# adobe-research/DiffusionHandles

Hardware: AMD Instinct MI355X
Metric: guided-denoise steps/sec at 512x512 (SD2-depth) (higher is better)
Workload: dtype f16; 1 GPU; single 512x512 edit per GPU, SD2-depth (865.9M params, seeded random weights), guided phase: 3 x (fwd + energy + bwd-to-latent) + CFG fwd (B=2) + DDIM step; resolution=512, edits_per_gpu=1, correspondences=24906, parallelism=independent edits, one process per GPU, no collectives

## Files before the change

diffusionhandles_amd/_lib.py:

```python
import ctypes
import os

import torch

_HERE = os.path.dirname(os.path.abspath(__file__))
LIB_PATH = os.environ.get("DIFFHANDLES_LIB") or os.path.join(_HERE, "libdiffhandles_hip.so")
_LIB = None

c_p = ctypes.c_void_p
c_i = ctypes.c_int
c_f = ctypes.c_float
c_d = ctypes.c_double
c_sz = ctypes.c_size_t


class UNetConfig(ctypes.Structure):
    _fields_ = [("in_channels", c_i), ("out_channels", c_i), ("n_levels", c_i),
                ("block_out_channels", c_i * 4), ("layers_per_block", c_i), ("heads", c_i * 4),
                ("cross_attention_dim", c_i), ("norm_groups", c_i), ("sample_size", c_i),
                ("text_len", c_i), ("max_batch", c_i), ("dtype", c_i), ("max_diff_batch", c_i)]


class VAEConfig(ctypes.Structure):
    _fields_ = [("latent_channels", c_i), ("out_channels", c_i), ("block_out_channels", c_i * 4),
# ... 74 lines not shown
    "dh_vae_encoder_create": (c_i, [c_p, ctypes.POINTER(c_p)]),
    "dh_vae_encoder_encode": (c_i, [c_p, c_p, c_i, c_p, c_p]),
    "dh_text_encoder_create": (c_i, [c_p, ctypes.POINTER(c_p)]),
    "dh_text_encoder_destroy": (None, [c_p]),
    "dh_text_encoder_num_params": (c_i, [c_p]),
    "dh_text_encoder_param_info": (c_i, [c_p, c_i, ctypes.POINTER(ctypes.c_char_p), ctypes.POINTER(c_i),
                                         ctypes.POINTER(ctypes.c_int64)]),
    "dh_text_encoder_load_param": (c_i, [c_p, c_i, c_p, c_p]),
    "dh_text_encoder_bytes": (c_sz, [c_p]),
    "dh_text_encoder_encode": (c_i, [c_p, c_p, c_i, c_i, c_p, c_p]),
    "dh_gemm_profile_begin": (c_i, []),
    "dh_gemm_profile_end": (c_i, [ctypes.POINTER(c_d), ctypes.POINTER(ctypes.c_int64), ctypes.POINTER(c_d)]),
    "dh_gemm_profile_bytes": (c_i, [ctypes.POINTER(c_d)]),
    "dh_ddim_cfg_step": (c_i, [c_p, c_p, c_p, c_p, c_f, c_f, c_f, c_i, c_p]),
    "dh_latent_update": (c_i, [c_p, c_p, c_p, c_f, c_f, c_i, c_p]),
    "dh_adam_step": (c_i, [c_p, c_p, c_p, c_p, c_f, c_f, c_f, c_f, c_i, c_i, c_p]),
    "dh_mse_fwd_bwd": (c_i, [c_p, c_p, c_i, c_p, c_p, c_p]),
    "dh_latent_update_strided": (c_i, [c_p, c_p, c_p, c_i, c_i, c_f, c_f, c_i, c_p]),
    "dh_pack_sample": (c_i, [c_p, c_p, c_i, c_i, c_p, c_i, c_i, c_i, c_i, c_p]),
    "dh_unet_io_ptr": (c_i, [c_p, c_i, c_i, ctypes.POINTER(c_p), ctypes.POINTER(c_sz)]),
    "dh_mse_cotangent": (c_i, [c_p, c_p, c_i, c_f, c_f, c_p, c_p, c_p, c_p]),
    "dh_adam_step_scaled": (c_i, [c_p, c_p, c_p, c_p, c_p, c_f, c_f, c_f, c_f, c_i, c_i, c_p]),
    "dh_mse_cotangent_batch": (c_i, [c_p, c_p, c_i, c_i, c_f, c_f, c_d, c_p, c_p, c_p, c_p, c_p, c_p]),
    "dh_adam_step_scaled_batch": (c_i, [c_p, c_p, c_p, c_p, c_p, c_p, c_f, c_f, c_f, c_f, c_i, c_i, c_i, c_p]),
    "dh_latent_update_guarded": (c_i, [c_p, c_p, c_p, c_i, c_i, c_f, c_i, c_i, c_p, c_i, c_i, c_p, c_p, c_i, c_i, c_p]),
    "dh_ddim_cfg_step_flagged": (c_i, [c_p, c_p, c_p, c_p, c_f, c_f, c_f, c_i, c_i, c_p, c_i, c_i, c_p]),
}

c_l = ctypes.c_long
DEBUG_SIGNATURES = {
    "dh_dbg_gemm": (c_i, [c_i, c_p, c_l, c_p, c_i, c_i, c_i, c_i, c_i, c_i, c_i, c_i, c_i, c_i, c_i, c_p, c_p, c_i, c_i,
                          c_p, c_l, c_p, c_l, c_i, c_p, c_sz, c_p]),
    "dh_dbg_gemm_groupnorm": (c_i, [c_i, c_p, c_l, c_p, c_i, c_i, c_i, c_i, c_i, c_i, c_i, c_p, c_p, c_p, c_sz, c_i, c_i, c_p, c_p, c_f, c_i,
                                    c_p, c_p, c_p, ctypes.POINTER(c_i), c_p]),
    "dh_dbg_gemm_groupnorm_bwd": (c_i, [c_i, c_p, c_l, c_p, c_i, c_i, c_i, c_i, c_i, c_i, c_i, c_p, c_p, c_sz, c_i, c_i, c_p, c_p, c_p, c_p, c_i,
                                        c_p, c_p, ctypes.POINTER(c_i), c_p]),
    "dh_dbg_gemm_groupnorm_res": (c_i, [c_i, c_p, c_l, c_p, c_i, c_i, c_i, c_i, c_i, c_i, c_i, c_p, c_p, c_l, c_p, c_p, c_sz, c_i, c_i, c_p, c_p,
                                    c_f, c_i, c_p, c_p, c_p, ctypes.POINTER(c_i), c_p]),
    "dh_dbg_gemm_groupnorm_bwd_res": (c_i, [c_i, c_p, c_l, c_p, c_i, c_i, c_i, c_i, c_i, c_i, c_i, c_p, c_l, c_p, c_p, c_sz, c_i, c_i, c_p, c_p, c_p,
                                        c_p, c_i, c_p, c_p, ctypes.POINTER(c_i), c_p]),
    "dh_dbg_concat_groupnorm": (c_i, [c_i, c_p, c_i, c_p, c_i, c_p, c_i, c_i, c_i, c_p, c_p, c_f, c_i, c_p, c_p, c_p, c_p]),
    "dh_dbg_gemm_last_tile": (c_i, [ctypes.POINTER(c_i)]),
    "dh_dbg_unet_concat_ops": (c_i, [ctypes.POINTER(UNetConfig), ctypes.POINTER(c_i), c_i, ctypes.POINTER(c_i)]),
    "dh_dbg_gemm_lnfold": (c_i, [c_i, c_p, c_l, c_p, c_i, c_i, c_i, c_p, c_p, c_p, c_f, c_p, c_l, c_p]),
    "dh_dbg_gemm_glu": (c_i, [c_i, c_i, c_p, c_l, c_p, c_i, c_i, c_i, c_p, c_p, c_p, c_p, c_p, c_p]),
    "dh_dbg_gemm_glub_split": (c_i, [c_i, c_p, c_l, c_p, c_i, c_i, c_i, c_i, c_p, c_l, c_i, c_p, c_p, ctypes.POINTER(c_i), c_p]),
    "dh_dbg_unet_ff_fold": (c_i, [c_p, c_i, ctypes.POINTER(c_i), ctypes.POINTER(c_i), c_p, c_p, c_p]),
    "dh_dbg_gemm_family": (c_i, [c_i]),
    "dh_dbg_gemm_stage": (c_i, [c_i]),
    "dh_dbg_gemm_xattn": (c_i, [c_i, c_p, c_l, c_p, c_i, c_i, c_i, c_p, c_p, c_p, c_p, c_f, c_p, c_p, c_p, c_l, c_p, c_p, c_i, c_i, c_i,
                                ctypes.POINTER(c_i), c_p]),
    "dh_dbg_gemm_xattn_dq": (c_i, [c_i, c_p, c_l, c_p, c_i, c_i, c_i, c_p, c_p, c_p, c_p, c_l, c_p, c_p, c_p, c_i, c_i, ctypes.POINTER(c_i), c_p]),
    "dh_dbg_gemm_xattn_carried": (c_i, [ctypes.POINTER(c_i), ctypes.POINTER(ctypes.c_longlong)]),
    "dh_dbg_gemm_pp_variant": (c_i, [c_i, c_p]),
    "dh_dbg_gemm_pp_ablate": (c_i, [c_i]),
    "dh_dbg_gemm_pp_persist": (c_i, [c_i]),
    "dh_dbg_gemm_pp_glu": (c_i, [c_i]),
    "dh_dbg_gemm_pp_plan": (c_i, [c_i, c_i, c_i, c_i, c_i, c_i, c_sz, ctypes.POINTER(c_i), ctypes.POINTER(c_i), ctypes.POINTER(c_i)]),
    "dh_dbg_touch_tiled": (c_i, [c_sz, c_p]),
    "dh_dbg_groupnorm": (c_i, [c_i, c_p, c_p, c_p, c_p, c_p, c_p, c_p, c_p, c_i, c_i, c_i, c_i, c_f, c_i, c_i, c_p]),
    "dh_dbg_layernorm": (c_i, [c_i, c_p, c_p, c_p, c_p, c_p, c_p, c_p, c_p, c_i, c_i, c_f, c_p]),
    "dh_dbg_geglu": (c_i, [c_i, c_p, c_p, c_p, c_p, c_i, c_i, c_p]),
    "dh_dbg_attention": (c_i, [c_i, c_p, c_l, c_p, c_p, c_l, c_p, c_l, c_p, c_p, c_p, c_p, c_p, c_p, c_i, c_i, c_i, c_i, c_p]),
    "dh_dbg_attention_bwd_pair": (c_i, [c_i, c_p, c_l, c_p, c_p, c_l, c_p, c_l, c_p, c_p, c_p, c_p, c_p, c_p, c_i, c_i, c_i, c_i, c_p, c_p]),
    "dh_dbg_pool2x2": (c_i, [c_i, c_p, c_p, c_i, c_i, c_i, c_i, c_i, c_p]),
    "dh_dbg_ellipse_offsets": (c_i, [c_i, ctypes.POINTER(ctypes.c_int32), c_i, ctypes.POINTER(c_i)]),
    "dh_dbg_lane_ops": (c_i, [c_p, c_p, c_p, c_p]),
    "dh_dbg_cg_limits": (c_i, [ctypes.POINTER(c_i)]),
    "dh_dbg_cg_max_iter": (c_i, [c_i]),
}


def lib():
    global _LIB
    if _LIB is None:
        if not os.path.exists(LIB_PATH):
            raise RuntimeError(
                f"native HIP library not found at {LIB_PATH}; build it with "
                "`python -c 'import __graft_entry__ as g; g.build()'` (there is no CPU fallback)")
        handle = ctypes.CDLL(LIB_PATH)
        missing = []
        for name, (res, args) in list(SIGNATURES.items()) + list(DEBUG_SIGNATURES.items()):
            try:
                fn = getattr(handle, name)
            except AttributeError:
                missing.append(name)
                continue
            fn.restype = res
            fn.argtypes = args
        handle.dh_missing_symbols = missing
        for env, fn in (("DH_GEMM_FAMILY", "dh_dbg_gemm_family"), ("DH_PP_GLU", "dh_dbg_gemm_pp_glu"),
                        ("DH_PP_PERSIST", "dh_dbg_gemm_pp_persist"), ("DH_GEMM_STAGE", "dh_dbg_gemm_stage")):
            if os.environ.get(env) and fn not in missing:
                getattr(handle, fn)(int(os.environ[env]))
        _LIB = handle
    return _LIB


def check(rc, what=""):
    if rc != 0:
        raise RuntimeError(f"{what} failed ({rc}): {lib().dh_last_error().decode()}")


def require_gpu(t=None):
    if not torch.cuda.is_available():
        raise RuntimeError("diffusionhandles_amd needs a HIP device (MI355X); there is no CPU fallback")
# ... 15 lines not shown
```

diffusionhandles_amd/csrc/debug_api.cpp:

```cpp
#include <stdlib.h>

#include "unet_kernels.h"
using namespace dh;

static void* g_dbg_tiled = nullptr;

__global__ void k_dbg_touch(const uint4* p, size_t n16, unsigned* sink) {
  unsigned acc = 0;
  for (size_t i = (size_t)blockIdx.x * blockDim.x + threadIdx.x; i < n16; i += (size_t)gridDim.x * blockDim.x) { const uint4 v = p[i]; acc ^= v.x ^ v.y ^ v.z ^ v.w; }
  if (acc == 0x9e3779b9u && sink) sink[0] = acc;
}
extern "C" int dh_dbg_touch_tiled(size_t bytes, void* stream) {
  DH_REQUIRE(g_dbg_tiled != nullptr, "no tiled weights yet (call dh_dbg_gemm first)");
  hipLaunchKernelGGL(k_dbg_touch, dim3(512), dim3(256), 0, (hipStream_t)stream, (const uint4*)g_dbg_tiled, bytes / 16, (unsigned*)nullptr);
  DH_LAUNCH_CHECK();
  return DH_OK;
}

extern "C" int dh_dbg_gemm(int dtype, const void* A, long lda, const void* W, int M, int N, int K, int mode, int Hin,
                           int Win, int Cin, int Hout, int Wout, int stride, int up, const float* bias,
                           const float* rowvec, int rowvec_ld, int rows_per_batch, const void* R, long ldr, void* C,
                           long ldc, int act_silu, float* partial, size_t partial_elems, void* stream) {
  DH_REQUIRE(A && W && C && K % 64 == 0 && N % 64 == 0, "bad arguments (N, K must be multiples of 64)");
  void*& tiled = g_dbg_tiled;
// ... 233 lines not shown
  DH_LAUNCH_CHECK();
  return DH_OK;
}
extern "C" int dh_dbg_attention(int dtype, const void* q, long ldq, const void* k, const void* v, long ldk, void* o,
                                long ldo, float* lse, const void* d_o, float* delta, void* dq, void* dk, void* dv,
                                int B, int H, int Nq, int Nk, void* stream) {
  hipStream_t st = (hipStream_t)stream;
  launch_attention_fwd(dtype, q, ldq, k, v, ldk, o, ldo, lse, B, H, Nq, Nk, st);
  if (d_o) {
    if (dq) launch_attention_bwd_dq(dtype, q, ldq, k, v, ldk, o, ldo, d_o, ldo, lse, delta, dq, ldq, B, H, Nq, Nk, st);
    else launch_attention_delta(dtype, o, ldo, d_o, ldo, delta, B, H, Nq, st);
    if (dk && dv) {
      static float* scratch = nullptr;
      constexpr size_t kScratch = (size_t)16 << 20;
      if (!scratch && hipMalloc((void**)&scratch, kScratch * sizeof(float)) != hipSuccess) scratch = nullptr;
      launch_attention_bwd_dkv(dtype, q, ldq, k, v, ldk, d_o, ldo, lse, delta, dk, dv, ldk, B, H, Nq, Nk, st, scratch,
                               scratch ? kScratch : 0);
    }
  }
  DH_LAUNCH_CHECK();
  return DH_OK;
}
extern "C" int dh_dbg_attention_bwd_pair(int dtype, const void* q, long ldq, const void* k, const void* v, long ldk, const void* o,
                                         long ldo, const float* lse, const void* d_o, float* delta, void* dq, void* dk, void* dv,
                                         int B, int H, int Nq, int Nk, void* stream, void* stream2) {
  hipStream_t st = (hipStream_t)stream, s2 = (hipStream_t)stream2;
  if (!s2) {
    launch_attention_bwd_dq(dtype, q, ldq, k, v, ldk, o, ldo, d_o, ldo, lse, delta, dq, ldq, B, H, Nq, Nk, st);
    launch_attention_bwd_dkv(dtype, q, ldq, k, v, ldk, d_o, ldo, lse, delta, dk, dv, ldk, B, H, Nq, Nk, st, nullptr, 0);
  } else {
    static hipEvent_t fork = nullptr, join = nullptr;
    if (!fork) { DH_CHECK_HIP(hipEventCreateWithFlags(&fork, hipEventDisableTiming)); DH_CHECK_HIP(hipEventCreateWithFlags(&join, hipEventDisableTiming)); }
    launch_attention_delta(dtype, o, ldo, d_o, ldo, delta, B, H, Nq, st);
    DH_CHECK_HIP(hipEventRecord(fork, st));
    DH_CHECK_HIP(hipStreamWaitEvent(s2, fork, 0));
    launch_attention_bwd_dkv(dtype, q, ldq, k, v, ldk, d_o, ldo, lse, delta, dk, dv, ldk, B, H, Nq, Nk, s2, nullptr, 0);
    launch_attention_bwd_dq(dtype, q, ldq, k, v, ldk, o, ldo, d_o, ldo, lse, nullptr, dq, ldq, B, H, Nq, Nk, st);
    DH_CHECK_HIP(hipEventRecord(join, s2));
    DH_CHECK_HIP(hipStreamWaitEvent(st, join, 0));
  }
  DH_LAUNCH_CHECK();
  return DH_OK;
}
extern "C" int dh_dbg_pool2x2(int dtype, const void* src, void* dst, int B, int h, int w, int C, int accumulate, void* stream) {
  launch_pool2x2_sum(dtype, src, dst, B, h, w, C, accumulate, (hipStream_t)stream);
  DH_LAUNCH_CHECK();
  return DH_OK;
}
extern "C" int dh_dbg_lane_ops(const float* in, float* out, unsigned* ex, void* stream) {
  launch_lane_ops_probe(in, out, ex, (hipStream_t)stream);
  DH_LAUNCH_CHECK();
  return DH_OK;
}
```

diffusionhandles_amd/csrc/gemm.hip:

```cpp
#include <stdlib.h>

#include <vector>

#include <hip/hip_ext.h>

#include "attn_tile.h"
#include "gemm_k.h"

namespace dh {

struct GemmProf {
  bool on = false;
  std::vector<hipEvent_t> ev;
  size_t used = 0;
  double flops = 0;
  double bytes = 0;
  hipEvent_t e0 = nullptr, e1 = nullptr;
};
static GemmProf g_prof;
static int g_buf_stage = 1;
static int g_pp_force = 0;
struct GemmTileReport {
  int bm, bn, kg, stages, mw, splits, pp, gn_epi, reduce_gn;
};
static thread_local GemmTileReport g_last_tile;
static thread_local int g_last_xattn = 0;
static thread_local long long g_xattn_total = 0;
#ifdef DH_TUNING
static unsigned long long* g_gemm_ts = nullptr;
#endif
bool gemm_profiling_on() { return g_prof.on; }

constexpr int BK = 64;
#ifdef DH_EXP_SETPRIO
#define DH_PRIO(x) __builtin_amdgcn_s_setprio(x)
#else
#define DH_PRIO(x) do { } while (0)
#endif


template <class T>
__device__ __forceinline__ uint2 epilogue_pack(const GemmK& p, int m, int n, float v0, float v1, float v2, float v3,
                                               bool have_r, uint2 rpre, bool have_b, float4 bpre) {
  float v[4] = {v0, v1, v2, v3};
  if (p.bias) {
    float4 b = bpre;
    if (!have_b) b = *reinterpret_cast<const float4*>(p.bias + n);
    v[0] += b.x; v[1] += b.y; v[2] += b.z; v[3] += b.w;
  }
  if (p.rowvec) {
    const float4 b = *reinterpret_cast<const float4*>(p.rowvec + (size_t)div_small(m, p.inv_rows_per_batch) * p.rowvec_ld + n);
    v[0] += b.x; v[1] += b.y; v[2] += b.z; v[3] += b.w;
  }
  if (p.act_silu) {
#pragma unroll
    for (int i = 0; i < 4; ++i) v[i] = v[i] / (1.f + __expf(-v[i]));
  }
  typedef T T4 __attribute__((ext_vector_type(4)));
  if (p.R) {
    const T* r = reinterpret_cast<const T*>(p.R) + (size_t)m * p.ldr + n;
    uint2 raw = rpre;
    if (!have_r) raw = *reinterpret_cast<const uint2*>(r);
    const T4 rv = __builtin_bit_cast(T4, raw);
#pragma unroll
    for (int i = 0; i < 4; ++i) v[i] += to_f32<T>(rv[i]);
  }
  T4 o;
#pragma unroll
  for (int i = 0; i < 4; ++i) o[i] = from_f32<T>(v[i]);
  return __builtin_bit_cast(uint2, o);
}
template <class T>
__device__ __forceinline__ void epilogue_store(const GemmK& p, int m, int n, float v0, float v1, float v2, float v3,
                                               bool have_r = false, uint2 rpre = make_uint2(0, 0), bool have_b = false,
                                               float4 bpre = make_float4(0.f, 0.f, 0.f, 0.f)) {
  *reinterpret_cast<uint2*>(reinterpret_cast<T*>(p.C) + (size_t)m * p.ldc + n) =
      epilogue_pack<T>(p, m, n, v0, v1, v2, v3, have_r, rpre, have_b, bpre);
}

template <class T>
__device__ __forceinline__ float epilogue_scalar(const GemmK& p, int m, int n, float v) {
  if (p.bias) v += p.bias[n];
  if (p.rowvec) v += p.rowvec[(size_t)div_small(m, p.inv_rows_per_batch) * p.rowvec_ld + n];
  if (p.act_silu) v = v / (1.f + __expf(-v));
  if (p.R) v += to_f32<T>(reinterpret_cast<const T*>(p.R)[(size_t)m * p.ldr + n]);
  return to_f32<T>(from_f32<T>(v));
}

__device__ uint4 g_zero_page[8];

__device__ __forceinline__ void dma16(const void* gsrc, unsigned lds_dst) {
  unsigned keep;
  asm volatile("s_mov_b32 %0, m0\n\ts_mov_b32 m0, %2\n\ts_nop 0\n\tglobal_load_lds_dwordx4 %1, off\n\ts_mov_b32 m0, %0"
               : "=&s"(keep) : "v"(gsrc), "s"(lds_dst) : "memory");
}

__device__ __forceinline__ void dma16_nt(const void* gsrc, unsigned lds_dst) {
  unsigned keep;
  asm volatile("s_mov_b32 %0, m0\n\ts_mov_b32 m0, %2\n\ts_nop 0\n\tglobal_load_lds_dwordx4 %1, off nt\n\ts_mov_b32 m0, %0"
               : "=&s"(keep) : "v"(gsrc), "s"(lds_dst) : "memory");
}

typedef int buf_v4i __attribute__((ext_vector_type(4)));
__device__ __forceinline__ void buf_dma16(unsigned voff, buf_v4i rsrc, unsigned soff, unsigned lds_dst) {
  unsigned tmp;
  soff = __builtin_amdgcn_readfirstlane(soff);
  lds_dst = __builtin_amdgcn_readfirstlane(lds_dst);
  asm volatile("s_mov_b32 m0, %4\n\ts_mov_b32 %0, %3\n\tbuffer_load_dwordx4 %1, %2, %0 offen lds"
               : "=&s"(tmp) : "v"(voff), "s"(rsrc), "s"(soff), "s"(lds_dst) : "memory");
}
__device__ __forceinline__ unsigned buf_mask_oob(unsigned nt, unsigned sh, unsigned voff) {
  return ((nt << sh) & 0x80000000u) | voff;
}

template <int N> __device__ __forceinline__ void wait_vmcnt() { asm volatile("s_waitcnt vmcnt(%0)" ::"n"(N) : "memory"); }

enum { GM_DENSE = 0, GM_CONV_S1 = 1, GM_GENERIC = 2 };
#ifdef DH_TUNING
#define LNF_ABL(bit) && !(p.lnf_abl & (bit))
#define LEAN_ABL && !(p.lnf_abl & 8)
#define DH_STAMP(i) do { if (p.ts && blockIdx.x == 0 && blockIdx.y == 0 && blockIdx.z == 0 && threadIdx.x == 0) p.ts[i] = __builtin_amdgcn_s_memtime(); } while (0)
#define DH_STAMP_T(kt, j) do { if (p.ts && (kt) < 40 && blockIdx.x == 0 && blockIdx.y == 0 && blockIdx.z == 0 && threadIdx.x == 0) p.ts[8 + 3 * (kt) + (j)] = __builtin_amdgcn_s_memtime(); } while (0)
#else
#define DH_STAMP_T(kt, j) do { } while (0)
#define LNF_ABL(bit)
#define LEAN_ABL
#define DH_STAMP(i) do { } while (0)
#endif

typedef _Float16 v2h __attribute__((ext_vector_type(2)));
typedef __bf16 v2b __attribute__((ext_vector_type(2)));
typedef unsigned u4v __attribute__((ext_vector_type(4)));
template <class T> __device__ __forceinline__ void frag_sums(const uint4& f, float& s1, float& s2);
template <> __device__ __forceinline__ void frag_sums<f16>(const uint4& f_in, float& s1, float& s2) {
  const v2h one = {(_Float16)1.f, (_Float16)1.f};
  u4v f = __builtin_bit_cast(u4v, f_in);
  asm("" : "+v"(f));
  const unsigned w[4] = {f[0], f[1], f[2], f[3]};
#pragma unroll
  for (int i = 0; i < 4; ++i) {
    const v2h h = __builtin_bit_cast(v2h, w[i]);
    s1 = __builtin_amdgcn_fdot2(h, one, s1, false);
    s2 = __builtin_amdgcn_fdot2(h, h, s2, false);
  }
}
template <> __device__ __forceinline__ void frag_sums<bf16>(const uint4& f_in, float& s1, float& s2) {
  const v2b one = {(__bf16)1.f, (__bf16)1.f};
  u4v f = __builtin_bit_cast(u4v, f_in);
  asm("" : "+v"(f));
  const unsigned w[4] = {f[0], f[1], f[2], f[3]};
#pragma unroll
  for (int i = 0; i < 4; ++i) {
    const v2b h = __builtin_bit_cast(v2b, w[i]);
    s1 = __builtin_amdgcn_fdot2_f32_bf16(h, one, s1, false);
    s2 = __builtin_amdgcn_fdot2_f32_bf16(h, h, s2, false);
  }
}

constexpr bool gn_epi_fwd_tile(int BN, int GLU, bool LNF) { return GLU == 0 && !LNF && BN % 64 == 0 && BN <= 128; }
constexpr bool gn_epi_bwd_tile(int BM, int BN, int WG, int GLU, bool LNF) {
  return gn_epi_fwd_tile(BN, GLU, LNF) && BN == 64 && BM <= 128 && WG == 1;
}

template <class T, int BM, int BN, int ST, int MODE, int ABL = 0, int WG = 1, int KG = 1, int MW = 1, bool LNF = false, int GLU = 0, bool BUF = false>
__global__ void __launch_bounds__(256 * WG * KG * MW) k_gemm_dma(const GemmK p) {
  static_assert(!BUF || MODE != GM_GENERIC, "the generic gather stages through addresses");
  static_assert((WG == 1) + (KG == 1) + (MW == 1) >= 2, "one kind of wave grouping per instantiation");
  static_assert(!LNF || (WG == 1 && MODE == GM_DENSE), "the folded LayerNorm needs every k-step of a row in one wave group");
  DH_STAMP(0);
  constexpr int NWV = 4 * MW;
  constexpr int WNS = BN % 64 ? 1 : 2, WMS = NWV / WNS;
  constexpr int RPW = BM / WMS, CPW = BN / WNS;
  constexpr int TM = RPW / 32, TN = CPW / 32;
  static_assert(RPW % 32 == 0 && CPW % 32 == 0, "a wave owns whole 32 x 32 blocks");
  static_assert(WNS == 2 || (!LNF && GLU == 0 && WG == 1 && KG == 1), "the one-column arrangement carries the plain epilogue only");
  constexpr int NPA = BM / 32 / WG / MW, NPB = BN / 32 / WG / MW;
  constexpr int NP = NPA + NPB;
  constexpr int STAGE = (BM + BN) * 128;
  __shared__ __attribute__((aligned(1024))) unsigned char smem_all[KG * ST * STAGE];

  const int tid = threadIdx.x, lane = tid & 63, wave = (tid >> 6) & (NWV - 1);
  const int grp = WG > 1 ? __builtin_amdgcn_readfirstlane(tid >> 8) : 0;
  const int kg = KG > 1 ? __builtin_amdgcn_readfirstlane(tid >> 8) : 0;
  unsigned char* smem = smem_all + kg * (ST * STAGE);
  const int wm = WNS == 2 ? wave >> 1 : wave, wn = WNS == 2 ? wave & 1 : 0, ln = lane & 31, hi = lane >> 5;
  const int m0 = blockIdx.x * BM, n0 = blockIdx.y * BN;
  int kbeg = blockIdx.z * p.k_per_split;
  int kend = kbeg + p.k_per_split;
  if (kend > p.K) kend = p.K;
  int ntiles = (kend - kbeg) / BK;
  int loop_tiles = ntiles;
  if (KG > 1) {
    loop_tiles = (ntiles + KG - 1) / KG;
    kbeg += kg * loop_tiles * BK;
    ntiles -= kg * loop_tiles;
    ntiles = ntiles < 0 ? 0 : (ntiles > loop_tiles ? loop_tiles : ntiles);
  }
  const T* Ag = reinterpret_cast<const T*>(p.A);
  const int wave_s = __builtin_amdgcn_readfirstlane(wave);
  const unsigned lds0 = (unsigned)(size_t)((__attribute__((address_space(3))) unsigned char*)smem_all) + kg * (ST * STAGE);
  const int prow = lane >> 3;
  const int lchunk = (lane & 7) ^ (4 * (wave & 1) + (prow >> 1));
  const T* zero = reinterpret_cast<const T*>(g_zero_page) + (lane & 7) * 8;

  const float inv_hw = MODE == GM_DENSE ? 0.f : __builtin_amdgcn_rcpf((float)(p.Hout * p.Wout));
  const float inv_w = MODE == GM_DENSE ? 0.f : __builtin_amdgcn_rcpf((float)p.Wout);
  bool a_ok[NPA];
  long a_off[NPA];
  int a_oy[NPA], a_ox[NPA];
#pragma unroll
  for (int j = 0; j < NPA; ++j) {
    const int m = m0 + 8 * (wave + NWV * (j * WG + grp)) + prow;
    a_ok[j] = m < p.M;
    if (MODE == GM_DENSE) {
      a_off[j] = (long)(a_ok[j] ? m : p.M - 1) * p.lda + lchunk * 8;
      a_oy[j] = a_ox[j] = 0;
    } else {
      const int hw = p.Hout * p.Wout;
      const int b = div_small(m, inv_hw), r = m - b * hw;
      a_oy[j] = div_small(r, inv_w);
      a_ox[j] = r - a_oy[j] * p.Wout;
      if (MODE == GM_CONV_S1) a_off[j] = (((long)b * p.Hin + a_oy[j]) * p.Win + a_ox[j]) * p.lda + lchunk * 8;
      else a_off[j] = (long)b * p.Hin * p.Win;
    }
  }
  unsigned a_taps[NPA];
#pragma unroll
  for (int j = 0; j < NPA; ++j) {
    a_taps[j] = 0;
    if (MODE == GM_CONV_S1 && a_ok[j]) {
#pragma unroll
      for (int t = 0; t < 9; ++t)
        if ((unsigned)(a_oy[j] + t / 3 - 1) < (unsigned)p.Hin && (unsigned)(a_ox[j] + t % 3 - 1) < (unsigned)p.Win) a_taps[j] |= 1u << t;
    }
  }
  const T* Wg = reinterpret_cast<const T*>(p.W);
  const int KT = p.K >> 6;
  const T* b_ptr[NPB];
#pragma unroll
  for (int j = 0; j < NPB; ++j) {
    const int row = 8 * (wave + NWV * (j * WG + grp));
    b_ptr[j] = Wg + ((size_t)((n0 + row) >> 6) * KT) * 4096 + (size_t)((n0 + row) & 63) * 64 + lane * 8;
  }
  int tap = 0, c0 = 0;
  if (MODE != GM_DENSE) { const int kt0 = kbeg >> 6, ch = kt0 / 9; tap = kt0 - ch * 9; c0 = ch * BK; }
  typedef int bv4i __attribute__((ext_vector_type(4)));
  bv4i ra = {0, 0, 0, 0}, rw = {0, 0, 0, 0};
  unsigned bv_a[NPA], bv_nt[NPA], bs_w[NPB];
  unsigned bs_tap = 0, bs_sh = 0;
  unsigned bs_step_px = 0, bs_step_row = 0; int bs_kx = 0;
  const unsigned bv_w = lane * 16;
  if constexpr (BUF) {
    const unsigned a_bias = MODE == GM_CONV_S1 ? (unsigned)((p.Win + 1) * (int)p.lda * 2) : 0u;
    const size_t a_base = (size_t)p.A - a_bias;
    ra[0] = (int)(unsigned)a_base; ra[1] = (int)((a_base >> 32) & 0xffff); ra[2] = (int)(p.pp_a_bytes + a_bias); ra[3] = 0x00020000;
    rw[0] = (int)(unsigned)(size_t)p.W; rw[1] = (int)(((size_t)p.W >> 32) & 0xffff); rw[2] = (int)p.pp_w_bytes; rw[3] = 0x00020000;
#pragma unroll
    for (int j = 0; j < NPA; ++j) {
      const int m = m0 + 8 * (wave + NWV * (j * WG + grp)) + prow;
      if (MODE == GM_DENSE) {
        bv_a[j] = a_ok[j] ? (unsigned)m * (unsigned)((int)p.lda * 2) + (unsigned)lchunk * 16u : 0x80000000u;
        bv_nt[j] = 0;
      } else {
        const int hw = p.Hout * p.Wout;
        const int b = div_small(m, inv_hw);
        (void)hw;
        bv_a[j] = (unsigned)((b * p.Hin + a_oy[j]) * p.Win + a_ox[j]) * (unsigned)((int)p.lda * 2) + (unsigned)lchunk * 16u;
        bv_nt[j] = ~a_taps[j];
      }
    }
#pragma unroll
    for (int j = 0; j < NPB; ++j) {
      const int n = n0 + 8 * (wave_s + NWV * (j * WG + grp));
      bs_w[j] = (unsigned)(((n >> 6) * KT) * 8192 + (n & 63) * 128);
    }
    if (MODE == GM_CONV_S1) {
      const int ky = tap / 3, kx = tap - ky * 3;
      bs_tap = (unsigned)((ky * p.Win + kx) * (int)p.lda + c0) * 2u;
      bs_sh = 31u - (unsigned)tap;
      bs_kx = kx;
      bs_step_px = (unsigned)((int)p.lda * 2);
      bs_step_row = (unsigned)((p.Win - 2) * (int)p.lda * 2);
    }
  }

  auto issue_piece = [&](int kt, int stage, int q) {
    const int k0 = kbeg + kt * BK;
    const unsigned sbase = __builtin_amdgcn_readfirstlane(lds0 + stage * STAGE + wave_s * 1024);
    if constexpr (BUF) {
      if (q < NPA) {
        const int j = q;
        const unsigned dst = sbase + (j * WG + grp) * (NWV * 1024);
        if (MODE == GM_DENSE) buf_dma16(bv_a[j], ra, (unsigned)k0 * 2u, dst);
        else buf_dma16(buf_mask_oob(bv_nt[j], bs_sh, bv_a[j]), ra, bs_tap, dst);
      } else {
        const int j = q - NPA;
        buf_dma16(bv_w, rw, bs_w[j] + (unsigned)(k0 >> 6) * 8192u, sbase + BM * 128 + (j * WG + grp) * (NWV * 1024));
      }
      return;
    }
    if (q < NPA) {
      const int j = q;
      if (MODE == GM_DENSE) {
        const T* ptr = Ag + a_off[j] + k0;
        dma16(ptr, sbase + (j * WG + grp) * (NWV * 1024));
      } else if (MODE == GM_CONV_S1) {
        const int ky = tap / 3, kx = tap - ky * 3;
        const long toff = ((long)(ky - 1) * p.Win + (kx - 1)) * p.lda + c0;
        const bool ok = (a_taps[j] & (1u << tap)) != 0;
        const T* ptr = Ag + a_off[j] + toff;
        dma16(ok ? ptr : zero, sbase + (j * WG + grp) * (NWV * 1024));
      } else {
        const int ky = tap / 3, kx = tap - ky * 3;
        bool ok = a_ok[j];
        int sy, sx;
        if (p.mode == A_CONV3) {
          const int iy = a_oy[j] * p.stride + ky - p.pad, ix = a_ox[j] * p.stride + kx - p.pad;
          ok = ok && iy >= 0 && ix >= 0 && iy < (p.Hin << p.up) && ix < (p.Win << p.up);
          sy = iy >> p.up; sx = ix >> p.up;
        } else {
          const int ty = a_oy[j] + ky - 1, tx = a_ox[j] + kx - 1;
          ok = ok && ty >= 0 && tx >= 0 && !(ty & 1) && !(tx & 1) && (ty >> 1) < p.Hin && (tx >> 1) < p.Win;
          sy = ty >> 1; sx = tx >> 1;
        }
        sy = sy < 0 ? 0 : (sy >= p.Hin ? p.Hin - 1 : sy);
        sx = sx < 0 ? 0 : (sx >= p.Win ? p.Win - 1 : sx);
        const T* ptr = Ag + (a_off[j] + (long)sy * p.Win + sx) * p.lda + c0 + lchunk * 8;
        dma16(ok ? ptr : zero, sbase + (j * WG + grp) * (NWV * 1024));
      }
    } else {
      const int j = q - NPA;
#ifdef DH_TUNING
      if (p.w_nt) dma16_nt(b_ptr[j] + (size_t)(k0 >> 6) * 4096, sbase + BM * 128 + (j * WG + grp) * (NWV * 1024));
      else
#endif
      dma16(b_ptr[j] + (size_t)(k0 >> 6) * 4096, sbase + BM * 128 + (j * WG + grp) * (NWV * 1024));
    }
  };
  auto next_tile = [&]() {
    if constexpr (BUF && MODE == GM_CONV_S1) {
      ++tap; ++bs_kx;
      const bool row_end = bs_kx == 3;
      bs_tap += row_end ? bs_step_row : bs_step_px;
      bs_kx = row_end ? 0 : bs_kx;
      if (tap == 9) { tap = 0; c0 += BK; bs_tap = (unsigned)c0 * 2u; }
      bs_sh = 31u - (unsigned)tap;
      return;
    }
    if (MODE != GM_DENSE) { if (++tap == 9) { tap = 0; c0 += BK; } }
  };
  auto issue = [&](int kt, int stage) {
#pragma unroll
    for (int q = 0; q < NP; ++q) issue_piece(kt, stage, q);
    next_tile();
  };

  v16f acc[TM][TN];
#pragma unroll
  for (int i = 0; i < TM; ++i)
#pragma unroll
    for (int j = 0; j < TN; ++j)
#pragma unroll
      for (int r = 0; r < 16; ++r) acc[i][j][r] = 0.f;

  const int wn_u = __builtin_amdgcn_readfirstlane(wn);
  float ln1[TM], ln2[TM];
#pragma unroll
  for (int i = 0; i < TM; ++i) { ln1[i] = 0.f; ln2[i] = 0.f; }

#pragma unroll
  for (int s = 0; s < ST - 1; ++s)
    if (s < ntiles) issue(s, s);
  DH_STAMP(1);

  constexpr bool PRE = TM * TN <= 8;
  const bool pre_r = PRE && p.R != nullptr && p.pre_r && p.splits == 1 && (WG == 1 || grp == 0) && (KG == 1 || kg == 0) &&
                     (GLU != 2 || !glub_tile_is_glu(n0, p.glub_f));
  constexpr bool PRE_B = PRE && !(MW == 2 && BN == 320) && WNS == 2;
  const bool pre_b = PRE_B && p.bias != nullptr && p.pre_r && p.splits == 1;
  float4 bpre[PRE_B ? TN : 1][4];
  if (pre_b) {
#pragma unroll
    for (int j = 0; j < TN; ++j)
#pragma unroll
      for (int g = 0; g < 4; ++g) {
        const int n = n0 + wn * CPW + j * 32 + 8 * g + 4 * hi;
        bpre[PRE_B ? j : 0][g] = n < p.N ? *reinterpret_cast<const float4*>(p.bias + n) : make_float4(0.f, 0.f, 0.f, 0.f);
      }
  }
  constexpr bool PRE_LN = LNF && PRE && !(MW == 2 && BM == 256);
  float4 lsp[PRE_LN ? TN : 1][4], ltp[PRE_LN ? TN : 1][4];
  if (PRE_LN) {
#pragma unroll
    for (int j = 0; j < TN; ++j)
#pragma unroll
      for (int g = 0; g < 4; ++g) {
        const int n = n0 + wn * CPW + j * 32 + 8 * g + 4 * hi;
        lsp[PRE_LN ? j : 0][g] = n < p.N ? *reinterpret_cast<const float4*>(p.ln_s + n) : make_float4(0.f, 0.f, 0.f, 0.f);
        ltp[PRE_LN ? j : 0][g] = n < p.N ? *reinterpret_cast<const float4*>(p.ln_t + n) : make_float4(0.f, 0.f, 0.f, 0.f);
      }
  }
  constexpr bool GNB = gn_epi_bwd_tile(BM, BN, WG, GLU, LNF);
  static_assert(!GNB || (PRE && WNS == 2), "the backward form carries the GroupNorm input tile in the residual's prefetch registers");
  const bool gnb = GNB && p.gn_epi == 2 && p.splits == 1;
  const bool pre_x = gnb && (KG == 1 || kg == 0);
  float4 gnb_col = make_float4(0.f, 0.f, 0.f, 0.f);
  if (GNB && pre_x && tid < BN) {
    const int n = n0 + tid, grp_n = (int)(((float)n + 0.5f) / (float)p.gn_cpg);
    const float2 st2 = *reinterpret_cast<const float2*>(p.gnb_stats + 2 * ((m0 / p.gn_HW) * p.gn_G + grp_n));
    gnb_col = make_float4(p.gnb_gamma[n], p.gnb_beta[n], st2.x, st2.y);
  }
  uint2 rpre[TM][TN][4];
  if (pre_r || pre_x) {
    const T* rsrc = reinterpret_cast<const T*>(pre_x ? p.gnb_x : p.R);
    const long rld = pre_x ? p.gnb_ldx : p.ldr;
#pragma unroll
    for (int i = 0; i < TM; ++i) {
      const int m = m0 + wm * RPW + i * 32 + ln;
#pragma unroll
      for (int j = 0; j < TN; ++j)
#pragma unroll
        for (int g = 0; g < 4; ++g) {
          const int n = n0 + wn * CPW + j * 32 + 8 * g + 4 * hi;
          rpre[i][j][g] = (m < p.M && n < p.N) ? *reinterpret_cast<const uint2*>(rsrc + (size_t)m * rld + n) : make_uint2(0, 0);
        }
    }
  }

  constexpr bool XA = GLU == EPI_XATTN || GLU == EPI_XATTN_DQ, XB = GLU == EPI_XATTN_DQ;
  static_assert(!XB || !LNF, "the input-gradient GEMM carries no LayerNorm");
  static_assert(!XA || xattn_epi_tile(BM, BN, WG, MW, BUF), "the cross-attention epilogue lives on the buffer-staged 64x64 / 128x64 tiles");
  constexpr int XA_CH = XA_KEYS * 8 / 256;
  u4v xa_kr[XA ? XA_CH : 1], xa_vr[XA ? XA_CH : 1];
  if constexpr (XA) {
    if (KG == 1 || kg == 0) {
      const int b = div_small(m0, __builtin_amdgcn_rcpf((float)p.xa_Nq));
      const size_t head = (size_t)b * p.xa_Nk * p.xa_ldk + n0;
      const T* kp = reinterpret_cast<const T*>(p.xa_k) + head;
      const T* vp = reinterpret_cast<const T*>(p.xa_v) + head;
#pragma unroll
      for (int j = 0; j < XA_CH; ++j) {
        const int idx = tid + j * 256;
        int r = idx >> 3;
        r = r < p.xa_Nk ? r : p.xa_Nk - 1;
        const size_t off = (size_t)r * p.xa_ldk + (idx & 7) * 8;
        xa_kr[j] = *reinterpret_cast<const u4v*>(kp + off);
        xa_vr[j] = *reinterpret_cast<const u4v*>(vp + off);
      }
    }
  }
  constexpr int XA_WPR = XA ? 4 / (BM / 32) : 1;
  u4v xb_qf[XB ? 4 : 1], xb_of[XB ? 4 : 1];
  float xb_lse = 0.f;
  if constexpr (XB) {
    if (KG == 1 || kg == 0) {
      int m = m0 + (wave_s / XA_WPR) * 32 + ln;
      m = m < p.M ? m : p.M - 1;
      const T* qp = reinterpret_cast<const T*>(p.xa_q) + (size_t)m * p.xa_ldq + n0 + 8 * hi;
      const T* op = reinterpret_cast<const T*>(p.xa_o) + (size_t)m * p.xa_ldo + n0 + 8 * hi;
#pragma unroll
      for (int kk = 0; kk < 4; ++kk) {
        xb_qf[kk] = *reinterpret_cast<const u4v*>(qp + 16 * kk);
        xb_of[kk] = *reinterpret_cast<const u4v*>(op + 16 * kk);
      }
      const int b = div_small(m0, __builtin_amdgcn_rcpf((float)p.xa_Nq));
      xb_lse = p.xa_lse[((size_t)b * p.xa_H + blockIdx.y) * p.xa_Nq + (m - b * p.xa_Nq)] * LOG2E;
    }
  }

  constexpr int KK = BK / 16 / WG;
  const int kk0 = grp * KK;
  unsigned fa_off[BK / 16], fb_off[BK / 16];
#pragma unroll
  for (int kk = 0; kk < BK / 16; ++kk) {
    const unsigned pc = (unsigned)(((2 * kk + hi) ^ ((ln >> 1) & 7)) << 4);
    fa_off[kk] = (unsigned)((wm * RPW + ln) * 128) + pc;
    fb_off[kk] = (unsigned)(BM * 128 + (wn * CPW + ln) * 128) + pc;
// ... 481 lines not shown
      if (tid < (BN / 8) * 8 && g < G && g * cpg < n0 + BN) {
        const int lo = g * cpg, hi_c = lo + cpg;
        const int c_lo = (lo > n0 ? lo : n0) - n0, c_hi = (hi_c < n0 + BN ? hi_c : n0 + BN) - n0;
        const int b = m0 / p.gn_HW, rt = (m0 - b * p.gn_HW) / BM;
        const int part = lo < n0 ? 1 : 0;
        if (GNB && gnb) {
          float a = 0.f, q = 0.f;
          for (int c = c_lo + sub; c < c_hi; c += 8) {
#pragma unroll
            for (int w2 = 0; w2 < WMS; ++w2) { const float2 v = *reinterpret_cast<const float2*>(cs + (w2 * BN + c) * 2); a += v.x; q += v.y; }
          }
          a = oct_sum(a); q = oct_sum(q);
          if (sub == 0) {
            float2* o = reinterpret_cast<float2*>(p.gn_part) + (size_t)(b * G + g) * Sx + 2 * rt + part;
            o[0] = make_float2(a, q);
            if (part == 0 && hi_c <= n0 + BN) o[1] = make_float2(0.f, 0.f);
          }
        } else {
          const float ref = cs[c_lo * 2];
          float dm = 0.f;
          for (int c = c_lo + sub; c < c_hi; c += 8) {
#pragma unroll
            for (int w2 = 0; w2 < WMS; ++w2) dm += cs[(w2 * BN + c) * 2] - ref;
          }
          dm = oct_sum(dm);
          const float pieces = (float)WMS * (float)(c_hi - c_lo);
          const float mean = ref + dm / pieces;
          float m2 = 0.f;
          for (int c = c_lo + sub; c < c_hi; c += 8) {
#pragma unroll
            for (int w2 = 0; w2 < WMS; ++w2) {
              const float2 v = *reinterpret_cast<const float2*>(cs + (w2 * BN + c) * 2);
              const float d = v.x - mean;
              m2 += v.y + (float)RPW * d * d;
            }
          }
          m2 = oct_sum(m2);
          if (sub == 0) {
            float* o = p.gn_part + ((size_t)(b * G + g) * 3) * Sx + 2 * rt + part;
            o[0] = (float)RPW * pieces; o[Sx] = mean; o[2 * Sx] = m2;
            if (part == 0 && hi_c <= n0 + BN) { o[1] = 0.f; o[Sx + 1] = 0.f; o[2 * Sx + 1] = 0.f; }
          }
        }
      }
    }
  };
  if (PRE && p.splits == 1 && p.wide_store && p.pre_r && !p.rowvec && !p.act_silu LEAN_ABL) {
    typedef T T4 __attribute__((ext_vector_type(4)));
    const bool hb = p.bias != nullptr, hr = p.R != nullptr;
#pragma unroll
    for (int i = 0; i < TM; ++i) {
      const int m = m0 + wm * RPW + i * 32 + ln;
      if (m >= p.M) continue;
      T* orow = reinterpret_cast<T*>(p.C) + (size_t)m * p.ldc + n0 + wn * CPW + 8 * hi;
#pragma unroll
      for (int j = 0; j < TN; ++j) {
        if (n0 + wn * CPW + j * 32 >= p.N) continue;
        uint2 w[4];
#pragma unroll
        for (int g = 0; g < 4; ++g) {
          float v0 = acc[i][j][4 * g], v1 = acc[i][j][4 * g + 1], v2 = acc[i][j][4 * g + 2], v3 = acc[i][j][4 * g + 3];
          if (hb) {
            float4 b = bpre[PRE_B ? j : 0][g];
            if (!PRE_B) b = *reinterpret_cast<const float4*>(p.bias + n0 + wn * CPW + j * 32 + 8 * g + 4 * hi);
            v0 += b.x; v1 += b.y; v2 += b.z; v3 += b.w;
          }
          if (hr) {
            const T4 rv = __builtin_bit_cast(T4, rpre[i][j][g]);
            v0 += to_f32<T>(rv[0]); v1 += to_f32<T>(rv[1]); v2 += to_f32<T>(rv[2]); v3 += to_f32<T>(rv[3]);
          }
          T4 o;
          o[0] = from_f32<T>(v0); o[1] = from_f32<T>(v1); o[2] = from_f32<T>(v2); o[3] = from_f32<T>(v3);
          w[g] = __builtin_bit_cast(uint2, o);
          if (gn_epi) { if (GNB && gnb) gnb_acc(g, w[g], rpre[i][j][g]); else gn_acc(i, j, g, w[g]); }
        }
        const uint4 ca = half_exchange(w[0], w[1]), cb = half_exchange(w[2], w[3]);
        *reinterpret_cast<uint4*>(orow + j * 32) = ca;
        *reinterpret_cast<uint4*>(orow + j * 32 + 16) = cb;
      }
      if (GNB && gnb) asm volatile("" ::: "memory");
    }
    if (gn_epi) gn_finish();
    DH_STAMP(6);
#ifdef DH_TUNING
    if (p.ts) { asm volatile("s_waitcnt vmcnt(0)" ::: "memory"); DH_STAMP(7); }
#endif
    return;
  }
  if (p.splits == 1 && p.wide_store) {
#pragma unroll
    for (int i = 0; i < TM; ++i) {
      const int m = m0 + wm * RPW + i * 32 + ln;
      if (m >= p.M) continue;
#pragma unroll
      for (int j = 0; j < TN; ++j) {
        const int nb = n0 + wn * CPW + j * 32;
        if (nb >= p.N) continue;
        uint2 w[4];
#pragma unroll
        for (int g = 0; g < 4; ++g) {
          w[g] = epilogue_pack<T>(p, m, nb + 8 * g + 4 * hi, acc[i][j][4 * g], acc[i][j][4 * g + 1], acc[i][j][4 * g + 2],
                                  acc[i][j][4 * g + 3], pre_r, rpre[i][j][g], pre_b, bpre[PRE_B ? j : 0][g]);
          if (gn_epi) gn_acc(i, j, g, w[g]);
        }
        const uint4 ca = half_exchange(w[0], w[1]), cb = half_exchange(w[2], w[3]);
        T* out = reinterpret_cast<T*>(p.C) + (size_t)m * p.ldc + nb + 8 * hi;
        *reinterpret_cast<uint4*>(out) = ca;
        *reinterpret_cast<uint4*>(out + 16) = cb;
      }
    }
    if (gn_epi) gn_finish();
    DH_STAMP(6);
#ifdef DH_TUNING
    if (p.ts) { asm volatile("s_waitcnt vmcnt(0)" ::: "memory"); DH_STAMP(7); }
#endif
    return;
  }

#pragma unroll
  for (int i = 0; i < TM; ++i) {
    const int m = m0 + wm * RPW + i * 32 + ln;
    if (m >= p.M) continue;
#pragma unroll
    for (int j = 0; j < TN; ++j)
#pragma unroll
      for (int g = 0; g < 4; ++g) {
        const int n = n0 + wn * CPW + j * 32 + 8 * g + 4 * hi;
        if (n >= p.N) continue;
        if (p.splits > 1) {
          float4 o = make_float4(acc[i][j][4 * g], acc[i][j][4 * g + 1], acc[i][j][4 * g + 2], acc[i][j][4 * g + 3]);
          *reinterpret_cast<float4*>(p.partial + ((size_t)blockIdx.z * p.M + m) * p.N + n) = o;
        } else {
          epilogue_store<T>(p, m, n, acc[i][j][4 * g], acc[i][j][4 * g + 1], acc[i][j][4 * g + 2], acc[i][j][4 * g + 3], pre_r,
                            rpre[i][j][g], pre_b, bpre[PRE_B ? j : 0][g]);
        }
      }
  }
}

template <class T>
__global__ void k_tile_weights(const T* src, T* dst, int N, int K, int conv_cin) {
  const size_t idx = (size_t)blockIdx.x * blockDim.x + threadIdx.x;
  if (idx >= (size_t)N * K) return;
  const int n = (int)(idx / K);
  int k = (int)(idx - (size_t)n * K);
  if (conv_cin) { const int tap = k / conv_cin; k = conv_k_index(tap, k - tap * conv_cin); }
  dst[wt_index(n, k, K)] = src[idx];
}
void launch_tile_weights(int dtype, const void* src, void* dst, int N, int K, hipStream_t st, int conv_cin) {
  const unsigned nb = (unsigned)(((size_t)N * K + 255) / 256);
  hipLaunchKernelGGL((k_tile_weights<unsigned short>), dim3(nb), dim3(256), 0, st, (const unsigned short*)src, (unsigned short*)dst, N, K, conv_cin);
}

template <class T>
__global__ void k_splitk_reduce(const GemmK p) {
  const size_t q = (size_t)blockIdx.x * blockDim.x + threadIdx.x;
  const size_t total = (size_t)p.M * p.N / 4;
  if (q >= total) return;
  const size_t e = q * 4;
  const int m = (int)((unsigned)e / (unsigned)p.N), n = (int)((unsigned)e - (unsigned)m * (unsigned)p.N);
  const bool have_r = p.R != nullptr, have_b = p.bias != nullptr;
  const uint2 rpre = have_r ? *reinterpret_cast<const uint2*>(reinterpret_cast<const T*>(p.R) + (size_t)m * p.ldr + n) : make_uint2(0, 0);
  const float4 bpre = have_b ? *reinterpret_cast<const float4*>(p.bias + n) : make_float4(0.f, 0.f, 0.f, 0.f);
  const size_t slab = (size_t)p.M * p.N;
  float4 s = make_float4(0.f, 0.f, 0.f, 0.f);
  int z = 0;
  for (; z + 4 <= p.splits; z += 4) {
    float4 v[4];
#pragma unroll
    for (int j = 0; j < 4; ++j) v[j] = *reinterpret_cast<const float4*>(p.partial + (size_t)(z + j) * slab + e);
#pragma unroll
    for (int j = 0; j < 4; ++j) { s.x += v[j].x; s.y += v[j].y; s.z += v[j].z; s.w += v[j].w; }
  }
  for (; z < p.splits; ++z) {
    const float4 v = *reinterpret_cast<const float4*>(p.partial + (size_t)z * slab + e);
    s.x += v.x; s.y += v.y; s.z += v.z; s.w += v.w;
  }
  epilogue_store<T>(p, m, n, s.x, s.y, s.z, s.w, have_r, rpre, have_b, bpre);
}

template <class T, bool BWD>
__global__ void __launch_bounds__(256) k_splitk_reduce_gn(const GemmK p) {
  __shared__ float sm_red[4][2 * GN_GB];
  __shared__ float sm_piv[GN_GB];
  const int HW = p.gn_HW, G = p.gn_G, S = p.gn_S;
  const int s = blockIdx.x, g0 = blockIdx.y * GN_GB, b = blockIdx.z, cpg = div_small(p.N, rcp_fast(G));
  const int W = GN_GB * cpg, nch = W >> 3;
  const float inv_nch = rcp_fast(nch), inv_S = rcp_fast(S), inv_cpg = rcp_fast(cpg);
  const int RP = div_small((int)blockDim.x, inv_nch);
  const int r0 = div_small(HW * s, inv_S), r1 = div_small(HW * (s + 1), inv_S);
  const size_t slab = (size_t)p.M * p.N;
  const int rr = div_small((int)threadIdx.x, inv_nch), ch = threadIdx.x - rr * nch;
  float ga[GN_GB], gq[GN_GB];
#pragma unroll
  for (int gl = 0; gl < GN_GB; ++gl) { ga[gl] = 0.f; gq[gl] = 0.f; }
  const int n = g0 * cpg + ch * 8;
  const bool live = rr < RP && n < p.N;
  int gi[8];
  float av[8], qv[8], pv[8];
#pragma unroll
  for (int i = 0; i < 8; ++i) {
    gi[i] = div_small(ch * 8 + i, inv_cpg);
    av[i] = 0.f; qv[i] = 0.f; pv[i] = 0.f;
  }
  float bias8[8] = {0.f, 0.f, 0.f, 0.f, 0.f, 0.f, 0.f, 0.f};
  float gm[8], bt[8], mu[8], rs[8];
  if (live) {
    if (p.bias) {
      *reinterpret_cast<float4*>(bias8) = *reinterpret_cast<const float4*>(p.bias + n);
      *reinterpret_cast<float4*>(bias8 + 4) = *reinterpret_cast<const float4*>(p.bias + n + 4);
    }
    if (BWD) {
      *reinterpret_cast<float4*>(gm) = *reinterpret_cast<const float4*>(p.gnb_gamma + n);
// ... 79 lines not shown
      for (int r = r0 + rr; r < r1; r += RP) row(r, f);
  } else {
    const bool first = live && r0 + rr < r1;
    if (first) row(r0 + rr, f);
    if (first && rr == 0) {
#pragma unroll
      for (int i = 0; i < 8; ++i)
        if (ch * 8 + i == gi[i] * cpg) sm_piv[gi[i]] = f[i];
    }
    __syncthreads();
#pragma unroll
    for (int i = 0; i < 8; ++i) pv[i] = g0 + gi[i] < G ? sm_piv[gi[i]] : 0.f;
    if (first) {
      acc(f);
      for (int r = r0 + rr + RP; r < r1; r += RP) { row(r, f); acc(f); }
    }
  }
  if (live) {
#pragma unroll
    for (int i = 0; i < 8; ++i)
#pragma unroll
      for (int gl = 0; gl < GN_GB; ++gl) {
        ga[gl] += gi[i] == gl ? av[i] : 0.f;
        gq[gl] += gi[i] == gl ? qv[i] : 0.f;
      }
  }
#pragma unroll
  for (int gl = 0; gl < GN_GB; ++gl) { ga[gl] = wave_sum(ga[gl]); gq[gl] = wave_sum(gq[gl]); }
  if ((threadIdx.x & 63) == 0) {
#pragma unroll
    for (int gl = 0; gl < GN_GB; ++gl) { sm_red[threadIdx.x >> 6][2 * gl] = ga[gl]; sm_red[threadIdx.x >> 6][2 * gl + 1] = gq[gl]; }
  }
  __syncthreads();
  if ((int)threadIdx.x < GN_GB && g0 + (int)threadIdx.x < G) {
    const int gl = threadIdx.x, g = g0 + gl;
    float sa = 0.f, sq = 0.f;
    for (int w = 0; w < 4; ++w) { sa += sm_red[w][2 * gl]; sq += sm_red[w][2 * gl + 1]; }
    if (BWD) {
      p.gn_part[((size_t)(b * G + g) * S + s) * 2] = sa;
      p.gn_part[((size_t)(b * G + g) * S + s) * 2 + 1] = sq;
    } else {
      const float cnt = (float)(r1 - r0) * (float)cpg;
      float* o = p.gn_part + ((size_t)(b * G + g) * 3) * S + s;
      o[0] = cnt; o[S] = sm_piv[gl] + sa / cnt; o[2 * S] = sq - sa * sa / cnt;
    }
  }
}

#define DH_GEMM_LAUNCH(KERNEL)                                                                              \
  do {                                                                                                      \
    if (g_prof.e0) hipExtLaunchKernelGGL(KERNEL, grid, dim3(TH), 0, st, g_prof.e0, g_prof.e1, 0, k);        \
    else hipLaunchKernelGGL(KERNEL, grid, dim3(TH), 0, st, k);                                              \
  } while (0)
template <class T, int BM, int BN, int ST, int WG, int KG, int MW, bool BUF>
static void launch_tile_b(int gm, bool lnf, dim3 grid, hipStream_t st, const GemmK& k, int glu) {
  constexpr int TH = 256 * WG * KG * MW;
  constexpr bool GLUOK = WG == 1 && KG == 1 && ((BM == 256 && BN == 128 && MW == 2) || (BM == 128 && BN == 128 && MW == 2 && ST == 4) || (BM == 64 && BN == 64));
  if constexpr (GLUOK) {
    if (glu == 1 && lnf) { DH_GEMM_LAUNCH((k_gemm_dma<T, BM, BN, ST, GM_DENSE, 0, WG, KG, MW, true, 1, BUF>)); return; }
    if (glu == 1) { DH_GEMM_LAUNCH((k_gemm_dma<T, BM, BN, ST, GM_DENSE, 0, WG, KG, MW, false, 1, BUF>)); return; }
    if (glu == 2) { DH_GEMM_LAUNCH((k_gemm_dma<T, BM, BN, ST, GM_DENSE, 0, WG, KG, MW, false, 2, BUF>)); return; }
  }
  if constexpr (xattn_epi_tile(BM, BN, WG, MW, BUF)) {
    if (glu == EPI_XATTN && lnf) { DH_GEMM_LAUNCH((k_gemm_dma<T, BM, BN, ST, GM_DENSE, 0, WG, KG, MW, true, EPI_XATTN, BUF>)); return; }
    if (glu == EPI_XATTN) { DH_GEMM_LAUNCH((k_gemm_dma<T, BM, BN, ST, GM_DENSE, 0, WG, KG, MW, false, EPI_XATTN, BUF>)); return; }
    if (glu == EPI_XATTN_DQ) { DH_GEMM_LAUNCH((k_gemm_dma<T, BM, BN, ST, GM_DENSE, 0, WG, KG, MW, false, EPI_XATTN_DQ, BUF>)); return; }
  }
  if (gm == GM_DENSE) {
    if constexpr (WG == 1 && BN != 320 && BN != 160) {
      if (lnf) { DH_GEMM_LAUNCH((k_gemm_dma<T, BM, BN, ST, GM_DENSE, 0, WG, KG, MW, true, 0, BUF>)); return; }
    }
    DH_GEMM_LAUNCH((k_gemm_dma<T, BM, BN, ST, GM_DENSE, 0, WG, KG, MW, false, 0, BUF>));
  } else if (gm == GM_CONV_S1) {
    DH_GEMM_LAUNCH((k_gemm_dma<T, BM, BN, ST, GM_CONV_S1, 0, WG, KG, MW, false, 0, BUF>));
  } else {
    DH_GEMM_LAUNCH((k_gemm_dma<T, BM, BN, ST, GM_GENERIC, 0, WG, KG, MW>));
  }
}
template <class T, int BM, int BN, int ST, int WG, int KG, int MW>
static void launch_tile(int gm, bool lnf, dim3 grid, hipStream_t st, const GemmK& k, int glu = 0) {
  g_last_tile.bm = BM; g_last_tile.bn = BN; g_last_tile.kg = KG; g_last_tile.stages = ST; g_last_tile.mw = MW;
  if (k.pp_a_bytes != 0 && gm != GM_GENERIC) launch_tile_b<T, BM, BN, ST, WG, KG, MW, true>(gm, lnf, grid, st, k, glu);
  else launch_tile_b<T, BM, BN, ST, WG, KG, MW, false>(gm, lnf, grid, st, k, glu);
}
#undef DH_GEMM_LAUNCH

#ifdef DH_TUNING
#define DH_KNOB(name, env, dflt) static const int name = getenv(env) ? atoi(getenv(env)) : (dflt)
#else
#define DH_KNOB(name, env, dflt) constexpr int name = (dflt)
#endif

template <class T>
static void gemm_dispatch(GemmK k, size_t partial_elems, hipStream_t st, int* gn_done, int* lnb_done, int* xa_done, int dtype) {
  DH_KNOB(kSplitTiles, "DH_SPLITK_TILES", 200);
  DH_KNOB(kSplitMinK, "DH_SPLITK_MINKT", 32);
  DH_KNOB(kSplitTarget, "DH_SPLITK_TARGET", 256);
  DH_KNOB(kBigTiles, "DH_BIG_TILES", 128);
  DH_KNOB(kNarrowTiles, "DH_NARROW_TILES", 40);
  DH_KNOB(kN320, "DH_GEMM_N320", 224);
  DH_KNOB(kMwBlocks, "DH_GEMM_MW", 64);
  DH_KNOB(kKg2MinKt, "DH_KG2_MINKT", 4);
  DH_KNOB(kManyBlocks, "DH_GEMM_MANY", 512);
  DH_KNOB(kMw128, "DH_GEMM_MW128", 1);
  DH_KNOB(kTwoPerCu, "DH_GEMM_TWO_PER_CU", 1);
#ifdef DH_TUNING
  DH_KNOB(kWnt, "DH_W_NT", 0);
#endif
  const bool lnf = k.ln_s != nullptr;
  g_last_tile = GemmTileReport{};
  int BM = 128, BN = (k.N % 128 == 0) ? 128 : 64;
  const int ktiles = k.K / BK;
  PpPlan pp;
  const bool use_pp = gemm_pp_plan(k, partial_elems, g_pp_force, &pp);
  if (BN == 128 && ktiles >= 16 && cdiv(k.M, 128) * cdiv(k.N, 128) <= kNarrowTiles) BN = 64;
  if (k.M <= 64 || (cdiv(k.M, 128) * cdiv(k.N, BN) < kBigTiles && ktiles < kSplitMinK)) { BM = 64; BN = 64; }
  const bool n320 = kN320 > 0 && k.N % 320 == 0 && k.N <= 960 && !lnf && BM == 128 && BN == 64 && cdiv(k.M, 128) >= kN320;
  if (n320) BN = 320;
  DH_KNOB(kMwShortK, "DH_GEMM_MW_SHORTK", 128);
  const long tiles256 = (long)cdiv(k.M, 256) * cdiv(k.N, 128);
  const bool mw2 = kMwBlocks > 0 && k.N % 128 == 0 && tiles256 >= kMwBlocks &&
                   !(k.M <= 256 && k.M > 128 && cdiv(k.N, 128) < 128) && (tiles256 >= kMwShortK || ktiles >= kSplitMinK);
  if (mw2) { BM = 256; BN = 128; }
  const int glu = k.glu_y ? 1 : (k.glub_x ? 2 : 0);
  if (glu && !(BM == 64 && BN == 64)) { BM = mw2 ? 256 : 128; BN = 128; }
  if (glu == 2 && !glub_split_ok(BN, k.glub_f)) { BM = 64; BN = 64; }
  DH_KNOB(kT160, "DH_GEMM_T160", 224);
  const long tiles160 = (long)cdiv(k.M, 128) * (k.N / 160);
  const bool t160 = kT160 > 0 && k.N % 160 == 0 && !lnf && !glu && !n320 && BM != 64 && tiles160 >= kT160 && tiles160 <= 256;
  if (t160) { BM = 128; BN = 160; }
  if (use_pp) { BM = pp.bm; BN = pp.bn; }
  const int tm = cdiv(k.M, BM), tn = cdiv(k.N, BN), tiles = tm * tn;
  int splits = 1;
  if (use_pp) splits = pp.splits;
  else if (k.partial && !lnf && !glu && tiles < kSplitTiles && ktiles >= kSplitMinK) {
    splits = kSplitTarget / tiles;
    if (splits > ktiles / 4) splits = ktiles / 4;
    if (splits > 32) splits = 32;
    const size_t fit = partial_elems / ((size_t)k.M * k.N);
    if ((size_t)splits > fit) splits = (int)fit;
    if (splits < 1) splits = 1;
  }
#ifdef DH_TUNING
  static const int kLog = getenv("DH_GEMM_LOG") ? atoi(getenv("DH_GEMM_LOG")) : 0;
  const int kForceTile = getenv("DH_FORCE_TILE") ? atoi(getenv("DH_FORCE_TILE")) : 0;
  const int kForceSplits = getenv("DH_FORCE_SPLITS") ? atoi(getenv("DH_FORCE_SPLITS")) : 0;
  int force_tile = 0;
  if (kForceTile && !use_pp && !(k.glu_y || k.glub_x)) {
    const int fbm = kForceTile == 1 ? 64 : (kForceTile == 6 ? 256 : 128), fbn = kForceTile == 7 ? 160 : ((kForceTile <= 3) ? 64 : 128);
    if ((k.N % fbn == 0 || fbn == 64) && !(fbn == 160 && lnf)) { BM = fbm; BN = fbn; force_tile = kForceTile; }
  }
  if (kForceSplits && !use_pp && k.partial && !lnf) {
    splits = kForceSplits;
    if (splits > ktiles / 2) splits = ktiles / 2 > 0 ? ktiles / 2 : 1;
    const size_t fit = partial_elems / ((size_t)k.M * k.N);
    if ((size_t)splits > fit) splits = (int)fit;
    if (splits < 1) splits = 1;
  }
  if (kLog) fprintf(stderr, "GEMMLOG M=%d N=%d K=%d mode=%d lnf=%d gn=%d gnb=%d bias=%d R=%d rowvec=%d | pp=%d BM=%d BN=%d splits=%d\n", k.M, k.N, k.K,
                    k.mode == A_DENSE ? 0 : (k.mode == A_CONV3 && k.stride == 1 && k.up == 0 ? 1 : 2), (int)lnf, k.gn_part != nullptr,
                    k.gnb_x != nullptr, k.bias != nullptr, k.R != nullptr, k.rowvec != nullptr, (int)use_pp, BM, BN, splits);
#endif
  const int tiles_per_split = cdiv(ktiles, splits);
  splits = cdiv(ktiles, tiles_per_split);
  k.splits = splits;
  k.k_per_split = tiles_per_split * BK;
  k.gn_epi = 0; k.gn_cpg = 0;
  if ((g_buf_stage & 4) == 0 && splits == 1 && !use_pp && gn_epi_fwd_tile(BN, glu, lnf) && k.gn_part && !k.gnb_x && gn_done && k.gn_G > 0 &&
      k.gn_HW > 0 && k.C && k.wide_store && k.M % k.gn_HW == 0 && k.gn_HW % BM == 0 && k.N % k.gn_G == 0 && k.N % BN == 0) {
    const int cpg = k.N / k.gn_G, sx = 2 * (k.gn_HW / BM);
    if (cpg >= 8 && cpg <= BN && sx <= 64) { k.gn_epi = 1; k.gn_cpg = cpg; k.gn_S = sx; }
  }
  if ((g_buf_stage & 8) == 0 && splits == 1 && !use_pp && gn_epi_bwd_tile(BM, BN, 1, glu, lnf) && k.gn_part && k.gnb_x && gn_done && k.gn_G > 0 &&
      k.gn_HW > 0 && k.C && k.wide_store && k.pre_r && !k.R && !k.bias && !k.rowvec && !k.act_silu && k.M % k.gn_HW == 0 && k.gn_HW % BM == 0 &&
      k.N % k.gn_G == 0 && k.N % BN == 0 && (((size_t)k.gnb_x | (size_t)(k.gnb_ldx * 2)) & 7) == 0) {
    const int cpg = k.N / k.gn_G, sx = 2 * (k.gn_HW / BM);
    if (cpg >= 8 && cpg <= BN && sx <= 64) { k.gn_epi = 2; k.gn_cpg = cpg; k.gn_S = sx; }
  }
#ifdef DH_TUNING
  k.w_nt = kWnt > 0 && tm <= kWnt;
  static const int kLnfAbl = getenv("DH_LNF_ABL") ? atoi(getenv("DH_LNF_ABL")) : 0;
  k.lnf_abl = kLnfAbl;
  k.ts = g_gemm_ts;
#endif
#ifdef DH_TUNING
  dim3 grid(force_tile ? cdiv(k.M, BM) : tm, force_tile ? cdiv(k.N, BN) : tn, splits);
#else
  dim3 grid(tm, tn, splits);
#endif
  int gm = GM_GENERIC;
  if (k.mode == A_DENSE) gm = GM_DENSE;
  else if (k.mode == A_CONV3 && k.stride == 1 && k.up == 0 && k.pad == 1) gm = GM_CONV_S1;
  if (!use_pp) {
    k.pp_a_bytes = 0; k.pp_w_bytes = 0;
    size_t ab = 0;
    if (k.mode == A_DENSE) ab = ((size_t)(k.M - 1) * k.lda + k.K) * 2;
    else if (k.Hout > 0 && k.Wout > 0 && k.M % (k.Hout * k.Wout) == 0)
      ab = (size_t)(k.M / (k.Hout * k.Wout)) * k.Hin * k.Win * (size_t)k.lda * 2;
    const size_t wb = (size_t)align_up((size_t)k.N, 64) * k.K * 2;
    const bool conv_ok = k.mode == A_DENSE || (k.Cin % 64 == 0 && k.K == 9 * k.Cin);
    if ((g_buf_stage & 1) && ab > 0 && conv_ok && ab + (size_t)(k.Win + 1) * k.lda * 2 < 0x7ff00000ull && wb < 0x7ff00000ull && k.lda % 8 == 0 &&
        ((size_t)k.A & 15) == 0 && ((size_t)k.W & 15) == 0) {
      k.pp_a_bytes = (unsigned)ab; k.pp_w_bytes = (unsigned)wb;
    }
  }
  k.xa = 0;
  const bool xa_bwd = k.xa_dq != nullptr;
  if (k.xa_o && xa_done && (g_buf_stage & (xa_bwd ? 32 : 16)) == 0 && splits == 1 && !use_pp && !glu && !t160 && !n320 && !mw2 &&
      xattn_epi_tile(BM, BN, 1, 1, k.pp_a_bytes != 0) && gm == GM_DENSE && k.xa_Nk >= 1 && k.xa_Nk <= XA_KEYS && k.xa_Nq > 0 &&
      k.N == 64 * k.xa_H && k.M % k.xa_Nq == 0 && k.M < (1 << 22) && (k.M == k.xa_Nq || k.xa_Nq % BM == 0) && k.C && k.wide_store && k.pre_r &&
      !k.R && !k.rowvec && !k.act_silu && !k.gn_epi && k.xa_lse && k.xa_ldk % 8 == 0 && k.xa_ldo % 8 == 0 &&
      (((size_t)k.xa_k | (size_t)k.xa_v | (size_t)k.xa_o) & 15) == 0 &&
      (!xa_bwd || (!lnf && !k.bias && k.xa_q && k.xa_ldq % 8 == 0 && k.xa_lddq % 8 == 0 && (((size_t)k.xa_q | (size_t)k.xa_dq) & 15) == 0)))
    k.xa = xa_bwd ? 2 : 1;
#ifdef DH_TUNING
  if (force_tile) k.xa = 0;
#endif
  const int epi = k.xa == 2 ? EPI_XATTN_DQ : (k.xa ? EPI_XATTN : glu);
  hipEvent_t e0 = nullptr, e1 = nullptr;
  if (g_prof.on) {
    if (g_prof.used + 2 > g_prof.ev.size()) {
      const size_t old = g_prof.ev.size();
      g_prof.ev.resize(old + 4096);
      for (size_t i = old; i < g_prof.ev.size(); ++i) (void)hipEventCreate(&g_prof.ev[i]);
    }
    e0 = g_prof.ev[g_prof.used++];
    e1 = g_prof.ev[g_prof.used++];
    g_prof.flops += 2.0 * (double)k.M * (double)k.N * (double)k.K;
    const double esz = 2.0;
    double a_elems = (double)k.M * k.K;
    if (k.mode != A_DENSE && k.Hout > 0 && k.Wout > 0) a_elems = (double)k.M / ((double)k.Hout * k.Wout) * k.Hin * k.Win * k.Cin;
    double c_elems = (double)k.M * k.N * (k.C ? 1.0 : 0.0) + (k.R ? (double)k.M * k.N : 0.0);
    if (k.glu_y) c_elems += 0.5 * (double)k.M * k.N;
    if (k.glub_x) c_elems += 4.0 * (double)k.M * k.glub_f - (k.C ? (double)k.M * k.glub_f : 0.0);
    if (k.gn_epi == 2) c_elems += (double)k.M * k.N;
    if (k.xa == 1) c_elems += (k.xa_save ? 1.0 : 0.0) * (double)k.M * k.N + 2.0 * (k.M / k.xa_Nq) * (double)k.xa_Nk * k.N;
    if (k.xa == 2) c_elems += 2.0 * (double)k.M * k.N + 2.0 * (k.M / k.xa_Nq) * (double)k.xa_Nk * k.N;
    g_prof.bytes += esz * (a_elems + (double)k.N * k.K + c_elems);
    g_prof.e0 = e0; g_prof.e1 = e1;
  }
#ifdef DH_TUNING
  static const int kAbl = getenv("DH_GEMM_ABLATE") ? atoi(getenv("DH_GEMM_ABLATE")) : 0;
  if (kAbl == 1 && BM == 128 && BN == 128) { hipLaunchKernelGGL((k_gemm_dma<T, 128, 128, 4, GM_CONV_S1, 1>), grid, dim3(256), 0, st, k); }
  else if (kAbl == 2 && BM == 128 && BN == 128) { hipLaunchKernelGGL((k_gemm_dma<T, 128, 128, 4, GM_CONV_S1, 2>), grid, dim3(256), 0, st, k); }
  else if (kAbl == 3 && BM == 128 && BN == 128) { hipLaunchKernelGGL((k_gemm_dma<T, 128, 128, 4, GM_DENSE, 1>), grid, dim3(256), 0, st, k); }
  else if (kAbl == 1 && mw2 && gm == GM_CONV_S1) { hipLaunchKernelGGL((k_gemm_dma<T, 256, 128, 3, GM_CONV_S1, 1, 1, 1, 2>), grid, dim3(512), 0, st, k); }
  else if (kAbl == 2 && mw2 && gm == GM_CONV_S1) { hipLaunchKernelGGL((k_gemm_dma<T, 256, 128, 3, GM_CONV_S1, 2, 1, 1, 2>), grid, dim3(512), 0, st, k); }
  else if (kAbl == 1 && mw2 && gm == GM_DENSE && !lnf) { hipLaunchKernelGGL((k_gemm_dma<T, 256, 128, 3, GM_DENSE, 1, 1, 1, 2>), grid, dim3(512), 0, st, k); }
  else if (kAbl == 2 && mw2 && gm == GM_DENSE && !lnf) { hipLaunchKernelGGL((k_gemm_dma<T, 256, 128, 3, GM_DENSE, 2, 1, 1, 2>), grid, dim3(512), 0, st, k); }
  else if (force_tile == 1) launch_tile<T, 64, 64, 4, 1, 1, 1>(gm, lnf, grid, st, k);
  else if (force_tile == 2) launch_tile<T, 128, 64, 3, 1, 2, 1>(gm, lnf, grid, st, k);
  else if (force_tile == 3) launch_tile<T, 128, 64, 5, 1, 1, 1>(gm, lnf, grid, st, k);
  else if (force_tile == 4) launch_tile<T, 128, 128, 4, 1, 1, 2>(gm, lnf, grid, st, k);
  else if (force_tile == 5) launch_tile<T, 128, 128, 4, 1, 1, 1>(gm, lnf, grid, st, k);
  else if (force_tile == 6) launch_tile<T, 256, 128, 3, 1, 1, 2>(gm, lnf, grid, st, k);
  else if (force_tile == 7) launch_tile<T, 128, 160, 4, 1, 1, 1>(gm, false, grid, st, k);
  else
#endif
  if (use_pp) { pp.splits = splits; g_last_tile.bm = pp.bm; g_last_tile.bn = pp.bn; launch_gemm_pp(dtype, k, pp, st, g_prof.e0, g_prof.e1); }
  else if (t160) launch_tile<T, 128, 160, 4, 1, 1, 1>(gm, false, grid, st, k);
  else if (mw2) launch_tile<T, 256, 128, 3, 1, 1, 2>(gm, lnf, grid, st, k, glu);
  else if (BM == 128 && BN == 128 && (glu || (kMw128 && tiles_per_split >= kMw128))) launch_tile<T, 128, 128, 4, 1, 1, 2>(gm, lnf, grid, st, k, glu);
  else if (kTwoPerCu && BM == 128 && BN == 64 && tiles * splits > 256 && tiles * splits <= 512)
    launch_tile<T, 128, 64, 3, 1, 1, 1>(gm, lnf, grid, st, k, epi);
  else if (BM == 128 && BN == 64 && tiles_per_split >= kKg2MinKt) launch_tile<T, 128, 64, 3, 1, 2, 1>(gm, lnf, grid, st, k, epi);
  else if (BN == 320) launch_tile<T, 128, 320, 2, 1, 1, 2>(gm, false, grid, st, k);
  else if (BM == 64) launch_tile<T, 64, 64, 4, 1, 1, 1>(gm, lnf, grid, st, k, epi);
  else if (BN == 128 && kManyBlocks > 0 && tiles * splits >= kManyBlocks) launch_tile<T, 128, 128, 2, 1, 1, 1>(gm, lnf, grid, st, k);
  else if (BN == 128) launch_tile<T, 128, 128, 4, 1, 1, 1>(gm, lnf, grid, st, k);
  else launch_tile<T, 128, 64, 5, 1, 1, 1>(gm, lnf, grid, st, k, epi);
  g_prof.e0 = g_prof.e1 = nullptr;
  g_last_xattn = k.xa;
  if (k.xa) { ++g_xattn_total; *xa_done = 1; }
  g_last_tile.splits = splits; g_last_tile.pp = use_pp ? 1 : 0; g_last_tile.gn_epi = k.gn_epi;
  if (k.gn_epi) *gn_done = k.gn_S;
  if (splits > 1) {
    if (k.gn_part && k.gn_G > 0 && k.gn_HW > 0 && k.N % k.gn_G == 0 && (GN_GB * (k.N / k.gn_G)) % 8 == 0 &&
        GN_GB * (k.N / k.gn_G) <= 2048 && k.M % k.gn_HW == 0) {
      k.gn_S = gn_slices(k.gn_HW, k.M / k.gn_HW);
      if (k.gnb_x) hipLaunchKernelGGL((k_splitk_reduce_gn<T, true>), dim3(k.gn_S, cdiv(k.gn_G, GN_GB), k.M / k.gn_HW), dim3(256), 0, st, k);
      else hipLaunchKernelGGL((k_splitk_reduce_gn<T, false>), dim3(k.gn_S, cdiv(k.gn_G, GN_GB), k.M / k.gn_HW), dim3(256), 0, st, k);
      g_last_tile.reduce_gn = 1;
      if (gn_done) *gn_done = 1;
    } else if (k.lnb_x && lnb_done && !k.bias && !k.rowvec && !k.R && !k.act_silu && k.N % 8 == 0 && k.ldc == k.N) {
      launch_splitk_reduce_ln_bwd(dtype, k.partial, splits, k.lnb_x, k.lnb_gamma, k.lnb_stats, k.lnb_add, k.lnb_dx, k.M, k.N, st, k.lnb_ldx);
      *lnb_done = 1;
    } else {
      const size_t groups = (size_t)k.M * k.N / 4;
      hipLaunchKernelGGL((k_splitk_reduce<T>), dim3((unsigned)((groups + 255) / 256)), dim3(256), 0, st, k);
    }
  }
}
#undef DH_KNOB

double launch_gemm(int dtype, const GemmArgs& a, hipStream_t st) {
  GemmK k;
  k.A = a.A; k.lda = a.lda; k.W = a.W; k.M = a.M; k.N = a.N; k.K = a.K;
  k.mode = a.mode; k.Hin = a.Hin; k.Win = a.Win; k.Cin = a.Cin; k.Hout = a.Hout; k.Wout = a.Wout;
  k.stride = a.stride; k.up = a.up; k.pad = a.pad;
  k.bias = a.bias; k.rowvec = a.rowvec; k.rowvec_ld = a.rowvec_ld;
  k.rows_per_batch = a.rows_per_batch > 0 ? a.rows_per_batch : 1;
  k.inv_rows_per_batch = 1.f / (float)k.rows_per_batch;
  k.R = a.R; k.ldr = a.ldr; k.C = a.C; k.ldc = a.ldc; k.act_silu = a.act_silu;
  k.partial = a.partial; k.splits = 1; k.k_per_split = a.K;
  k.pre_r = 1;
  k.wide_store = a.N % 32 == 0 && a.ldc % 8 == 0 && ((size_t)a.C & 15) == 0;
  k.ln_s = a.ln_s; k.ln_t = a.ln_t; k.ln_stats = a.ln_stats; k.ln_eps = a.ln_eps;
  k.gn_part = a.gn_part; k.gn_HW = a.gn_HW; k.gn_G = a.gn_G; k.gn_S = 0;
  k.gnb_x = a.gnb_x; k.gnb_ldx = a.gnb_ldx; k.gnb_gamma = a.gnb_gamma; k.gnb_beta = a.gnb_beta; k.gnb_stats = a.gnb_stats;
  k.gnb_silu = a.gnb_silu;
  k.lnb_x = a.lnb_x; k.lnb_ldx = a.lnb_ldx > 0 ? a.lnb_ldx : a.N;
  k.lnb_gamma = a.lnb_gamma; k.lnb_stats = a.lnb_stats; k.lnb_add = a.lnb_add; k.lnb_dx = a.lnb_dx;
  k.glu_y = a.glu_y; k.glu_ldy = a.glu_ldy; k.glub_x = a.glub_x; k.glub_dx = a.glub_dx;
  k.glub_f = a.glub_x && a.glub_f > 0 && a.glub_f < a.N ? a.glub_f : a.N;
  if (k.glub_f < a.N) {
    if (k.C) k.C = reinterpret_cast<unsigned short*>(k.C) - k.glub_f;
    if (k.R) k.R = reinterpret_cast<const unsigned short*>(k.R) - k.glub_f;
  } else if (a.glub_x) {
    k.C = nullptr;
  }
  k.xa = 0; k.xa_k = a.xa_k; k.xa_v = a.xa_v; k.xa_ldk = a.xa_ldk; k.xa_o = a.xa_o; k.xa_ldo = a.xa_ldo; k.xa_lse = a.xa_lse;
  k.xa_H = a.xa_H; k.xa_Nq = a.xa_Nq; k.xa_Nk = a.xa_Nk; k.xa_save = a.xa_save;
  k.xa_q = a.xa_q; k.xa_ldq = a.xa_ldq; k.xa_dq = a.xa_dq; k.xa_lddq = a.xa_lddq;
  if (a.gn_done) *a.gn_done = 0;
  if (a.lnb_done) *a.lnb_done = 0;
  if (a.xa_done) *a.xa_done = 0;
  if (dtype == DH_DTYPE_F16) gemm_dispatch<f16>(k, a.partial_elems, st, a.gn_done, a.lnb_done, a.xa_done, dtype);
  else gemm_dispatch<bf16>(k, a.partial_elems, st, a.gn_done, a.lnb_done, a.xa_done, dtype);
  return 2.0 * (double)a.M * (double)a.N * (double)a.K;
}

}

#ifdef DH_TUNING
extern "C" int dh_dbg_gemm_timeline(unsigned long long* ts) { dh::g_gemm_ts = ts; return DH_OK; }
#endif

extern "C" int dh_dbg_gemm_family(int force) {
  DH_REQUIRE(force >= 0 && force <= 2, "family: 0 policy, 1 k_gemm_dma, 2 k_gemm_pp");
  dh::g_pp_force = force;
  return DH_OK;
}

extern "C" int dh_dbg_gemm_stage(int buf) {
  dh::g_buf_stage = buf;
  return DH_OK;
}

extern "C" int dh_dbg_gemm_last_tile(int* out) {
  DH_REQUIRE(out != nullptr, "null pointer");
  const dh::GemmTileReport& r = dh::g_last_tile;
  const int v[9] = {r.bm, r.bn, r.kg, r.stages, r.mw, r.splits, r.pp, r.gn_epi, r.reduce_gn};
  for (int i = 0; i < 9; ++i) out[i] = v[i];
  return DH_OK;
}

extern "C" int dh_dbg_gemm_xattn_carried(int* last, long long* total) {
  if (last) *last = dh::g_last_xattn;
  if (total) *total = dh::g_xattn_total;
  return DH_OK;
}

extern "C" int dh_gemm_profile_begin(void) {
  dh::g_prof.on = true;
  dh::g_prof.used = 0;
  dh::g_prof.flops = 0;
  dh::g_prof.bytes = 0;
  return DH_OK;
}
extern "C" int dh_gemm_profile_bytes(double* bytes) {
  if (bytes) *bytes = dh::g_prof.bytes;
  return DH_OK;
}
extern "C" int dh_gemm_profile_end(double* ms_total, int64_t* launches, double* flops) {
  using namespace dh;
  g_prof.on = false;
  double ms = 0;
  if (g_prof.used >= 2) DH_CHECK_HIP(hipEventSynchronize(g_prof.ev[g_prof.used - 1]));
  for (size_t i = 0; i + 1 < g_prof.used; i += 2) {
    float t = 0;
    DH_CHECK_HIP(hipEventElapsedTime(&t, g_prof.ev[i], g_prof.ev[i + 1]));
    ms += t;
  }
  if (ms_total) *ms_total = ms;
  if (launches) *launches = (int64_t)(g_prof.used / 2);
  if (flops) *flops = g_prof.flops;
  return DH_OK;
}
```

diffusionhandles_amd/csrc/gemm_k.h:

```cpp
#pragma once
#include "unet_kernels.h"

namespace dh {

typedef _Float16 v8h __attribute__((ext_vector_type(8)));
typedef __bf16 v8b __attribute__((ext_vector_type(8)));
typedef float v16f __attribute__((ext_vector_type(16)));

template <class T> struct Mfma;
template <> struct Mfma<f16> {
  static __device__ __forceinline__ v16f run(uint4 a, uint4 b, v16f c) {
    return __builtin_amdgcn_mfma_f32_32x32x16_f16(__builtin_bit_cast(v8h, a), __builtin_bit_cast(v8h, b), c, 0, 0, 0);
  }
};
template <> struct Mfma<bf16> {
  static __device__ __forceinline__ v16f run(uint4 a, uint4 b, v16f c) {
    return __builtin_amdgcn_mfma_f32_32x32x16_bf16(__builtin_bit_cast(v8b, a), __builtin_bit_cast(v8b, b), c, 0, 0, 0);
  }
};

struct GemmK {
  const void* A; long lda;
  const void* W;
  int M, N, K;
  int mode, Hin, Win, Cin, Hout, Wout, stride, up, pad;
  const float* bias;
  const float* rowvec; int rowvec_ld; int rows_per_batch; float inv_rows_per_batch;
  const void* R; long ldr;
  void* C; long ldc;
  int act_silu;
  int pre_r;
  int wide_store;
#ifdef DH_TUNING
  int w_nt;
  unsigned long long* ts;
  int lnf_abl;
#endif
  const float* ln_s; const float* ln_t; float* ln_stats; float ln_eps;
  float* partial;
  int splits, k_per_split;
  float* gn_part; int gn_HW, gn_G, gn_S;
  int gn_epi, gn_cpg;
  const void* gnb_x; long gnb_ldx; const float *gnb_gamma, *gnb_beta, *gnb_stats; int gnb_silu;
  const void* lnb_x; long lnb_ldx; const float *lnb_gamma, *lnb_stats; const void* lnb_add; void* lnb_dx;
  void* glu_y; long glu_ldy; const void* glub_x; void* glub_dx;
  int glub_f;
  int pp_tm, pp_tn, pp_order, pp_nwork; unsigned pp_a_bytes, pp_w_bytes;
  unsigned long long* pp_ts;
  int xa, xa_Nq, xa_Nk, xa_H, xa_save;
  const void *xa_k, *xa_v; long xa_ldk; void* xa_o; long xa_ldo; float* xa_lse;
  const void* xa_q; long xa_ldq; void* xa_dq; long xa_lddq;
};


__host__ __device__ constexpr bool glub_tile_is_glu(int n0, int glub_f) { return n0 < glub_f; }
__host__ __device__ constexpr bool glub_split_ok(int BN, int glub_f) { return BN > 0 && glub_f % BN == 0; }

constexpr int EPI_XATTN = 3, EPI_XATTN_DQ = 4;
constexpr int XA_KEYS = 96;
__host__ __device__ constexpr bool xattn_epi_tile(int BM, int BN, int WG, int MW, bool BUF) {
  return BN == 64 && (BM == 64 || BM == 128) && WG == 1 && MW == 1 && BUF;
}

struct PpPlan { int bm = 0, bn = 0, splits = 1; };
bool gemm_pp_plan(const GemmK& k, size_t partial_elems, int force, PpPlan* plan);
void launch_gemm_pp(int dtype, const GemmK& k, const PpPlan& plan, hipStream_t st, hipEvent_t e0, hipEvent_t e1);

}
```

diffusionhandles_amd/csrc/unet_engine.cpp:

```cpp
#include <stdlib.h>

#include <algorithm>
#include <map>
#include <numeric>
#include <vector>

#include "unet_kernels.h"

namespace dh {

enum OpType { OP_CONV_IN, OP_CONV_OUT, OP_GEMM, OP_GN, OP_LN, OP_ATTN, OP_GEGLU, OP_CONCAT, OP_TIMESTEP, OP_T2F };
enum ParamKind { PK_F32, PK_MAT };

struct Ten {
  size_t off = 0, goff = 0;
  size_t off_fo = 0;
  int rows = 0, C = 0;
  int ld = 0;
  int view = -1, col = 0;
  bool req_grad = true;
  bool persistent = false;
};

struct Wt {
  size_t fwd_off = 0, bwd_off = 0;
  int N = 0, K = 0, taps = 1;
  bool has_bwd = true, f32 = false;
  int glu_F = 0;
};

struct ParamInfo {
  std::string name;
  int ndim = 0;
  int64_t shape[4] = {0, 0, 0, 0};
  int kind = PK_F32;
  size_t f32_off = 0;
  int wt = -1;
  int row_off = 0;
  int glu_F = 0;
};

struct Op {
  int type = OP_GEMM;
  int in0 = -1, in1 = -1, out = -1, res = -1;
  int wt = -1;
  long bias_off = -1;
  long gamma_off = -1, beta_off = -1;
  int mode = A_DENSE, Hin = 0, Win = 0, Cin = 0, Hout = 0, Wout = 0, stride = 1, up = 0;
  int in_col = 0, in_cols = 0;
  long rowvec_off = -1; int rowvec_ld = 0;
  int act_silu = 0;
  float eps = 1e-5f; int silu = 0; int groups = 32; size_t stats_off = 0;
  int heads = 0, Nq = 0, Nk = 0, cross = 0, kv_col = 0; size_t lse_off = 0;
  int gn_next = -1;
  int ln_fold = -1, folded = 0;
  long ln_s_off = -1, ln_t_off = -1;
  int glu_op = -1, glub_op = -1;
  int xattn_op = -1;
  int xattn_bwd_op = -1;
};

struct FfFold {
  int wt_po = -1, wt_ffo = -1, wt = -1;
  long b_po = -1, b_ffo = -1, bias = -1;
};

}

using namespace dh;

struct dh_unet {
  dh_unet_config cfg;
  int dtype = DH_DTYPE_F16;
  std::vector<Ten> tens;
  std::vector<Wt> wts;
  std::vector<ParamInfo> params;
  std::vector<Op> ops;
  std::vector<FfFold> ffolds;
  std::map<std::string, int> pindex;
  size_t w16_elems = 0, pf_elems = 0, act_elems = 0, grad_elems = 0, f32_elems = 0;
  size_t fo_elems = 0;
// ... 72 lines not shown
  int weight(int N, int K, int taps = 1, bool has_bwd = true, bool f32 = false, bool pad_bwd = false) {
    Wt w;
    w.N = N; w.K = K; w.taps = taps; w.has_bwd = has_bwd; w.f32 = f32;
    size_t& arena = f32 ? u.pf_elems : u.w16_elems;
    w.fwd_off = arena; arena += align_up((size_t)N * K, 128);
    if (has_bwd) { w.bwd_off = arena; arena += align_up((size_t)N * (pad_bwd ? align_up((size_t)K, 128) : (size_t)K), 128); }
    u.wts.push_back(w);
    return (int)u.wts.size() - 1;
  }
  void bind_mat(const std::string& name, int wt, int rows, int row_off, int cin, int taps) {
    ParamInfo p;
    p.name = name; p.kind = PK_MAT; p.wt = wt; p.row_off = row_off;
    if (taps == 9) { p.ndim = 4; p.shape[0] = rows; p.shape[1] = cin; p.shape[2] = 3; p.shape[3] = 3; }
    else { p.ndim = 2; p.shape[0] = rows; p.shape[1] = cin; }
    u.pindex[name] = (int)u.params.size();
    u.params.push_back(p);
  }
  void bind_conv1x1(const std::string& name, int wt, int rows, int cin) {
    bind_mat(name, wt, rows, 0, cin, 1);
    ParamInfo& p = u.params.back();
    p.ndim = 4; p.shape[2] = 1; p.shape[3] = 1;
  }

  int gn(int x, const std::string& pre, float eps, bool silu) {
    const Ten tx = u.tens[x];
    Op o;
    o.type = OP_GN; o.in0 = x; o.out = tensor(tx.rows, tx.C);
    o.gamma_off = param_f32(pre + ".weight", tx.C);
    o.beta_off = param_f32(pre + ".bias", tx.C);
    o.eps = eps; o.silu = silu; o.groups = u.cfg.norm_groups;
    o.stats_off = f32_slot((size_t)maxB * o.groups * 2);
    u.ops.push_back(o);
    return o.out;
  }
  int ln(int x, const std::string& pre) {
    const Ten tx = u.tens[x];
    Op o;
    o.type = OP_LN; o.in0 = x; o.out = tensor(tx.rows, tx.C);
    o.gamma_off = param_f32(pre + ".weight", tx.C);
    o.beta_off = param_f32(pre + ".bias", tx.C);
    o.eps = 1e-5f;
    o.stats_off = f32_slot((size_t)maxB * tx.rows * 2);
    u.ops.push_back(o);
    return o.out;
  }
  int conv3(int x, const std::string& pre, int Cout, int Hs, int stride, int up, long temb_off, int res) {
    const Ten& tx = u.tens[x];
    const int Cin = tx.C;
    const int Hv = Hs << up, Ho = stride == 2 ? Hv / 2 : Hv;
    Op o;
    o.type = OP_GEMM; o.mode = A_CONV3; o.in0 = x; o.res = res;
    o.Hin = Hs; o.Win = Hs; o.Cin = Cin; o.Hout = Ho; o.Wout = Ho; o.stride = stride; o.up = up;
    o.wt = weight(Cout, 9 * Cin, 9);
    bind_mat(pre + ".weight", o.wt, Cout, 0, Cin, 9);
    o.bias_off = param_f32(pre + ".bias", Cout);
    if (temb_off >= 0) { o.rowvec_off = u.temb_f32_off + temb_off; o.rowvec_ld = u.temb_total; }
    o.out = tensor(Ho * Ho, Cout);
    u.ops.push_back(o);
    return o.out;
  }
  int linear_w(int x, int wt, long bias_off, int res, int in_col = 0, int in_cols = 0, bool silu = false,
               bool req_grad = true) {
    const Ten tx = u.tens[x];
    Op o;
    o.type = OP_GEMM; o.mode = A_DENSE; o.in0 = x; o.res = res; o.wt = wt; o.bias_off = bias_off;
    o.in_col = in_col; o.in_cols = in_cols ? in_cols : tx.C; o.act_silu = silu;
    o.out = tensor(tx.rows, u.wts[wt].N, req_grad);
    u.ops.push_back(o);
    return o.out;
  }
  int linear(int x, const std::string& pre, int N, bool bias, int res, bool as_conv1x1 = false) {
    const int K = u.tens[x].C;
    const int wt = weight(N, K);
    if (as_conv1x1) bind_conv1x1(pre + ".weight", wt, N, K); else bind_mat(pre + ".weight", wt, N, 0, K, 1);
    const long b = bias ? param_f32(pre + ".bias", N) : -1;
    return linear_w(x, wt, b, res);
  }
  int concat(int a, int b) {
    Op o;
    o.type = OP_CONCAT; o.in0 = a; o.in1 = b;
    o.out = tensor(u.tens[a].rows, u.tens[a].C + u.tens[b].C);
    u.ops.push_back(o);
    return o.out;
  }

  void fold_ln_into_last_gemm() {
    const int gi = (int)u.ops.size() - 1, li = gi - 1;
    Op& g = u.ops[gi];
    Op& l = u.ops[li];
    if (g.type != OP_GEMM || l.type != OP_LN || g.in0 != l.out || g.mode != A_DENSE || g.in_col != 0) return;
    const int N = u.wts[g.wt].N;
    g.ln_fold = li; l.folded = 1;
    g.ln_s_off = (long)u.pf_elems; u.pf_elems += align_up((size_t)N, 64);
    g.ln_t_off = (long)u.pf_elems; u.pf_elems += align_up((size_t)N, 64);
  }

  int temb_cursor = 0, kv_cursor = 0;
  int wt_temb = -1, wt_kv = -1;
  size_t temb_bias_off = 0;

  int resnet(int x, const std::string& pre, int Cout, int H) {
    const int Cin = u.tens[x].C;
    int h = gn(x, pre + ".norm1", 1e-5f, true);
    bind_mat(pre + ".time_emb_proj.weight", wt_temb, Cout, temb_cursor, u.cfg.block_out_channels[0] * 4, 1);
    param_f32_at(pre + ".time_emb_proj.bias", Cout, temb_bias_off + temb_cursor);
    const long toff = temb_cursor;
// ... 369 lines not shown
  const int n = blockIdx.x;
  float s = 0.f;
  for (int j = threadIdx.x; j < C; j += blockDim.x) s += to_f32<D>(po[(size_t)n * C + j]) * b_ffo[j];
  s = block_sum(s, sm);
  if (threadIdx.x == 0) out[n] = s + b_po[n];
}

static size_t ff_fold_scratch(int C) { return align_up((size_t)C * C, 128) + (size_t)4 * C * C; }

template <class D>
static void fold_ff_t(dh_unet* u, hipStream_t st) {
  for (const FfFold& f : u->ffolds) {
    const Wt& po = u->wts[f.wt_po];
    const Wt& ffo = u->wts[f.wt_ffo];
    const Wt& wf = u->wts[f.wt];
    const int C = po.N;
    D* po_plain = (D*)u->scratch;
    D* prod = po_plain + align_up((size_t)C * C, 128);
    hipLaunchKernelGGL((k_untile<D>), dim3(cdiv(C * C, 256)), dim3(256), 0, st, (const D*)(u->w16 + po.fwd_off), C, C, po_plain);
    GemmArgs g;
    g.A = po_plain; g.lda = C;
    g.W = u->w16 + ffo.bwd_off;
    g.mode = A_DENSE; g.M = C; g.N = 4 * C; g.K = C;
    g.C = prod; g.ldc = 4 * C;
    launch_gemm(u->dtype, g, st);
    hipLaunchKernelGGL((k_pack_ff_fold<D>), dim3(cdiv(5 * C * C, 256)), dim3(256), 0, st, (const D*)prod, (const D*)po_plain, C,
                       (D*)(u->w16 + wf.fwd_off), (D*)(u->w16 + wf.bwd_off));
    hipLaunchKernelGGL((k_fold_ff_bias<D>), dim3(C), dim3(256), 0, st, (const D*)po_plain, C, u->pf + f.b_ffo, u->pf + f.b_po,
                       u->pf + f.bias);
  }
}

static void fold_layernorms(dh_unet* u, hipStream_t st) {
  { int cmax = 0;
    for (const Op& o : u->ops) if (o.type == OP_LN) cmax = std::max(cmax, u->tens[o.in0].C);
    if (cmax > 0) {
      hipLaunchKernelGGL(k_fill_f32, dim3(cdiv(cmax, 256)), dim3(256), 0, st, u->pf + u->ones_off, cmax, 1.f);
      hipLaunchKernelGGL(k_fill_f32, dim3(cdiv(cmax, 256)), dim3(256), 0, st, u->pf + u->zeros_off, cmax, 0.f);
    } }
  for (const Op& g : u->ops) {
    if (g.type != OP_GEMM || g.ln_fold < 0) continue;
    const Op& l = u->ops[g.ln_fold];
    const Wt& w = u->wts[g.wt];
    const float* bias = g.bias_off >= 0 ? u->pf + g.bias_off : nullptr;
    if (u->dtype == DH_DTYPE_F16)
      hipLaunchKernelGGL((k_fold_ln<f16>), dim3(w.N), dim3(256), 0, st, (const f16*)(u->w16 + w.bwd_off), w.N, u->pf + l.gamma_off,
                         u->pf + l.beta_off, bias, (f16*)(u->w16 + w.fwd_off), w.K, u->pf + g.ln_s_off, u->pf + g.ln_t_off);
    else
      hipLaunchKernelGGL((k_fold_ln<bf16>), dim3(w.N), dim3(256), 0, st, (const bf16*)(u->w16 + w.bwd_off), w.N, u->pf + l.gamma_off,
                         u->pf + l.beta_off, bias, (bf16*)(u->w16 + w.fwd_off), w.K, u->pf + g.ln_s_off, u->pf + g.ln_t_off);
  }
  if (u->dtype == DH_DTYPE_F16) fold_ff_t<f16>(u, st);
  else fold_ff_t<bf16>(u, st);
  u->fold_dirty = false;
}

}

static int create_engine(const dh_unet_config* cfg, dh_unet* parent, dh_unet** out);
extern "C" int dh_unet_create(const dh_unet_config* cfg, dh_unet** out) {
  DH_REQUIRE(cfg && out, "null pointer");
  DH_REQUIRE(cfg->n_levels == 4, "n_levels must be 4");
  DH_REQUIRE(cfg->dtype == DH_DTYPE_F16 || cfg->dtype == DH_DTYPE_BF16, "dtype must be f16 or bf16");
  DH_REQUIRE(cfg->max_batch >= 1 && cfg->max_batch < 4096 && cfg->sample_size % 8 == 0 && cfg->sample_size >= 8, "bad batch / sample size");
  DH_REQUIRE((long)cfg->max_batch * cfg->sample_size * cfg->sample_size < (1L << 21), "max_batch * sample_size^2 must stay below 2^21 rows");
  DH_REQUIRE(cfg->norm_groups >= 1 && cfg->norm_groups <= 32, "1..32 GroupNorm groups");
  DH_REQUIRE(cfg->in_channels <= 8 && cfg->out_channels <= 8, "in/out channels must be <= 8");
  DH_REQUIRE(cfg->block_out_channels[0] <= 2048, "block_out_channels[0] must be <= 2048 (few-channel convolutions)");
  DH_REQUIRE(cfg->cross_attention_dim % 64 == 0, "cross_attention_dim must be a multiple of 64");
  for (int i = 0; i < 4; ++i) {
    DH_REQUIRE(cfg->block_out_channels[i] % 64 == 0, "block_out_channels must be multiples of 64");
    DH_REQUIRE(cfg->block_out_channels[i] == cfg->heads[i] * 64, "head dim must be 64");
    DH_REQUIRE(cfg->block_out_channels[i] % cfg->norm_groups == 0, "channels must divide into norm groups");
  }
  return create_engine(cfg, nullptr, out);
}

static int create_engine(const dh_unet_config* cfg, dh_unet* parent, dh_unet** out) {
  dh_unet* u = new dh_unet();
  u->cfg = *cfg;
  if (u->cfg.max_diff_batch <= 0 || u->cfg.max_diff_batch > u->cfg.max_batch) u->cfg.max_diff_batch = u->cfg.max_batch;
  u->dtype = cfg->dtype;
  int rc = build(*u);
  if (rc != DH_OK) { delete u; return rc; }
  auto fail = [&](hipError_t e, const char* what) {
    set_error(std::string(what) + ": " + hipGetErrorString(e));
    dh_unet_destroy(u);
    return DH_ERR_HIP;
  };
  hipError_t e;
  if (parent) {
    if (u->w16_elems != parent->w16_elems || u->pf_elems != parent->pf_elems) {
      set_error("internal: shared engine lays its parameters out differently");
      delete u;
      return DH_ERR_STATE;
    }
    u->owns_weights = false;
    u->w16 = parent->w16; u->pf = parent->pf;
    u->fold_dirty = false;
  } else {
    if ((e = hipMalloc((void**)&u->w16, u->w16_elems * 2 + 256)) != hipSuccess) return fail(e, "hipMalloc weights");
    if ((e = hipMalloc((void**)&u->pf, u->pf_elems * 4 + 256)) != hipSuccess) return fail(e, "hipMalloc f32 params");
  }
  if ((e = hipMalloc((void**)&u->act, u->act_elems * 2 + 256)) != hipSuccess) return fail(e, "hipMalloc activations");
  if ((e = hipMalloc((void**)&u->grad, u->grad_elems * 2 + 256)) != hipSuccess) return fail(e, "hipMalloc gradients");
  if ((e = hipMalloc((void**)&u->f32a, u->f32_elems * 4 + 256)) != hipSuccess) return fail(e, "hipMalloc f32 arena");
// ... 68 lines not shown
  }
  u->temb_rows = 0; u->fold_dirty = true; u->kv_key = 0;
  hipStream_t st = (hipStream_t)stream;
  const ParamInfo& p = u->params[i];
  if (p.kind == PK_F32) {
    if (p.glu_F) {
      hipLaunchKernelGGL(k_load_glu_bias, dim3(cdiv((int)p.shape[0], 256)), dim3(256), 0, st, src, u->pf + p.f32_off, p.glu_F);
      DH_LAUNCH_CHECK();
      return DH_OK;
    }
    DH_CHECK_HIP(hipMemcpyAsync(u->pf + p.f32_off, src, (size_t)p.shape[0] * 4, hipMemcpyDeviceToDevice, st));
    return DH_OK;
  }
  const Wt& w = u->wts[p.wt];
  const int N = (int)p.shape[0], C = (int)p.shape[1], taps = w.taps;
  const size_t total = (size_t)N * C * taps;
  const unsigned nb = (unsigned)((total + 255) / 256);
  const long fwd_ld = w.K;
  const long bwd_ld = (long)taps * w.N;
  if (w.f32) {
    float* f = u->pf + w.fwd_off;
    float* b = w.has_bwd ? u->pf + w.bwd_off : nullptr;
    hipLaunchKernelGGL((k_load_weight<float, false>), dim3(nb), dim3(256), 0, st, src, N, C, taps, f, fwd_ld, (long)p.row_off,
                       b, bwd_ld, (long)p.row_off, w.N);
  } else if (u->dtype == DH_DTYPE_F16) {
    f16* f = (f16*)(u->w16 + w.fwd_off);
    f16* b = w.has_bwd ? (f16*)(u->w16 + w.bwd_off) : nullptr;
    hipLaunchKernelGGL((k_load_weight<f16, true>), dim3(nb), dim3(256), 0, st, src, N, C, taps, f, fwd_ld, (long)p.row_off, b,
                       bwd_ld, (long)p.row_off, w.N, 1.f, w.glu_F);
  } else {
    bf16* f = (bf16*)(u->w16 + w.fwd_off);
    bf16* b = w.has_bwd ? (bf16*)(u->w16 + w.bwd_off) : nullptr;
    hipLaunchKernelGGL((k_load_weight<bf16, true>), dim3(nb), dim3(256), 0, st, src, N, C, taps, f, fwd_ld, (long)p.row_off, b,
                       bwd_ld, (long)p.row_off, w.N, 1.f, w.glu_F);
  }
  DH_LAUNCH_CHECK();
  return DH_OK;
}

extern "C" size_t dh_unet_weight_bytes(const dh_unet* u) { return u && u->owns_weights ? u->w16_elems * 2 + u->pf_elems * 4 : 0; }
extern "C" size_t dh_unet_workspace_bytes(const dh_unet* u) {
  return u ? (u->act_elems + u->grad_elems + u->scratch_elems) * 2 + (u->f32_elems + u->partial_elems + u->small_elems) * 4 : 0;
}

static void fill_gemm(dh_unet* u, const Op& o, int B, GemmArgs& g) {
  const Wt& w = u->wts[o.wt];
  const Ten& ti = u->tens[o.in0];
  const Ten& to = u->tens[o.out];
  g.A = u->aptr(o.in0) + o.in_col; g.lda = ti.ld;
  g.W = u->w16 + w.fwd_off;
  g.M = B * to.rows; g.N = w.N; g.K = w.K;
  g.mode = o.mode; g.Hin = o.Hin; g.Win = o.Win; g.Cin = o.Cin; g.Hout = o.Hout; g.Wout = o.Wout;
  g.stride = o.stride; g.up = o.up;
  g.bias = o.bias_off >= 0 ? u->pf + o.bias_off : nullptr;
  if (o.rowvec_off >= 0) { g.rowvec = u->f32a + o.rowvec_off; g.rowvec_ld = o.rowvec_ld; g.rows_per_batch = to.rows; }
  if (o.res >= 0) { g.R = u->aptr(o.res); g.ldr = u->tens[o.res].ld; }
  g.C = u->aptr(o.out); g.ldc = to.ld;
  g.act_silu = o.act_silu;
  g.partial = u->partial; g.partial_elems = u->partial_elems;
  if (o.ln_fold >= 0) {
    const Op& l = u->ops[o.ln_fold];
    if (use_ln_fold(u, B)) {
      g.A = u->aptr(l.in0); g.lda = u->tens[l.in0].ld;
      g.bias = nullptr;
      g.ln_s = u->pf + o.ln_s_off; g.ln_t = u->pf + o.ln_t_off; g.ln_stats = u->f32a + l.stats_off; g.ln_eps = l.eps;
    } else {
      g.bias = u->pf + o.ln_t_off;
    }
  }
}

static void forward_ops(dh_unet* u, int B, int n_ops, int first_op, bool kv_hit, bool save, hipStream_t st) {
  const int dt = u->dtype;
  const dh_unet_config& c = u->cfg;
  u->flops_fwd = 0;
  int gn_have = 0;
  int xa_have = 0;
  if (!kv_hit) launch_f32_to_t(dt, u->in_text, u->aptr(u->t_text), (size_t)B * c.text_len * c.cross_attention_dim, st);
  for (int oi = first_op; oi < n_ops; ++oi) {
    const Op& o = u->ops[oi];
    if (kv_hit && oi == u->temb_ops) continue;
    switch (o.type) {
      case OP_TIMESTEP:
        launch_timestep_embedding(dt, u->t_dev, c.block_out_channels[0], B, u->aptr(o.out), st);
        break;
      case OP_T2F:
        launch_t_to_f32(dt, u->aptr(o.in0), u->f32a + u->temb_f32_off, (size_t)B * u->temb_total, 0, st);
        break;
      case OP_CONV_IN: {
        const Wt& w = u->wts[o.wt];
        launch_conv_small_fwd(dt, u->in_sample, 1, u->pf + w.fwd_off, u->pf + o.bias_off, u->aptr(o.out), 0, B, o.Hin, o.Hin,
                              o.Cin, w.N, st);
        u->flops_fwd += 2.0 * B * o.Hin * o.Hin * w.N * w.K;
        break;
      }
      case OP_CONV_OUT: {
        const Wt& w = u->wts[o.wt];
        launch_conv_small_fwd(dt, u->aptr(o.in0), 0, u->pf + w.fwd_off, u->pf + o.bias_off, u->io_eps, 1, B, o.Hin, o.Hin,
                              o.Cin, w.N, st);
        u->flops_fwd += 2.0 * B * o.Hin * o.Hin * w.N * w.K;
        break;
      }
      case OP_GEMM: {
        GemmArgs g;
        fill_gemm(u, o, B, g);
        gn_have = 0;
// ... 225 lines not shown
          g.glub_x = u->aptr(ge.in0); g.glub_dx = u->gptr(ge.in0); g.glub_f = u->tens[ge.out].C;
          g.C = u->gptr(t2); g.ldc = u->tens[t2].C;
          if (u->gready[t2]) { g.R = g.C; g.ldr = g.ldc; }
          u->flops_bwd += launch_gemm(dt, g, st);
          u->gready[ge.in0] = 1; u->gready[ge.out] = 1; u->gready[t2] = 1;
          glub_done = o.glub_op;
          break;
        }
        if (!ti.req_grad || !w.has_bwd) break;
        if (o.in0 == u->t_text && !bw.need_text) break;
        GemmArgs g;
        g.A = u->gptr(o.out); g.lda = to.C;
        g.W = u->w16 + w.bwd_off;
        g.partial = u->partial; g.partial_elems = u->partial_elems;
        if (o.mode == A_DENSE) {
          g.mode = A_DENSE;
          g.M = B * to.rows; g.N = w.K; g.K = w.N;
          g.C = u->gptr(o.in0) + o.in_col; g.ldc = ti.C;
          if (u->gready[o.in0]) { g.R = g.C; g.ldr = ti.C; }
          lnb_have = 0;
          if (oi > 0 && u->ops[oi - 1].type == OP_LN && u->ops[oi - 1].out == o.in0 && !u->gready[o.in0] && o.in_col == 0 &&
              w.K == ti.C) {
            const Op& ln = u->ops[oi - 1];
            g.lnb_x = u->aptr(ln.in0); g.lnb_ldx = u->tens[ln.in0].ld; g.lnb_gamma = u->pf + ln.gamma_off; g.lnb_stats = u->f32a + ln.stats_off;
            g.lnb_add = u->gready[ln.in0] ? u->gptr(ln.in0) : nullptr; g.lnb_dx = u->gptr(ln.in0);
            g.lnb_done = &lnb_have;
            lnb_for = oi - 1;
          }
          if (oi > 0 && u->ops[oi - 1].type == OP_GN && u->ops[oi - 1].out == o.in0 && !u->gready[o.in0] && o.in_col == 0 &&
              w.K == ti.C) {
            const Op& gn = u->ops[oi - 1];
            const Ten& tx = u->tens[gn.in0];
            g.gnb_x = u->aptr(gn.in0); g.gnb_ldx = tx.ld;
            g.gnb_gamma = u->pf + gn.gamma_off; g.gnb_beta = u->pf + gn.beta_off; g.gnb_stats = u->f32a + gn.stats_off;
            g.gnb_silu = gn.silu;
            g.gn_part = u->small; g.gn_HW = tx.rows; g.gn_G = gn.groups; g.gn_done = &gnb_have;
            gnb_have = 0;
            gnb_for = oi - 1;
          }
          xb_have = 0;
          if (o.xattn_bwd_op >= 0 && !bw.need_text && !u->gready[o.in0] && o.in0 == u->ops[o.xattn_bwd_op].out) {
            const Op& at = u->ops[o.xattn_bwd_op];
            const unsigned short* kv = u->aptr(at.in1) + at.kv_col;
            const int C = u->tens[at.out].C, ldq = u->tens[at.in0].C;
            g.xa_k = kv; g.xa_v = kv + C; g.xa_ldk = u->tens[at.in1].C; g.xa_o = u->aptr(at.out); g.xa_ldo = C;
            g.xa_lse = u->f32a + at.lse_off; g.xa_H = at.heads; g.xa_Nq = at.Nq; g.xa_Nk = at.Nk;
            g.xa_q = u->aptr(at.in0); g.xa_ldq = ldq; g.xa_dq = u->gptr(at.in0); g.xa_lddq = ldq;
            g.xa_done = &xb_have;
            xb_for = o.xattn_bwd_op;
          }
          u->flops_bwd += launch_gemm(dt, g, st);
          u->gready[o.in0] = 1;
        } else if (o.up) {
          g.mode = A_CONV3; g.stride = 1; g.up = 0;
          g.Hin = o.Hout; g.Win = o.Wout; g.Cin = w.N; g.Hout = o.Hout; g.Wout = o.Wout;
          g.M = B * o.Hout * o.Wout; g.N = o.Cin; g.K = 9 * w.N;
          g.C = u->scratch; g.ldc = o.Cin;
          u->flops_bwd += launch_gemm(dt, g, st);
          launch_pool2x2_sum(dt, u->scratch, u->gptr(o.in0), B, o.Hin, o.Win, o.Cin, u->gready[o.in0] ? 1 : 0, st);
          u->gready[o.in0] = 1;
        } else {
          g.mode = o.stride == 2 ? A_CONVT2 : A_CONV3;
          g.stride = 1; g.up = 0;
          g.Hin = o.Hout; g.Win = o.Wout; g.Cin = w.N;
          g.Hout = o.Hin; g.Wout = o.Win;
          g.M = B * o.Hin * o.Win; g.N = o.Cin; g.K = 9 * w.N;
          g.C = u->gptr(o.in0); g.ldc = ti.C;
          if (u->gready[o.in0]) { g.R = g.C; g.ldr = ti.C; }
          gnb_have = 0;
          int gi = -1;
          if (oi > 0 && u->ops[oi - 1].type == OP_GN && u->ops[oi - 1].out == o.in0) gi = oi - 1;
          else if (oi > 1 && u->ops[oi - 1].type == OP_GEMM && u->ops[oi - 1].mode == A_DENSE && u->ops[oi - 1].out == o.res &&
                   u->ops[oi - 1].in0 != o.in0 && u->ops[oi - 2].type == OP_GN && u->ops[oi - 2].out == o.in0)
            gi = oi - 2;
          if (gi >= 0) {
            const Op& gn = u->ops[gi];
            const Ten& tx = u->tens[gn.in0];
            g.gnb_x = u->aptr(gn.in0); g.gnb_ldx = tx.ld;
            g.gnb_gamma = u->pf + gn.gamma_off; g.gnb_beta = u->pf + gn.beta_off; g.gnb_stats = u->f32a + gn.stats_off;
            g.gnb_silu = gn.silu;
            g.gn_part = u->small; g.gn_HW = tx.rows; g.gn_G = gn.groups; g.gn_done = &gnb_have;
            gnb_for = gi;
          }
          u->flops_bwd += launch_gemm(dt, g, st);
          u->gready[o.in0] = 1;
        }
        if (o.in0 == u->t_text) text_grad_written = true;
        break;
      }
      case OP_GN: {
        if (!u->gready[o.out]) break;
        const Ten& t = u->tens[o.in0];
        GnBwdSplit split;
        if (oi > 0 && u->ops[oi - 1].type == OP_CONCAT && u->ops[oi - 1].out == o.in0) {
          const Op& cat = u->ops[oi - 1];
          const int ca = u->tens[cat.in0].C;
          if (!u->gready[cat.in0] && !u->gready[cat.in1] && ca % 8 == 0 && ca + u->tens[cat.in1].C == t.C) {
            split.out0 = u->gptr(cat.in0); split.out1 = u->gptr(cat.in1); split.split_c = ca;
            cat_done = oi - 1;
          }
        }
        launch_groupnorm_bwd(dt, u->aptr(o.in0), u->gptr(o.out), u->pf + o.gamma_off, u->pf + o.beta_off,
                             u->f32a + o.stats_off, u->gptr(o.in0), u->small, B, t.rows, t.C, o.groups, o.silu,
                             u->gready[o.in0] ? 1 : 0, st, gnb_for == oi ? gnb_have : 0, split);
        gnb_have = 0;
        u->gready[o.in0] = 1;
        if (split.out0) { u->gready[u->ops[oi - 1].in0] = 1; u->gready[u->ops[oi - 1].in1] = 1; }
        break;
      }
      case OP_LN: {
        if (!u->gready[o.out]) break;
        if (lnb_have && lnb_for == oi) {
          lnb_have = 0;
          u->gready[o.in0] = 1;
          break;
// ... 131 lines not shown
  u->text_key = key;
  return DH_OK;
}

extern "C" int dh_unet_stats(const dh_unet* u, double* flops_fwd, double* flops_bwd, int64_t* launches) {
  DH_REQUIRE(u, "null engine");
  if (flops_fwd) *flops_fwd = u->flops_fwd;
  if (flops_bwd) *flops_bwd = u->flops_bwd;
  if (launches) *launches = (int64_t)u->ops.size();
  return DH_OK;
}

extern "C" int dh_dbg_unet_concat_ops(const dh_unet_config* cfg, int* out, int cap, int* n_out) {
  DH_REQUIRE(cfg && n_out && (out || cap == 0), "null pointer");
  dh_unet u;
  u.cfg = *cfg;
  const int rc = build(u);
  if (rc != DH_OK) return rc;
  int n = 0;
  for (size_t i = 0; i < u.ops.size(); ++i) {
    const Op& o = u.ops[i];
    if (o.type != OP_CONCAT) continue;
    const Ten &a = u.tens[o.in0], &b = u.tens[o.in1], &t = u.tens[o.out];
    const int G = o.gn_next >= 0 ? u.ops[o.gn_next].groups : 0;
    const bool fused = o.gn_next >= 0 && i + 1 < u.ops.size() && a.C % 8 == 0 && b.C % 8 == 0 && t.C % G == 0 &&
                       (GN_GB * (t.C / G)) % 8 == 0 && GN_GB * (t.C / G) <= 2048;
    if (n < cap) {
      int* e = out + 5 * n;
      e[0] = a.C; e[1] = b.C; e[2] = t.rows; e[3] = G; e[4] = fused ? 1 : 0;
    }
    ++n;
  }
  *n_out = n;
  return DH_OK;
}

extern "C" int dh_dbg_unet_ff_fold(dh_unet* u, int i, int* n_folds, int* C, void* w, float* bias, void* stream) {
  DH_REQUIRE(u && n_folds && C, "null pointer");
  hipStream_t st = (hipStream_t)stream;
  *n_folds = (int)u->ffolds.size();
  *C = 0;
  if (i < 0 || i >= (int)u->ffolds.size()) return DH_OK;
  if (u->fold_dirty) fold_layernorms(u, st);
  const FfFold& f = u->ffolds[i];
  const Wt& wf = u->wts[f.wt];
  *C = wf.N;
  if (w)
    hipLaunchKernelGGL((k_untile<unsigned short>), dim3(cdiv(wf.N * wf.K, 256)), dim3(256), 0, st,
                       (const unsigned short*)(u->w16 + wf.fwd_off), wf.N, wf.K, (unsigned short*)w);
  if (bias) DH_CHECK_HIP(hipMemcpyAsync(bias, u->pf + f.bias, (size_t)wf.N * 4, hipMemcpyDeviceToDevice, st));
  DH_LAUNCH_CHECK();
  return DH_OK;
}
```

diffusionhandles_amd/csrc/unet_kernels.h:

```cpp
#pragma once
#include "common.h"

namespace dh {

__device__ inline float silu_grad(float z) {
  const float s = 1.f / (1.f + __expf(-z));
  return s * (1.f + z * (1.f - s));
}

struct GeluParts { float Phi, pdf; };
__device__ __forceinline__ GeluParts gelu_parts(float g) {
  const float x = fabsf(g) * 0.70710678118654752f;
  const float t = __builtin_amdgcn_rcpf(fmaf(0.3275911f, x, 1.f));
  const float e = __expf(-x * x);
  const float poly = t * (0.254829592f + t * (-0.284496736f + t * (1.421413741f + t * (-1.453152027f + t * 1.061405429f))));
  const float q = 0.5f * poly * e;
  return {g < 0.f ? q : 1.f - q, e * 0.3989422804014327f};
}
__device__ __forceinline__ float gelu_f(float g) { return g * gelu_parts(g).Phi; }
__device__ __forceinline__ float gelu_grad(float g) { const GeluParts p = gelu_parts(g); return fmaf(g, p.pdf, p.Phi); }
__host__ __device__ inline int glu_col(int o, int gate) { return 32 * (o >> 4) + 16 * gate + (o & 15); }
__host__ __device__ inline int glu_src_row(int n, int F) { return ((n >> 4) & 1) * F + 16 * (n >> 5) + (n & 15); }

enum { A_DENSE = 0, A_CONV3 = 1, A_CONVT2 = 2 };

struct GemmArgs {
  const void* A = nullptr; long lda = 0;
  const void* W = nullptr;
  int M = 0, N = 0, K = 0;
  int mode = A_DENSE;
  int Hin = 0, Win = 0, Cin = 0;
  int Hout = 0, Wout = 0;
  int stride = 1, up = 0;
  int pad = 1;
  const float* bias = nullptr;
  const float* rowvec = nullptr; int rowvec_ld = 0; int rows_per_batch = 1;
  const void* R = nullptr; long ldr = 0;
  void* C = nullptr; long ldc = 0;
  int act_silu = 0;
  float* partial = nullptr; size_t partial_elems = 0;
  float* gn_part = nullptr; int gn_HW = 0, gn_G = 0; int* gn_done = nullptr;
  const void* gnb_x = nullptr; long gnb_ldx = 0; const float *gnb_gamma = nullptr, *gnb_beta = nullptr, *gnb_stats = nullptr;
  int gnb_silu = 0;
  const float* ln_s = nullptr; const float* ln_t = nullptr; float* ln_stats = nullptr; float ln_eps = 1e-5f;
  const void* lnb_x = nullptr; long lnb_ldx = 0; const float *lnb_gamma = nullptr, *lnb_stats = nullptr; const void* lnb_add = nullptr;
  void* lnb_dx = nullptr; int* lnb_done = nullptr;
  void* glu_y = nullptr; long glu_ldy = 0;
  const void* glub_x = nullptr; void* glub_dx = nullptr; int glub_f = 0;
  const void *xa_k = nullptr, *xa_v = nullptr; long xa_ldk = 0; void* xa_o = nullptr; long xa_ldo = 0; float* xa_lse = nullptr;
  int xa_H = 0, xa_Nq = 0, xa_Nk = 0, xa_save = 1; int* xa_done = nullptr;
  const void* xa_q = nullptr; long xa_ldq = 0; void* xa_dq = nullptr; long xa_lddq = 0;
};
void launch_splitk_reduce_ln_bwd(int dtype, const float* partial, int splits, const void* x, const float* gamma,
                                 const float* stats, const void* add, void* dx, int rows, int C, hipStream_t st, long ldx = 0);
double launch_gemm(int dtype, const GemmArgs& a, hipStream_t st);
bool gemm_profiling_on();
void launch_tile_weights(int dtype, const void* src, void* dst, int N, int K, hipStream_t st, int conv_cin = 0);
__host__ __device__ inline size_t wt_index(int n, int k, int K) {
  const int r = n & 63, c = (k & 63) >> 3;
  return ((size_t)(n >> 6) * (K >> 6) + (k >> 6)) * 4096 + (size_t)r * 64 + (size_t)((c ^ ((r >> 1) & 7)) << 3) + (k & 7);
}

__host__ __device__ inline int conv_k_index(int tap, int c) { return (c >> 6) * 576 + tap * 64 + (c & 63); }

void launch_load_weight(int dtype, const float* src, int N, int C, int taps, void* fwd, long fwd_K, long row_off, void* bwd,
                        long bwd_K, long col_off, int Nb, float scale, hipStream_t st);

void launch_conv_small_fwd(int dtype, const void* x, int x_is_f32, const float* w, const float* bias, void* y,
                           int y_is_f32, int B, int H, int W, int Cin, int Cout, hipStream_t st);
void launch_conv_small_bwd(int dtype, const void* dy, int dy_is_f32, const float* w, void* dx, int dx_is_f32,
                           int accumulate, int B, int H, int W, int Cin, int Cout, hipStream_t st);

void launch_groupnorm_fwd(int dtype, const void* x, const float* gamma, const float* beta, void* y, float* stats,
                          float* scratch, int B, int HW, int C, int G, float eps, int silu, hipStream_t st,
                          int have_partials = 0);
int gn_slices(int HW, int B);
constexpr int GN_GB = 4;
void launch_concat_gn(int dtype, const void* a, int Ca, const void* b, int Cb, void* out, float* gn_part, int B, int HW,
                      int G, hipStream_t st);
struct GnBwdSplit { void* out0 = nullptr; void* out1 = nullptr; int split_c = 0; };
void launch_groupnorm_bwd(int dtype, const void* x, const void* dy, const float* gamma, const float* beta,
                          const float* stats, void* dx, float* scratch, int B, int HW, int C, int G, int silu,
                          int accumulate, hipStream_t st, int have_partials = 0, GnBwdSplit split = GnBwdSplit());
void launch_gelu(int dtype, const void* x, void* y, size_t n, hipStream_t st);
void launch_layernorm_fwd(int dtype, const void* x, const float* gamma, const float* beta, void* y, float* stats,
                          int rows, int C, float eps, hipStream_t st, long ldx = 0);
void launch_layernorm_bwd(int dtype, const void* x, const void* dy, const float* gamma, const float* stats,
                          const void* add, void* dx, int rows, int C, hipStream_t st, long ldx = 0);
void launch_geglu_fwd(int dtype, const void* x, void* y, int rows, int F, hipStream_t st);
void launch_geglu_bwd(int dtype, const void* x, const void* dy, void* dx, int rows, int F, hipStream_t st);
void launch_copy_cols(int dtype, const void* src, long lds, void* dst, long ldd, int rows, int cols, int accumulate,
                      hipStream_t st);
void launch_split_cols(int dtype, const void* src, long lds, void* dstA, long ldA, int colsA, int accA, void* dstB, long ldB,
                       int colsB, int accB, int rows, hipStream_t st);
void launch_lane_ops_probe(const float* in, float* out, unsigned* ex, hipStream_t st);
void launch_pool2x2_sum(int dtype, const void* src, void* dst, int B, int h, int w, int C, int accumulate,
                        hipStream_t st);
void launch_f32_to_t(int dtype, const float* src, void* dst, size_t n, hipStream_t st);
void launch_t_to_f32(int dtype, const void* src, float* dst, size_t n, int accumulate, hipStream_t st);
void launch_timestep_embedding(int dtype, const float* t_dev, int dim, int B, void* out, hipStream_t st);
void launch_set_scalar(float* p, float v, hipStream_t st);

void launch_attention_fwd(int dtype, const void* q, long ldq, const void* k, const void* v, long ldk, void* o,
                          long ldo, float* lse, int B, int H, int Nq, int Nk, hipStream_t st, int causal = 0);
void launch_attention_delta(int dtype, const void* o, long ldo, const void* d_o, long lddo, float* delta, int B,
                            int H, int Nq, hipStream_t st);
void launch_attention_bwd_dq(int dtype, const void* q, long ldq, const void* k, const void* v, long ldk, const void* o,
                             long ldo, const void* d_o, long lddo, const float* lse, float* delta, void* dq, long lddq,
                             int B, int H, int Nq, int Nk, hipStream_t st);
void launch_attention_bwd_dkv(int dtype, const void* q, long ldq, const void* k, const void* v, long ldk,
                              const void* d_o, long lddo, const float* lse, const float* delta, void* dk, void* dv,
                              long lddk, int B, int H, int Nq, int Nk, hipStream_t st, float* scratch = nullptr,
                              size_t scratch_elems = 0);

}
```

diffusionhandles_amd/csrc/vae_engine.cpp:

```cpp
#include <algorithm>
#include <string>
#include <vector>

#include "unet_kernels.h"

namespace dh {

template <class T>
__global__ void k_tile_rows(const T* src, long ld, int col0, T* dst, int N, int K, int transpose) {
  const size_t idx = (size_t)blockIdx.x * blockDim.x + threadIdx.x;
  if (idx >= (size_t)N * K) return;
  int n, k;
  if (transpose) { k = (int)(idx / N); n = (int)(idx - (size_t)k * N); }
  else { n = (int)(idx / K); k = (int)(idx - (size_t)n * K); }
  dst[wt_index(n, k, K)] = transpose ? src[(size_t)k * ld + col0 + n] : src[(size_t)n * ld + col0 + k];
}

template <class T>
__global__ void __launch_bounds__(256) k_softmax_rows(T* s, int rows, int cols) {
  const int row = blockIdx.x * 4 + (threadIdx.x >> 6), lane = threadIdx.x & 63;
  if (row >= rows) return;
  T* p = s + (size_t)row * cols;
  float mx = -INFINITY;
  for (int c = lane * 8; c < cols; c += 512) {
    const uint4 raw = *reinterpret_cast<const uint4*>(p + c);
    const T* v = reinterpret_cast<const T*>(&raw);
#pragma unroll
    for (int i = 0; i < 8; ++i) mx = fmaxf(mx, to_f32<T>(v[i]));
  }
  mx = wave_max(mx);
  float sum = 0.f;
  for (int c = lane * 8; c < cols; c += 512) {
    const uint4 raw = *reinterpret_cast<const uint4*>(p + c);
    const T* v = reinterpret_cast<const T*>(&raw);
#pragma unroll
    for (int i = 0; i < 8; ++i) sum += __expf(to_f32<T>(v[i]) - mx);
  }
  sum = wave_sum(sum);
  const float inv = 1.f / sum;
  for (int c = lane * 8; c < cols; c += 512) {
    uint4 raw = *reinterpret_cast<const uint4*>(p + c);
    T* v = reinterpret_cast<T*>(&raw);
#pragma unroll
    for (int i = 0; i < 8; ++i) v[i] = from_f32<T>(__expf(to_f32<T>(v[i]) - mx) * inv);
    *reinterpret_cast<uint4*>(p + c) = raw;
  }
}

enum VOp { V_CONV_IN, V_CONV_OUT, V_CONV, V_LINEAR, V_GN, V_ATTN };

struct VTen { size_t off; int H, C; };
struct VWt { size_t off; int N, K, taps; bool f32; };
struct VParam { std::string name; int ndim; int64_t shape[4]; int wt; int row_off; long f32_off; float scale; };
struct VOpRec {
  int type = 0, in0 = -1, out = -1, res = -1, wt = -1;
  long bias = -1, gamma = -1, beta = -1;
  int Hin = 0, Cin = 0, Hout = 0, up = 0, silu = 0, stride = 1, pad = 1;
  float eps = 1e-6f;
  size_t stats = 0;
};

}
using namespace dh;

struct dh_vae_decoder {
  dh_vae_config cfg;
  int dtype = DH_DTYPE_F16;
  std::vector<VTen> tens;
  std::vector<VWt> wts;
  std::vector<VParam> params;
  std::vector<VOpRec> ops;
  size_t w16_elems = 0, pf_elems = 0, act_elems = 0, f32_elems = 0, small_elems = 0, scores_elems = 0, tiled_elems = 0;
  unsigned short *w16 = nullptr, *act = nullptr, *scores = nullptr, *tiled = nullptr;
  float *pf = nullptr, *f32a = nullptr, *small = nullptr, *partial = nullptr;
  size_t partial_elems = 0;
  int t_out = -1;
  bool encoder = false;
};

namespace {
struct VB {
  dh_vae_decoder& v;
  explicit VB(dh_vae_decoder& d) : v(d) {}
  int tensor(int H, int C) {
    VTen t{v.act_elems, H, C};
    v.act_elems += align_up((size_t)H * H * C, 128);
    v.tens.push_back(t);
    return (int)v.tens.size() - 1;
  }
  long pf32(const std::string& name, int n, float scale = 1.f) {
    VParam p{name, 1, {n, 0, 0, 0}, -1, 0, (long)v.pf_elems, scale};
    v.pf_elems += align_up((size_t)n, 64);
    v.params.push_back(p);
    return p.f32_off;
  }
  void pf32_at(const std::string& name, int n, long off, float scale) {
    VParam p{name, 1, {n, 0, 0, 0}, -1, 0, off, scale};
    v.params.push_back(p);
  }
  int weight(int N, int K, int taps, bool f32) {
    VWt w{f32 ? v.pf_elems : v.w16_elems, N, K, taps, f32};
    (f32 ? v.pf_elems : v.w16_elems) += align_up((size_t)N * K, 128);
    v.wts.push_back(w);
    return (int)v.wts.size() - 1;
  }
  void bind(const std::string& name, int wt, int rows, int row_off, int cin, int taps, float scale = 1.f) {
    VParam p{name, taps == 9 ? 4 : 2, {rows, cin, taps == 9 ? 3 : 0, taps == 9 ? 3 : 0}, wt, row_off, -1, scale};
    v.params.push_back(p);
  }
  void bind1x1(const std::string& name, int wt, int rows, int cin) {
    VParam p{name, 4, {rows, cin, 1, 1}, wt, 0, -1, 1.f};
    v.params.push_back(p);
  }
  int gn(int x, const std::string& pre, bool silu) {
    const VTen t = v.tens[x];
    VOpRec o;
    o.type = V_GN; o.in0 = x; o.out = tensor(t.H, t.C); o.silu = silu;
    o.gamma = pf32(pre + ".weight", t.C); o.beta = pf32(pre + ".bias", t.C);
    o.stats = v.f32_elems; v.f32_elems += 64 * 2;
    v.ops.push_back(o);
    return o.out;
  }
  int conv3(int x, const std::string& pre, int Cout, int up, int res, int stride = 1, int pad = 1) {
    const VTen t = v.tens[x];
    VOpRec o;
    o.type = V_CONV; o.in0 = x; o.res = res; o.Hin = t.H; o.Cin = t.C; o.up = up; o.stride = stride; o.pad = pad;
    o.Hout = stride == 2 ? t.H / 2 : t.H << up;
    o.wt = weight(Cout, 9 * t.C, 9, false);
    bind(pre + ".weight", o.wt, Cout, 0, t.C, 9);
    o.bias = pf32(pre + ".bias", Cout);
    o.out = tensor(o.Hout, Cout);
    v.ops.push_back(o);
    return o.out;
  }
  int resnet(int x, const std::string& pre, int Cout) {
    const int Cin = v.tens[x].C;
    int h = gn(x, pre + ".norm1", true);
    h = conv3(h, pre + ".conv1", Cout, 0, -1);
    h = gn(h, pre + ".norm2", true);
    int sc = x;
    if (Cin != Cout) {
      VOpRec o;
      o.type = V_LINEAR; o.in0 = x; o.wt = weight(Cout, Cin, 1, false);
      bind1x1(pre + ".conv_shortcut.weight", o.wt, Cout, Cin);
      o.bias = pf32(pre + ".conv_shortcut.bias", Cout);
      o.out = tensor(v.tens[x].H, Cout);
      v.ops.push_back(o);
      sc = o.out;
    }
    return conv3(h, pre + ".conv2", Cout, 0, sc);
  }
  int attention(int x, const std::string& pre) {
    const int Ctop = v.tens[x].C, S = v.tens[x].H;
    int t = gn(x, pre + ".group_norm", false);
    VOpRec q;
    q.type = V_LINEAR; q.in0 = t; q.wt = weight(3 * Ctop, Ctop, 1, false);
    const float sc = 1.f / sqrtf((float)Ctop);
    bind(pre + ".to_q.weight", q.wt, Ctop, 0, Ctop, 1, sc);
    bind(pre + ".to_k.weight", q.wt, Ctop, Ctop, Ctop, 1);
    bind(pre + ".to_v.weight", q.wt, Ctop, 2 * Ctop, Ctop, 1);
    q.bias = (long)v.pf_elems; v.pf_elems += align_up((size_t)3 * Ctop, 64);
    pf32_at(pre + ".to_q.bias", Ctop, q.bias, sc);
    pf32_at(pre + ".to_k.bias", Ctop, q.bias + Ctop, 1.f);
    pf32_at(pre + ".to_v.bias", Ctop, q.bias + 2 * Ctop, 1.f);
    q.out = tensor(S, 3 * Ctop);
    v.ops.push_back(q);
    VOpRec a;
    a.type = V_ATTN; a.in0 = q.out; a.out = tensor(S, Ctop);
    v.ops.push_back(a);
    VOpRec o;
    o.type = V_LINEAR; o.in0 = a.out; o.res = x; o.wt = weight(Ctop, Ctop, 1, false);
    bind(pre + ".to_out.0.weight", o.wt, Ctop, 0, Ctop, 1);
    o.bias = pf32(pre + ".to_out.0.bias", Ctop);
    o.out = tensor(S, Ctop);
    v.ops.push_back(o);
    v.scores_elems = (size_t)S * S * S * S;
    v.tiled_elems = (size_t)S * S * Ctop;
    return o.out;
  }
};

// ... 142 lines not shown
  if ((e = hipMalloc((void**)&v->w16, v->w16_elems * 2 + 256)) != hipSuccess) return fail(e, "hipMalloc weights");
  if ((e = hipMalloc((void**)&v->pf, v->pf_elems * 4 + 256)) != hipSuccess) return fail(e, "hipMalloc f32 params");
  if ((e = hipMalloc((void**)&v->act, v->act_elems * 2 + 256)) != hipSuccess) return fail(e, "hipMalloc activations");
  if ((e = hipMalloc((void**)&v->scores, v->scores_elems * 2 + 256)) != hipSuccess) return fail(e, "hipMalloc attention scores");
  if ((e = hipMalloc((void**)&v->tiled, v->tiled_elems * 2 + 256)) != hipSuccess) return fail(e, "hipMalloc tiled operand");
  if ((e = hipMalloc((void**)&v->f32a, v->f32_elems * 4 + 256)) != hipSuccess) return fail(e, "hipMalloc statistics");
  if ((e = hipMalloc((void**)&v->small, v->small_elems * 4)) != hipSuccess) return fail(e, "hipMalloc scratch");
  if ((e = hipMalloc((void**)&v->partial, v->partial_elems * 4)) != hipSuccess) return fail(e, "hipMalloc split-K");
  (void)hipMemset(v->w16, 0, v->w16_elems * 2);
  (void)hipMemset(v->pf, 0, v->pf_elems * 4);
  *out = v;
  return DH_OK;
}

extern "C" int dh_vae_decoder_create(const dh_vae_config* cfg, dh_vae_decoder** out) { return vae_create(cfg, out, false); }
extern "C" int dh_vae_encoder_create(const dh_vae_config* cfg, dh_vae_decoder** out) {
  DH_REQUIRE(cfg && 2 * cfg->latent_channels <= 8, "the moments (2 * latent_channels) must fit the few-output convolution (<= 8)");
  return vae_create(cfg, out, true);
}

extern "C" void dh_vae_decoder_destroy(dh_vae_decoder* v) {
  if (!v) return;
  (void)hipFree(v->w16); (void)hipFree(v->pf); (void)hipFree(v->act); (void)hipFree(v->scores); (void)hipFree(v->tiled);
  (void)hipFree(v->f32a); (void)hipFree(v->small); (void)hipFree(v->partial);
  delete v;
}

extern "C" int dh_vae_decoder_num_params(const dh_vae_decoder* v) { return v ? (int)v->params.size() : 0; }

extern "C" int dh_vae_decoder_param_info(const dh_vae_decoder* v, int i, const char** name, int* ndim, int64_t* shape4) {
  DH_REQUIRE(v && i >= 0 && i < (int)v->params.size() && name && ndim && shape4, "bad arguments");
  const VParam& p = v->params[i];
  *name = p.name.c_str();
  *ndim = p.ndim;
  for (int k = 0; k < 4; ++k) shape4[k] = p.shape[k];
  return DH_OK;
}

__global__ void k_scale_copy(const float* src, float* dst, int n, float s) {
  const int i = blockIdx.x * blockDim.x + threadIdx.x;
  if (i < n) dst[i] = src[i] * s;
}

extern "C" int dh_vae_decoder_load_param(dh_vae_decoder* v, int i, const float* src, void* stream) {
  DH_REQUIRE(v && src && i >= 0 && i < (int)v->params.size(), "bad arguments");
  hipStream_t st = (hipStream_t)stream;
  const VParam& p = v->params[i];
  if (p.wt < 0) {
    hipLaunchKernelGGL(k_scale_copy, dim3(cdiv((int)p.shape[0], 256)), dim3(256), 0, st, src, v->pf + p.f32_off, (int)p.shape[0], p.scale);
    DH_LAUNCH_CHECK();
    return DH_OK;
  }
  const VWt& w = v->wts[p.wt];
  void* dst = w.f32 ? (void*)(v->pf + w.off) : (void*)(v->w16 + w.off);
  launch_load_weight(w.f32 ? DH_DTYPE_F32 : v->dtype, src, (int)p.shape[0], (int)p.shape[1], w.taps, dst, w.K, p.row_off, nullptr, 0, 0, w.N,
                     p.scale, st);
  DH_LAUNCH_CHECK();
  return DH_OK;
}

extern "C" size_t dh_vae_decoder_bytes(const dh_vae_decoder* v) {
  return v ? (v->w16_elems + v->act_elems + v->scores_elems + v->tiled_elems) * 2 + (v->pf_elems + v->f32_elems + v->small_elems + v->partial_elems) * 4 : 0;
}

static int vae_run(dh_vae_decoder* v, const float* z, int batch, float* image, void* stream) {
  hipStream_t st = (hipStream_t)stream;
  const int dt = v->dtype;
  const dh_vae_config& c = v->cfg;
  const int S = c.latent_size, R = 8 * S;
  const size_t in_elems = v->encoder ? (size_t)R * R * c.out_channels : (size_t)S * S * c.latent_channels;
  const size_t out_elems = v->encoder ? (size_t)S * S * 2 * c.latent_channels : (size_t)R * R * c.out_channels;
  auto aptr = [&](int t) { return v->act + v->tens[t].off; };
  for (int b = 0; b < batch; ++b) {
    const float* zb = z + (size_t)b * in_elems;
    float* ib = image + (size_t)b * out_elems;
    for (const VOpRec& o : v->ops) {
      switch (o.type) {
        case V_CONV_IN: {
          const VWt& w = v->wts[o.wt];
          launch_conv_small_fwd(dt, zb, 1, v->pf + w.off, v->pf + o.bias, aptr(o.out), 0, 1, o.Hin, o.Hin, o.Cin, w.N, st);
          break;
        }
        case V_CONV_OUT: {
          const VWt& w = v->wts[o.wt];
          launch_conv_small_fwd(dt, aptr(o.in0), 0, v->pf + w.off, v->pf + o.bias, ib, 1, 1, o.Hin, o.Hin, o.Cin, w.N, st);
          break;
        }
        case V_CONV: case V_LINEAR: {
          const VWt& w = v->wts[o.wt];
          const VTen &ti = v->tens[o.in0], &to = v->tens[o.out];
          GemmArgs g;
          g.A = aptr(o.in0); g.lda = ti.C; g.W = v->w16 + w.off;
          g.M = to.H * to.H; g.N = w.N; g.K = w.K;
          if (o.type == V_CONV) {
            g.mode = A_CONV3; g.Hin = o.Hin; g.Win = o.Hin; g.Cin = o.Cin; g.Hout = o.Hout; g.Wout = o.Hout; g.stride = o.stride; g.up = o.up;
            g.pad = o.pad;
          }
          g.bias = v->pf + o.bias;
          if (o.res >= 0) { g.R = aptr(o.res); g.ldr = v->tens[o.res].C; }
          g.C = aptr(o.out); g.ldc = to.C;
          g.partial = v->partial; g.partial_elems = v->partial_elems;
          launch_gemm(dt, g, st);
          break;
        }
        case V_GN: {
          const VTen& t = v->tens[o.in0];
          launch_groupnorm_fwd(dt, aptr(o.in0), v->pf + o.gamma, v->pf + o.beta, aptr(o.out), v->f32a + o.stats, v->small, 1, t.H * t.H,
                               t.C, c.norm_groups, o.eps, o.silu, st, 0);
          break;
        }
        case V_ATTN: {
          const VTen& t = v->tens[o.in0];
          const int N = t.H * t.H, C = t.C / 3;
          const unsigned short* qkv = aptr(o.in0);
          const unsigned nb = (unsigned)(((size_t)N * C + 255) / 256);
          hipLaunchKernelGGL((k_tile_rows<unsigned short>), dim3(nb), dim3(256), 0, st, qkv, (long)t.C, C, v->tiled, N, C, 0);
          GemmArgs g;
          g.A = qkv; g.lda = t.C; g.W = v->tiled; g.M = N; g.N = N; g.K = C; g.C = v->scores; g.ldc = N;
          launch_gemm(dt, g, st);
          if (dt == DH_DTYPE_F16) hipLaunchKernelGGL((k_softmax_rows<f16>), dim3(cdiv(N, 4)), dim3(256), 0, st, (f16*)v->scores, N, N);
          else hipLaunchKernelGGL((k_softmax_rows<bf16>), dim3(cdiv(N, 4)), dim3(256), 0, st, (bf16*)v->scores, N, N);
          hipLaunchKernelGGL((k_tile_rows<unsigned short>), dim3(nb), dim3(256), 0, st, qkv, (long)t.C, 2 * C, v->tiled, C, N, 1);
          GemmArgs h;
          h.A = v->scores; h.lda = N; h.W = v->tiled; h.M = N; h.N = C; h.K = N; h.C = aptr(o.out); h.ldc = C;
          h.partial = v->partial; h.partial_elems = v->partial_elems;
          launch_gemm(dt, h, st);
          break;
        }
      }
    }
  }
  DH_LAUNCH_CHECK();
  return DH_OK;
}

extern "C" int dh_vae_decoder_decode(dh_vae_decoder* v, const float* z, int batch, float* image, void* stream) {
  DH_REQUIRE(v && z && image && batch >= 1, "bad arguments");
  DH_REQUIRE(!v->encoder, "this handle is an encoder (dh_vae_encoder_create)");
  return vae_run(v, z, batch, image, stream);
}

extern "C" int dh_vae_encoder_encode(dh_vae_decoder* v, const float* image, int batch, float* moments, void* stream) {
  DH_REQUIRE(v && image && moments && batch >= 1, "bad arguments");
  DH_REQUIRE(v->encoder, "this handle is a decoder (dh_vae_decoder_create)");
  return vae_run(v, image, batch, moments, stream);
}
```

Baseline: 38.00 steps/s.

## Use sub-pixel decomposition for upsample convs and their input gradients

Nearest-2x upsample followed by a 3x3 conv is rewritten as four 2x2 phase convolutions over the low-resolution input. Their weights are pre-summed into sub-pixel tiles, and the GEMM epilogue scatters each output row to its interleaved position. The backward pass of the upsample conv becomes a 16-tap gather over the high-resolution gradient (A_UPT4), and stride-2 transposed backward gets derived 2x2 weights. This removes the redundant taps that read duplicated upsampled pixels, at the cost of extra derived weight storage, precompute at fold time, and new GEMM modes.

Measured after the change: 38.36 steps/s, median of 6. Within noise of the previous version (+0.9%).

```diff
diff --git a/diffusionhandles_amd/_lib.py b/diffusionhandles_amd/_lib.py
--- a/diffusionhandles_amd/_lib.py
+++ b/diffusionhandles_amd/_lib.py
@@ -150,6 +150,14 @@
                                 ctypes.POINTER(c_i), c_p]),
     "dh_dbg_gemm_xattn_dq": (c_i, [c_i, c_p, c_l, c_p, c_i, c_i, c_i, c_p, c_p, c_p, c_p, c_l, c_p, c_p, c_p, c_i, c_i, ctypes.POINTER(c_i), c_p]),
     "dh_dbg_gemm_xattn_carried": (c_i, [ctypes.POINTER(c_i), ctypes.POINTER(ctypes.c_longlong)]),
+    "dh_dbg_gemm_subpixel_carried": (c_i, [ctypes.POINTER(c_i)]),
+    "dh_dbg_gemm_force_splits": (c_i, [c_i]),
+    "dh_dbg_gemm_subpixel_counts": (c_i, [ctypes.POINTER(ctypes.c_longlong)]),
+    "dh_dbg_gemm_subpixel": (c_i, [c_i]),
+    "dh_dbg_subpixel_conv": (c_i, [c_i, c_p, c_l, c_p, c_i, c_i, c_i, c_i, c_i, c_p, c_p, c_l, c_p, c_l, c_p, c_sz, c_p, c_p]),
+    "dh_dbg_subpixel_conv_bwd": (c_i, [c_i, c_p, c_l, c_p, c_i, c_i, c_i, c_i, c_i, c_p, c_l, c_i, c_p, c_sz, ctypes.POINTER(c_i), c_p, c_p]),
+    "dh_dbg_t2_conv_bwd": (c_i, [c_i, c_p, c_l, c_p, c_i, c_i, c_i, c_i, c_i, c_p, c_l, c_i, c_p, c_sz, c_p, c_p]),
+    "dh_dbg_unet_subpixel_weights": (c_i, [c_p, c_i, ctypes.POINTER(c_i), ctypes.POINTER(c_i), ctypes.POINTER(c_i), c_p, c_p, c_p]),
     "dh_dbg_gemm_pp_variant": (c_i, [c_i, c_p]),
     "dh_dbg_gemm_pp_ablate": (c_i, [c_i]),
     "dh_dbg_gemm_pp_persist": (c_i, [c_i]),
diff --git a/diffusionhandles_amd/csrc/debug_api.cpp b/diffusionhandles_amd/csrc/debug_api.cpp
--- a/diffusionhandles_amd/csrc/debug_api.cpp
+++ b/diffusionhandles_amd/csrc/debug_api.cpp
@@ -309,3 +309,83 @@
   DH_LAUNCH_CHECK();
   return DH_OK;
 }
+
+struct Prepared {
+  void* buf = nullptr; size_t cap = 0;
+  const void* w = nullptr; int n = 0, c = 0, dtype = -1;
+};
+template <class Derive>
+static int prepared(Prepared& p, int dtype, const void* W, int N, int C, hipStream_t st, Derive derive, unsigned short** t9, unsigned short** td) {
+  const size_t e9 = (size_t)N * 9 * C, ed = (size_t)16 * N * C;
+  if ((e9 + ed) * 2 > p.cap) {
+    if (p.buf) (void)hipFree(p.buf);
+    p.buf = nullptr; p.cap = 0; p.w = nullptr;
+    DH_CHECK_HIP(hipMalloc(&p.buf, (e9 + ed) * 2));
+    p.cap = (e9 + ed) * 2;
+  }
+  *t9 = (unsigned short*)p.buf;
+  *td = *t9 + e9;
+  static const bool pretiled = getenv("DH_DBG_PRETILED") != nullptr;
+  if (!pretiled || p.w != W || p.n != N || p.c != C || p.dtype != dtype) {
+    launch_tile_weights(dtype, W, *t9, N, 9 * C, st, C);
+    derive(*t9, *td);
+  }
+  p.w = W; p.n = N; p.c = C; p.dtype = dtype;
+  return DH_OK;
+}
+
+extern "C" int dh_dbg_subpixel_conv(int dtype, const void* x, long lda, const void* W, int B, int H, int Wd, int Cin, int N, const float* bias,
+                                    const void* R, long ldr, void* C, long ldc, float* partial, size_t partial_elems, void* w_sub, void* stream) {
+  DH_REQUIRE(x && W && C && Cin % 64 == 0 && N % 64 == 0 && B > 0 && H > 0 && Wd > 0, "bad arguments (N, Cin must be multiples of 64)");
+  hipStream_t st = (hipStream_t)stream;
+  static Prepared prep;
+  unsigned short *t9, *t4;
+  int rc = prepared(prep, dtype, W, N, Cin, st, [&](unsigned short* a, unsigned short* b) { launch_subpixel_weights(dtype, a, N, Cin, b, st); }, &t9, &t4);
+  if (rc != DH_OK) return rc;
+  if (w_sub) launch_untile_subpixel(t4, N, Cin, w_sub, st);
+  GemmArgs g;
+  g.A = x; g.lda = lda; g.W = t9; g.W_sub = t4; g.M = B * 4 * H * Wd; g.N = N; g.K = 9 * Cin; g.mode = A_CONV3;
+  g.Hin = H; g.Win = Wd; g.Cin = Cin; g.Hout = 2 * H; g.Wout = 2 * Wd; g.stride = 1; g.up = 1; g.bias = bias;
+  g.R = R; g.ldr = ldr; g.C = C; g.ldc = ldc; g.partial = partial; g.partial_elems = partial_elems;
+  launch_gemm(dtype, g, st);
+  DH_LAUNCH_CHECK();
+  return DH_OK;
+}
+
+extern "C" int dh_dbg_subpixel_conv_bwd(int dtype, const void* dy, long ldy, const void* W, int B, int H, int Wd, int Cin, int N, void* dx, long lddx,
+                                        int accumulate, float* partial, size_t partial_elems, int* carried, void* w_upb, void* stream) {
+  DH_REQUIRE(dy && W && dx && carried && Cin % 64 == 0 && N % 64 == 0 && B > 0 && H > 0 && Wd > 0, "bad arguments (N, Cin must be multiples of 64)");
+  hipStream_t st = (hipStream_t)stream;
+  static Prepared prep;
+  unsigned short *t9, *t16;
+  int rc = prepared(prep, dtype, W, N, Cin, st, [&](unsigned short* a, unsigned short* b) { launch_upb_weights(dtype, a, N, Cin, b, st); }, &t9, &t16);
+  if (rc != DH_OK) return rc;
+  if (w_upb) launch_untile_upb(t16, N, Cin, w_upb, st);
+  GemmArgs g;
+  g.A = dy; g.lda = ldy; g.W = t16; g.M = B * H * Wd; g.N = Cin; g.K = 16 * N; g.mode = A_UPT4;
+  g.Hin = 2 * H; g.Win = 2 * Wd; g.Cin = N; g.Hout = H; g.Wout = Wd;
+  g.C = dx; g.ldc = lddx; if (accumulate) { g.R = dx; g.ldr = lddx; }
+  g.partial = partial; g.partial_elems = partial_elems;
+  *carried = launch_gemm(dtype, g, st) >= 0 ? 1 : 0;
+  DH_LAUNCH_CHECK();
+  return DH_OK;
+}
+
+extern "C" int dh_dbg_t2_conv_bwd(int dtype, const void* dy, long ldy, const void* Wb, int B, int H, int Wd, int C, int N, void* dx, long lddx,
+                                  int accumulate, float* partial, size_t partial_elems, void* w_t2, void* stream) {
+  DH_REQUIRE(dy && Wb && dx && C % 64 == 0 && N % 64 == 0 && B > 0 && H > 0 && Wd > 0, "bad arguments (N, C must be multiples of 64)");
+  hipStream_t st = (hipStream_t)stream;
+  static Prepared prep;
+  unsigned short *t9, *t4;
+  int rc = prepared(prep, dtype, Wb, N, C, st, [&](unsigned short* a, unsigned short* b) { launch_t2_weights(a, N, C, b, st); }, &t9, &t4);
+  if (rc != DH_OK) return rc;
+  if (w_t2) launch_untile_subpixel(t4, N, C, w_t2, st);
+  GemmArgs g;
+  g.A = dy; g.lda = ldy; g.W = t9; g.W_sub = t4; g.M = B * 4 * H * Wd; g.N = N; g.K = 9 * C; g.mode = A_CONVT2;
+  g.Hin = H; g.Win = Wd; g.Cin = C; g.Hout = 2 * H; g.Wout = 2 * Wd; g.stride = 1; g.up = 0;
+  g.C = dx; g.ldc = lddx; if (accumulate) { g.R = dx; g.ldr = lddx; }
+  g.partial = partial; g.partial_elems = partial_elems;
+  launch_gemm(dtype, g, st);
+  DH_LAUNCH_CHECK();
+  return DH_OK;
+}
diff --git a/diffusionhandles_amd/csrc/gemm.hip b/diffusionhandles_amd/csrc/gemm.hip
--- a/diffusionhandles_amd/csrc/gemm.hip
+++ b/diffusionhandles_amd/csrc/gemm.hip
@@ -19,12 +19,16 @@
 };
 static GemmProf g_prof;
 static int g_buf_stage = 1;
+static int g_sub_force = 0;
+static int g_force_splits = 0;
 static int g_pp_force = 0;
 struct GemmTileReport {
   int bm, bn, kg, stages, mw, splits, pp, gn_epi, reduce_gn;
+  int sub;
 };
 static thread_local GemmTileReport g_last_tile;
 static thread_local int g_last_xattn = 0;
+static thread_local long long g_sub_total[3] = {0, 0, 0};
 static thread_local long long g_xattn_total = 0;
 #ifdef DH_TUNING
 static unsigned long long* g_gemm_ts = nullptr;
@@ -115,7 +119,7 @@
 
 template <int N> __device__ __forceinline__ void wait_vmcnt() { asm volatile("s_waitcnt vmcnt(%0)" ::"n"(N) : "memory"); }
 
-enum { GM_DENSE = 0, GM_CONV_S1 = 1, GM_GENERIC = 2 };
+enum { GM_DENSE = 0, GM_CONV_S1 = 1, GM_GENERIC = 2, GM_CONV_SUB = 3, GM_CONV_UPB = 4 };
 #ifdef DH_TUNING
 #define LNF_ABL(bit) && !(p.lnf_abl & (bit))
 #define LEAN_ABL && !(p.lnf_abl & 8)
@@ -165,6 +169,11 @@
 template <class T, int BM, int BN, int ST, int MODE, int ABL = 0, int WG = 1, int KG = 1, int MW = 1, bool LNF = false, int GLU = 0, bool BUF = false>
 __global__ void __launch_bounds__(256 * WG * KG * MW) k_gemm_dma(const GemmK p) {
   static_assert(!BUF || MODE != GM_GENERIC, "the generic gather stages through addresses");
+  static_assert(MODE != GM_CONV_SUB || (BUF && !LNF && GLU == 0), "the sub-pixel form stages through descriptors and carries the plain epilogue");
+  static_assert(MODE != GM_CONV_UPB || (BUF && !LNF && GLU == 0), "the up-sampler's input gradient stages through descriptors and carries the plain epilogue");
+  constexpr bool SUB = MODE == GM_CONV_SUB, UPB = MODE == GM_CONV_UPB;
+  constexpr bool WIN = MODE == GM_CONV_S1 || SUB || UPB;
+  constexpr int TAPS = SUB ? 4 : (UPB ? 16 : 9), TW = SUB ? 2 : (UPB ? 4 : 3);
   static_assert((WG == 1) + (KG == 1) + (MW == 1) >= 2, "one kind of wave grouping per instantiation");
   static_assert(!LNF || (WG == 1 && MODE == GM_DENSE), "the folded LayerNorm needs every k-step of a row in one wave group");
   DH_STAMP(0);
@@ -197,6 +206,8 @@
     ntiles = ntiles < 0 ? 0 : (ntiles > loop_tiles ? loop_tiles : ntiles);
   }
   const T* Ag = reinterpret_cast<const T*>(p.A);
+  const int sub_ph = SUB ? __builtin_amdgcn_readfirstlane(m0 / p.sub_mlow) : 0;
+  const int sub_m0 = SUB ? sub_ph * p.sub_mlow : 0, sub_a = sub_ph >> 1, sub_b = sub_ph & 1;
   const int wave_s = __builtin_amdgcn_readfirstlane(wave);
   const unsigned lds0 = (unsigned)(size_t)((__attribute__((address_space(3))) unsigned char*)smem_all) + kg * (ST * STAGE);
   const int prow = lane >> 3;
@@ -216,8 +227,8 @@
       a_off[j] = (long)(a_ok[j] ? m : p.M - 1) * p.lda + lchunk * 8;
       a_oy[j] = a_ox[j] = 0;
     } else {
-      const int hw = p.Hout * p.Wout;
-      const int b = div_small(m, inv_hw), r = m - b * hw;
+      const int hw = p.Hout * p.Wout, ml = m - sub_m0;
+      const int b = div_small(ml, inv_hw), r = ml - b * hw;
       a_oy[j] = div_small(r, inv_w);
       a_ox[j] = r - a_oy[j] * p.Wout;
       if (MODE == GM_CONV_S1) a_off[j] = (((long)b * p.Hin + a_oy[j]) * p.Win + a_ox[j]) * p.lda + lchunk * 8;
@@ -233,6 +244,16 @@
       for (int t = 0; t < 9; ++t)
         if ((unsigned)(a_oy[j] + t / 3 - 1) < (unsigned)p.Hin && (unsigned)(a_ox[j] + t % 3 - 1) < (unsigned)p.Win) a_taps[j] |= 1u << t;
     }
+    if (SUB && a_ok[j]) {
+#pragma unroll
+      for (int t = 0; t < 4; ++t)
+        if ((unsigned)(a_oy[j] + sub_a - 1 + (t >> 1)) < (unsigned)p.Hin && (unsigned)(a_ox[j] + sub_b - 1 + (t & 1)) < (unsigned)p.Win) a_taps[j] |= 1u << t;
+    }
+    if (UPB && a_ok[j]) {
+#pragma unroll
+      for (int t = 0; t < 16; ++t)
+        if ((unsigned)(2 * a_oy[j] - 1 + (t >> 2)) < (unsigned)p.Hin && (unsigned)(2 * a_ox[j] - 1 + (t & 3)) < (unsigned)p.Win) a_taps[j] |= 1u << t;
+    }
   }
   const T* Wg = reinterpret_cast<const T*>(p.W);
   const int KT = p.K >> 6;
@@ -243,7 +264,7 @@
     b_ptr[j] = Wg + ((size_t)((n0 + row) >> 6) * KT) * 4096 + (size_t)((n0 + row) & 63) * 64 + lane * 8;
   }
   int tap = 0, c0 = 0;
-  if (MODE != GM_DENSE) { const int kt0 = kbeg >> 6, ch = kt0 / 9; tap = kt0 - ch * 9; c0 = ch * BK; }
+  if (MODE != GM_DENSE) { const int kt0 = kbeg >> 6, ch = kt0 / TAPS; tap = kt0 - ch * TAPS; c0 = ch * BK; }
   typedef int bv4i __attribute__((ext_vector_type(4)));
   bv4i ra = {0, 0, 0, 0}, rw = {0, 0, 0, 0};
   unsigned bv_a[NPA], bv_nt[NPA], bs_w[NPB];
@@ -251,7 +272,7 @@
   unsigned bs_step_px = 0, bs_step_row = 0; int bs_kx = 0;
   const unsigned bv_w = lane * 16;
   if constexpr (BUF) {
-    const unsigned a_bias = MODE == GM_CONV_S1 ? (unsigned)((p.Win + 1) * (int)p.lda * 2) : 0u;
+    const unsigned a_bias = WIN ? (unsigned)((p.Win + 1) * (int)p.lda * 2) : 0u;
     const size_t a_base = (size_t)p.A - a_bias;
     ra[0] = (int)(unsigned)a_base; ra[1] = (int)((a_base >> 32) & 0xffff); ra[2] = (int)(p.pp_a_bytes + a_bias); ra[3] = 0x00020000;
     rw[0] = (int)(unsigned)(size_t)p.W; rw[1] = (int)(((size_t)p.W >> 32) & 0xffff); rw[2] = (int)p.pp_w_bytes; rw[3] = 0x00020000;
@@ -262,10 +283,9 @@
         bv_a[j] = a_ok[j] ? (unsigned)m * (unsigned)((int)p.lda * 2) + (unsigned)lchunk * 16u : 0x80000000u;
         bv_nt[j] = 0;
       } else {
-        const int hw = p.Hout * p.Wout;
-        const int b = div_small(m, inv_hw);
-        (void)hw;
-        bv_a[j] = (unsigned)((b * p.Hin + a_oy[j]) * p.Win + a_ox[j]) * (unsigned)((int)p.lda * 2) + (unsigned)lchunk * 16u;
+        const int b = div_small(m - sub_m0, inv_hw);
+        const int sy = UPB ? 2 * a_oy[j] : a_oy[j], sx = UPB ? 2 * a_ox[j] : a_ox[j];
+        bv_a[j] = (unsigned)((b * p.Hin + sy) * p.Win + sx) * (unsigned)((int)p.lda * 2) + (unsigned)lchunk * 16u;
         bv_nt[j] = ~a_taps[j];
       }
     }
@@ -273,14 +293,15 @@
     for (int j = 0; j < NPB; ++j) {
       const int n = n0 + 8 * (wave_s + NWV * (j * WG + grp));
       bs_w[j] = (unsigned)(((n >> 6) * KT) * 8192 + (n & 63) * 128);
-    }
-    if (MODE == GM_CONV_S1) {
-      const int ky = tap / 3, kx = tap - ky * 3;
-      bs_tap = (unsigned)((ky * p.Win + kx) * (int)p.lda + c0) * 2u;
+      if (SUB) bs_w[j] += (unsigned)sub_ph * (unsigned)(((p.N + 63) >> 6) * KT) * 8192u;
+    }
+    if (WIN) {
+      const int ky = tap / TW, kx = tap - ky * TW;
+      bs_tap = (unsigned)(((ky + sub_a) * p.Win + kx + sub_b) * (int)p.lda + c0) * 2u;
       bs_sh = 31u - (unsigned)tap;
       bs_kx = kx;
       bs_step_px = (unsigned)((int)p.lda * 2);
-      bs_step_row = (unsigned)((p.Win - 2) * (int)p.lda * 2);
+      bs_step_row = (unsigned)((p.Win - (TW - 1)) * (int)p.lda * 2);
     }
   }
 
@@ -338,21 +359,30 @@
     }
   };
   auto next_tile = [&]() {
-    if constexpr (BUF && MODE == GM_CONV_S1) {
+    if constexpr (BUF && WIN) {
       ++tap; ++bs_kx;
-      const bool row_end = bs_kx == 3;
+      const bool row_end = bs_kx == TW;
       bs_tap += row_end ? bs_step_row : bs_step_px;
       bs_kx = row_end ? 0 : bs_kx;
-      if (tap == 9) { tap = 0; c0 += BK; bs_tap = (unsigned)c0 * 2u; }
+      if (tap == TAPS) { tap = 0; c0 += BK; bs_tap = (unsigned)((sub_a * p.Win + sub_b) * (int)p.lda + c0) * 2u; }
       bs_sh = 31u - (unsigned)tap;
       return;
     }
-    if (MODE != GM_DENSE) { if (++tap == 9) { tap = 0; c0 += BK; } }
+    if (MODE != GM_DENSE) { if (++tap == TAPS) { tap = 0; c0 += BK; } }
   };
   auto issue = [&](int kt, int stage) {
 #pragma unroll
     for (int q = 0; q < NP; ++q) issue_piece(kt, stage, q);
     next_tile();
+  };
+
+  auto out_row = [&](int m) -> int {
+    if constexpr (SUB) {
+      const int hw = p.Hout * p.Wout, ml = m - sub_m0;
+      const int b = div_small(ml, inv_hw), r = ml - b * hw, oy = div_small(r, inv_w), ox = r - oy * p.Wout;
+      return (b * 2 * p.Hout + 2 * oy + sub_a) * 2 * p.Wout + 2 * ox + sub_b;
+    }
+    return m;
   };
 
   v16f acc[TM][TN];
@@ -422,7 +452,7 @@
 #pragma unroll
         for (int g = 0; g < 4; ++g) {
           const int n = n0 + wn * CPW + j * 32 + 8 * g + 4 * hi;
-          rpre[i][j][g] = (m < p.M && n < p.N) ? *reinterpret_cast<const uint2*>(rsrc + (size_t)m * rld + n) : make_uint2(0, 0);
+          rpre[i][j][g] = (m < p.M && n < p.N) ? *reinterpret_cast<const uint2*>(rsrc + (size_t)out_row(m) * rld + n) : make_uint2(0, 0);
         }
     }
   }
@@ -1010,7 +1040,7 @@
     for (int i = 0; i < TM; ++i) {
       const int m = m0 + wm * RPW + i * 32 + ln;
       if (m >= p.M) continue;
-      T* orow = reinterpret_cast<T*>(p.C) + (size_t)m * p.ldc + n0 + wn * CPW + 8 * hi;
+      T* orow = reinterpret_cast<T*>(p.C) + (size_t)out_row(m) * p.ldc + n0 + wn * CPW + 8 * hi;
 #pragma unroll
       for (int j = 0; j < TN; ++j) {
         if (n0 + wn * CPW + j * 32 >= p.N) continue;
@@ -1050,6 +1080,7 @@
     for (int i = 0; i < TM; ++i) {
       const int m = m0 + wm * RPW + i * 32 + ln;
       if (m >= p.M) continue;
+      const int mo = out_row(m);
 #pragma unroll
       for (int j = 0; j < TN; ++j) {
         const int nb = n0 + wn * CPW + j * 32;
@@ -1057,12 +1088,12 @@
         uint2 w[4];
 #pragma unroll
         for (int g = 0; g < 4; ++g) {
-          w[g] = epilogue_pack<T>(p, m, nb + 8 * g + 4 * hi, acc[i][j][4 * g], acc[i][j][4 * g + 1], acc[i][j][4 * g + 2],
+          w[g] = epilogue_pack<T>(p, mo, nb + 8 * g + 4 * hi, acc[i][j][4 * g], acc[i][j][4 * g + 1], acc[i][j][4 * g + 2],
                                   acc[i][j][4 * g + 3], pre_r, rpre[i][j][g], pre_b, bpre[PRE_B ? j : 0][g]);
           if (gn_epi) gn_acc(i, j, g, w[g]);
         }
         const uint4 ca = half_exchange(w[0], w[1]), cb = half_exchange(w[2], w[3]);
-        T* out = reinterpret_cast<T*>(p.C) + (size_t)m * p.ldc + nb + 8 * hi;
+        T* out = reinterpret_cast<T*>(p.C) + (size_t)mo * p.ldc + nb + 8 * hi;
         *reinterpret_cast<uint4*>(out) = ca;
         *reinterpret_cast<uint4*>(out + 16) = cb;
       }
@@ -1089,7 +1120,7 @@
           float4 o = make_float4(acc[i][j][4 * g], acc[i][j][4 * g + 1], acc[i][j][4 * g + 2], acc[i][j][4 * g + 3]);
           *reinterpret_cast<float4*>(p.partial + ((size_t)blockIdx.z * p.M + m) * p.N + n) = o;
         } else {
-          epilogue_store<T>(p, m, n, acc[i][j][4 * g], acc[i][j][4 * g + 1], acc[i][j][4 * g + 2], acc[i][j][4 * g + 3], pre_r,
+          epilogue_store<T>(p, out_row(m), n, acc[i][j][4 * g], acc[i][j][4 * g + 1], acc[i][j][4 * g + 2], acc[i][j][4 * g + 3], pre_r,
                             rpre[i][j][g], pre_b, bpre[PRE_B ? j : 0][g]);
         }
       }
@@ -1111,12 +1142,107 @@
 }
 
 template <class T>
+__global__ void k_subpixel_weights(const T* w9, int N, int Cin, T* out) {
+  const size_t idx = (size_t)blockIdx.x * blockDim.x + threadIdx.x;
+  const int K4 = 4 * Cin;
+  const size_t per = (size_t)N * K4;
+  if (idx >= 4 * per) return;
+  const int ph = (int)(idx / per);
+  const size_t r = idx - (size_t)ph * per;
+  const int n = (int)(r / K4), k = (int)(r - (size_t)n * K4), t = k / Cin, c = k - t * Cin;
+  const int a = ph >> 1, b = ph & 1, ty = t >> 1, tx = t & 1;
+  double s = 0.0;
+  for (int ky = sub_tap_lo(a, ty); ky < sub_tap_hi(a, ty); ++ky)
+    for (int kx = sub_tap_lo(b, tx); kx < sub_tap_hi(b, tx); ++kx)
+      s += (double)to_f32<T>(w9[wt_index(n, conv_k_index(ky * 3 + kx, c), 9 * Cin)]);
+  float f = (float)s;
+  if ((double)f != s) {
+    unsigned u = __float_as_uint(f);
+    if (fabs((double)f) > fabs(s)) --u;
+    f = __uint_as_float(u | 1u);
+  }
+  out[(size_t)ph * per + wt_index(n, sub_k_index(t, c), K4)] = from_f32<T>(f);
+}
+void launch_subpixel_weights(int dtype, const void* w9, int N, int Cin, void* out, hipStream_t st) {
+  const unsigned nb = (unsigned)(((size_t)16 * N * Cin + 255) / 256);
+  if (dtype == DH_DTYPE_F16) hipLaunchKernelGGL((k_subpixel_weights<f16>), dim3(nb), dim3(256), 0, st, (const f16*)w9, N, Cin, (f16*)out);
+  else hipLaunchKernelGGL((k_subpixel_weights<bf16>), dim3(nb), dim3(256), 0, st, (const bf16*)w9, N, Cin, (bf16*)out);
+}
+__host__ __device__ inline int upb_tap_lo(int u) { return u == 0 ? 2 : (u == 1 ? 1 : 0); }
+__host__ __device__ inline int upb_tap_hi(int u) { return u <= 1 ? 3 : (u == 2 ? 2 : 1); }
+template <class T>
+__global__ void k_upb_weights(const T* w9, int N, int Cin, T* out) {
+  const size_t idx = (size_t)blockIdx.x * blockDim.x + threadIdx.x;
+  const int K16 = 16 * N;
+  if (idx >= (size_t)Cin * K16) return;
+  const int ci = (int)(idx / K16), k = (int)(idx - (size_t)ci * K16), t = k / N, co = k - t * N;
+  double s = 0.0;
+  for (int ky = upb_tap_lo(t >> 2); ky < upb_tap_hi(t >> 2); ++ky)
+    for (int kx = upb_tap_lo(t & 3); kx < upb_tap_hi(t & 3); ++kx)
+      s += (double)to_f32<T>(w9[wt_index(co, conv_k_index(ky * 3 + kx, ci), 9 * Cin)]);
+  float f = (float)s;
+  if ((double)f != s) {
+    unsigned u = __float_as_uint(f);
+    if (fabs((double)f) > fabs(s)) --u;
+    f = __uint_as_float(u | 1u);
+  }
+  out[wt_index(ci, upb_k_index(t, co), K16)] = from_f32<T>(f);
+}
+void launch_upb_weights(int dtype, const void* w9, int N, int Cin, void* out, hipStream_t st) {
+  const unsigned nb = (unsigned)(((size_t)16 * N * Cin + 255) / 256);
+  if (dtype == DH_DTYPE_F16) hipLaunchKernelGGL((k_upb_weights<f16>), dim3(nb), dim3(256), 0, st, (const f16*)w9, N, Cin, (f16*)out);
+  else hipLaunchKernelGGL((k_upb_weights<bf16>), dim3(nb), dim3(256), 0, st, (const bf16*)w9, N, Cin, (bf16*)out);
+}
+__host__ __device__ inline int t2_tap(int a, int t) { return a == 0 ? (t == 0 ? -1 : 1) : (t == 0 ? 0 : 2); }
+__global__ void k_t2_weights(const unsigned short* wb, int N, int C, unsigned short* out) {
+  const size_t idx = (size_t)blockIdx.x * blockDim.x + threadIdx.x;
+  const int K4 = 4 * C;
+  const size_t per = (size_t)N * K4;
+  if (idx >= 4 * per) return;
+  const int ph = (int)(idx / per);
+  const size_t r = idx - (size_t)ph * per;
+  const int n = (int)(r / K4), k = (int)(r - (size_t)n * K4), t = k / C, c = k - t * C;
+  const int ky = t2_tap(ph >> 1, t >> 1), kx = t2_tap(ph & 1, t & 1);
+  out[(size_t)ph * per + wt_index(n, sub_k_index(t, c), K4)] = (ky < 0 || kx < 0) ? (unsigned short)0 : wb[wt_index(n, conv_k_index(ky * 3 + kx, c), 9 * C)];
+}
+void launch_t2_weights(const void* wb, int N, int C, void* out, hipStream_t st) {
+  const unsigned nb = (unsigned)(((size_t)16 * N * C + 255) / 256);
+  hipLaunchKernelGGL(k_t2_weights, dim3(nb), dim3(256), 0, st, (const unsigned short*)wb, N, C, (unsigned short*)out);
+}
+__global__ void k_untile_upb(const unsigned short* tiled, int N, int Cin, unsigned short* plain) {
+  const size_t idx = (size_t)blockIdx.x * blockDim.x + threadIdx.x;
+  const int K16 = 16 * N;
+  if (idx >= (size_t)Cin * K16) return;
+  const int ci = (int)(idx / K16), k = (int)(idx - (size_t)ci * K16), t = k / N, co = k - t * N;
+  plain[idx] = tiled[wt_index(ci, upb_k_index(t, co), K16)];
+}
+void launch_untile_upb(const void* tiled, int N, int Cin, void* plain, hipStream_t st) {
+  const unsigned nb = (unsigned)(((size_t)16 * N * Cin + 255) / 256);
+  hipLaunchKernelGGL(k_untile_upb, dim3(nb), dim3(256), 0, st, (const unsigned short*)tiled, N, Cin, (unsigned short*)plain);
+}
+__global__ void k_untile_subpixel(const unsigned short* tiled, int N, int Cin, unsigned short* plain) {
+  const size_t idx = (size_t)blockIdx.x * blockDim.x + threadIdx.x;
+  const int K4 = 4 * Cin;
+  const size_t per = (size_t)N * K4;
+  if (idx >= 4 * per) return;
+  const int ph = (int)(idx / per);
+  const size_t r = idx - (size_t)ph * per;
+  const int n = (int)(r / K4), k = (int)(r - (size_t)n * K4), t = k / Cin, c = k - t * Cin;
+  plain[idx] = tiled[(size_t)ph * per + wt_index(n, sub_k_index(t, c), K4)];
+}
+void launch_untile_subpixel(const void* tiled, int N, int Cin, void* plain, hipStream_t st) {
+  const unsigned nb = (unsigned)(((size_t)16 * N * Cin + 255) / 256);
+  hipLaunchKernelGGL(k_untile_subpixel, dim3(nb), dim3(256), 0, st, (const unsigned short*)tiled, N, Cin, (unsigned short*)plain);
+}
+
+template <class T>
 __global__ void k_splitk_reduce(const GemmK p) {
   const size_t q = (size_t)blockIdx.x * blockDim.x + threadIdx.x;
   const size_t total = (size_t)p.M * p.N / 4;
   if (q >= total) return;
   const size_t e = q * 4;
-  const int m = (int)((unsigned)e / (unsigned)p.N), n = (int)((unsigned)e - (unsigned)m * (unsigned)p.N);
+  const int ms = (int)((unsigned)e / (unsigned)p.N), n = (int)((unsigned)e - (unsigned)ms * (unsigned)p.N);
+  const int m = p.sub ? sub_out_row(p, ms) : ms;
   const bool have_r = p.R != nullptr, have_b = p.bias != nullptr;
   const uint2 rpre = have_r ? *reinterpret_cast<const uint2*>(reinterpret_cast<const T*>(p.R) + (size_t)m * p.ldr + n) : make_uint2(0, 0);
   const float4 bpre = have_b ? *reinterpret_cast<const float4*>(p.bias + n) : make_float4(0.f, 0.f, 0.f, 0.f);
@@ -1302,6 +1428,15 @@
     if (g_prof.e0) hipExtLaunchKernelGGL(KERNEL, grid, dim3(TH), 0, st, g_prof.e0, g_prof.e1, 0, k);        \
     else hipLaunchKernelGGL(KERNEL, grid, dim3(TH), 0, st, k);                                              \
   } while (0)
+constexpr bool sub_tile(int BM, int BN, int ST, int WG, int KG, int MW) {
+  return WG == 1 && ((KG == 1 && ((BM == 256 && BN == 128 && ST == 3 && MW == 2) || (BM == 128 && BN == 128 && ST == 4 && MW == 2) ||
+                                  (BM == 128 && BN == 160 && ST == 4 && MW == 1) || (BM == 64 && BN == 64 && ST == 4 && MW == 1))) ||
+                     (MW == 1 && BM == 128 && BN == 64 && (ST == 3 || ST == 5) && KG <= 2));
+}
+constexpr bool upb_tile(int BM, int BN, int ST, int WG, int KG, int MW) {
+  return WG == 1 && ((MW == 1 && BM == 128 && BN == 64 && (ST == 3 || ST == 5) && KG <= 2) || (MW == 1 && BM == 64 && BN == 64 && ST == 4 && KG == 1) ||
+                     (MW == 2 && KG == 1 && BN == 128 && ((BM == 256 && ST == 3) || (BM == 128 && ST == 4))));
+}
 template <class T, int BM, int BN, int ST, int WG, int KG, int MW, bool BUF>
 static void launch_tile_b(int gm, bool lnf, dim3 grid, hipStream_t st, const GemmK& k, int glu) {
   constexpr int TH = 256 * WG * KG * MW;
@@ -1323,6 +1458,12 @@
     DH_GEMM_LAUNCH((k_gemm_dma<T, BM, BN, ST, GM_DENSE, 0, WG, KG, MW, false, 0, BUF>));
   } else if (gm == GM_CONV_S1) {
     DH_GEMM_LAUNCH((k_gemm_dma<T, BM, BN, ST, GM_CONV_S1, 0, WG, KG, MW, false, 0, BUF>));
+  } else if (gm == GM_CONV_SUB) {
+    if constexpr (BUF && sub_tile(BM, BN, ST, WG, KG, MW)) DH_GEMM_LAUNCH((k_gemm_dma<T, BM, BN, ST, GM_CONV_SUB, 0, WG, KG, MW, false, 0, BUF>));
+    else { fprintf(stderr, "gemm: no sub-pixel instantiation of tile %dx%d (stages %d, K groups %d, waves x%d, buffer staging %d)\n", BM, BN, ST, KG, MW, (int)BUF); abort(); }
+  } else if (gm == GM_CONV_UPB) {
+    if constexpr (BUF && upb_tile(BM, BN, ST, WG, KG, MW)) DH_GEMM_LAUNCH((k_gemm_dma<T, BM, BN, ST, GM_CONV_UPB, 0, WG, KG, MW, false, 0, BUF>));
+    else { fprintf(stderr, "gemm: no 4x4 input-gradient instantiation of tile %dx%d (stages %d, K groups %d, waves x%d, buffer staging %d)\n", BM, BN, ST, KG, MW, (int)BUF); abort(); }
   } else {
     DH_GEMM_LAUNCH((k_gemm_dma<T, BM, BN, ST, GM_GENERIC, 0, WG, KG, MW>));
   }
@@ -1342,7 +1483,22 @@
 #endif
 
 template <class T>
-static void gemm_dispatch(GemmK k, size_t partial_elems, hipStream_t st, int* gn_done, int* lnb_done, int* xa_done, int dtype) {
+static int gemm_dispatch(GemmK k, size_t partial_elems, hipStream_t st, int* gn_done, int* lnb_done, int* xa_done, int dtype, const void* w_sub) {
+  DH_KNOB(kSubMinRows, "DH_SUB_MIN_ROWS", 128);
+  DH_KNOB(kUpbMinRows, "DH_UPB_MIN_ROWS", 256);
+  DH_KNOB(kT2MinRows, "DH_T2_MIN_ROWS", 2048);
+  const GemmK k9 = k;
+  const int sub_mlow = k.M / 4;
+  const bool sub_up = k.mode == A_CONV3 && k.stride == 1 && k.up == 1 && k.pad == 1 && (g_buf_stage & 64) == 0;
+  const bool sub_t2 = k.mode == A_CONVT2 && (g_buf_stage & 256) == 0;
+  const bool sub = w_sub != nullptr && (g_buf_stage & 1) && (sub_up || sub_t2) &&
+                   k.Cin % 64 == 0 && k.K == 9 * k.Cin && k.Hout == 2 * k.Hin && k.Wout == 2 * k.Win && k.M % (4 * k.Hin * k.Win) == 0 &&
+                   (sub_mlow >= (sub_t2 ? kT2MinRows : kSubMinRows) || g_sub_force == 2) && !k.ln_s && !k.glu_y && !k.glub_x && !k.xa_o && !k.lnb_x;
+  if (sub) {
+    k.W = w_sub; k.K = 4 * k.Cin; k.Hout = k.Hin; k.Wout = k.Win; k.up = 0; k.mode = A_CONV3;
+    k.sub = 1; k.sub_mlow = sub_mlow;
+    k.gn_part = nullptr;
+  }
   DH_KNOB(kSplitTiles, "DH_SPLITK_TILES", 200);
   DH_KNOB(kSplitMinK, "DH_SPLITK_MINKT", 32);
   DH_KNOB(kSplitTarget, "DH_SPLITK_TARGET", 256);
@@ -1362,7 +1518,11 @@
   int BM = 128, BN = (k.N % 128 == 0) ? 128 : 64;
   const int ktiles = k.K / BK;
   PpPlan pp;
-  const bool use_pp = gemm_pp_plan(k, partial_elems, g_pp_force, &pp);
+  const bool upb = k.mode == A_UPT4;
+  if (upb && ((g_buf_stage & 128) || !(g_buf_stage & 1) || k.Cin % 64 != 0 || k.K != 16 * k.Cin || k.Hin != 2 * k.Hout || k.Win != 2 * k.Wout ||
+              (k.M < kUpbMinRows && g_sub_force != 2)))
+    return -1;
+  const bool use_pp = !sub && !upb && gemm_pp_plan(k, partial_elems, g_pp_force, &pp);
   if (BN == 128 && ktiles >= 16 && cdiv(k.M, 128) * cdiv(k.N, 128) <= kNarrowTiles) BN = 64;
   if (k.M <= 64 || (cdiv(k.M, 128) * cdiv(k.N, BN) < kBigTiles && ktiles < kSplitMinK)) { BM = 64; BN = 64; }
   const bool n320 = kN320 > 0 && k.N % 320 == 0 && k.N <= 960 && !lnf && BM == 128 && BN == 64 && cdiv(k.M, 128) >= kN320;
@@ -1391,6 +1551,13 @@
     if ((size_t)splits > fit) splits = (int)fit;
     if (splits < 1) splits = 1;
   }
+  if (g_force_splits > 0 && !use_pp && k.partial && !lnf && !glu) {
+    splits = g_force_splits;
+    if (splits > ktiles) splits = ktiles;
+    const size_t fit = partial_elems / ((size_t)k.M * k.N);
+    if ((size_t)splits > fit) splits = (int)fit;
+    if (splits < 1) splits = 1;
+  }
 #ifdef DH_TUNING
   static const int kLog = getenv("DH_GEMM_LOG") ? atoi(getenv("DH_GEMM_LOG")) : 0;
   const int kForceTile = getenv("DH_FORCE_TILE") ? atoi(getenv("DH_FORCE_TILE")) : 0;
@@ -1439,16 +1606,19 @@
   dim3 grid(tm, tn, splits);
 #endif
   int gm = GM_GENERIC;
-  if (k.mode == A_DENSE) gm = GM_DENSE;
+  if (sub) gm = GM_CONV_SUB;
+  else if (upb) gm = GM_CONV_UPB;
+  else if (k.mode == A_DENSE) gm = GM_DENSE;
   else if (k.mode == A_CONV3 && k.stride == 1 && k.up == 0 && k.pad == 1) gm = GM_CONV_S1;
   if (!use_pp) {
     k.pp_a_bytes = 0; k.pp_w_bytes = 0;
     size_t ab = 0;
     if (k.mode == A_DENSE) ab = ((size_t)(k.M - 1) * k.lda + k.K) * 2;
+    else if (sub) ab = (size_t)(sub_mlow / (k.Hin * k.Win)) * k.Hin * k.Win * (size_t)k.lda * 2;
     else if (k.Hout > 0 && k.Wout > 0 && k.M % (k.Hout * k.Wout) == 0)
       ab = (size_t)(k.M / (k.Hout * k.Wout)) * k.Hin * k.Win * (size_t)k.lda * 2;
-    const size_t wb = (size_t)align_up((size_t)k.N, 64) * k.K * 2;
-    const bool conv_ok = k.mode == A_DENSE || (k.Cin % 64 == 0 && k.K == 9 * k.Cin);
+    const size_t wb = (size_t)align_up((size_t)k.N, 64) * k.K * 2 * (sub ? 4 : 1);
+    const bool conv_ok = k.mode == A_DENSE || (k.Cin % 64 == 0 && k.K == (sub ? 4 : (upb ? 16 : 9)) * k.Cin);
     if ((g_buf_stage & 1) && ab > 0 && conv_ok && ab + (size_t)(k.Win + 1) * k.lda * 2 < 0x7ff00000ull && wb < 0x7ff00000ull && k.lda % 8 == 0 &&
         ((size_t)k.A & 15) == 0 && ((size_t)k.W & 15) == 0) {
       k.pp_a_bytes = (unsigned)ab; k.pp_w_bytes = (unsigned)wb;
@@ -1467,6 +1637,35 @@
   if (force_tile) k.xa = 0;
 #endif
   const int epi = k.xa == 2 ? EPI_XATTN_DQ : (k.xa ? EPI_XATTN : glu);
+  enum { P_128x160_S4_K1_W1, P_256x128_S3_K1_W2, P_128x128_S4_K1_W2, P_128x64_S3_K1_W1, P_128x64_S3_K2_W1, P_128x320_S2_K1_W2, P_64x64_S4_K1_W1, P_128x128_S2_K1_W1, P_128x128_S4_K1_W1, P_128x64_S5_K1_W1 };
+  static const int kPickGeom[][5] = {{128, 160, 4, 1, 1}, {256, 128, 3, 1, 2}, {128, 128, 4, 1, 2}, {128, 64, 3, 1, 1}, {128, 64, 3, 2, 1}, {128, 320, 2, 1, 2}, {64, 64, 4, 1, 1}, {128, 128, 2, 1, 1}, {128, 128, 4, 1, 1}, {128, 64, 5, 1, 1}};
+  int pick = 0;
+  if (t160) pick = P_128x160_S4_K1_W1;
+  else if (mw2) pick = P_256x128_S3_K1_W2;
+  else if (BM == 128 && BN == 128 && (glu || (kMw128 && tiles_per_split >= kMw128))) pick = P_128x128_S4_K1_W2;
+  else if (kTwoPerCu && BM == 128 && BN == 64 && tiles * splits > 256 && tiles * splits <= 512)
+    pick = P_128x64_S3_K1_W1;
+  else if (BM == 128 && BN == 64 && tiles_per_split >= kKg2MinKt) pick = P_128x64_S3_K2_W1;
+  else if (BN == 320) pick = P_128x320_S2_K1_W2;
+  else if (BM == 64) pick = P_64x64_S4_K1_W1;
+  else if (BN == 128 && kManyBlocks > 0 && tiles * splits >= kManyBlocks) pick = P_128x128_S2_K1_W1;
+  else if (BN == 128) pick = P_128x128_S4_K1_W1;
+  else pick = P_128x64_S5_K1_W1;
+  const int* pg = kPickGeom[pick];
+  if (sub) {
+    bool ok = !use_pp && sub_tile(pg[0], pg[1], pg[2], 1, pg[3], pg[4]) && k.pp_a_bytes != 0 && sub_mlow % pg[0] == 0;
+#ifdef DH_TUNING
+    if (force_tile) ok = false;
+#endif
+    if (!ok) return gemm_dispatch<T>(k9, partial_elems, st, gn_done, lnb_done, xa_done, dtype, nullptr);
+  }
+  if (upb) {
+    bool ok = upb_tile(pg[0], pg[1], pg[2], 1, pg[3], pg[4]) && k.pp_a_bytes != 0;
+#ifdef DH_TUNING
+    if (force_tile) ok = false;
+#endif
+    if (!ok) return -1;
+  }
   hipEvent_t e0 = nullptr, e1 = nullptr;
   if (g_prof.on) {
     if (g_prof.used + 2 > g_prof.ev.size()) {
@@ -1480,13 +1679,14 @@
     const double esz = 2.0;
     double a_elems = (double)k.M * k.K;
     if (k.mode != A_DENSE && k.Hout > 0 && k.Wout > 0) a_elems = (double)k.M / ((double)k.Hout * k.Wout) * k.Hin * k.Win * k.Cin;
+    if (sub) a_elems = (double)sub_mlow * k.Cin;
     double c_elems = (double)k.M * k.N * (k.C ? 1.0 : 0.0) + (k.R ? (double)k.M * k.N : 0.0);
     if (k.glu_y) c_elems += 0.5 * (double)k.M * k.N;
     if (k.glub_x) c_elems += 4.0 * (double)k.M * k.glub_f - (k.C ? (double)k.M * k.glub_f : 0.0);
     if (k.gn_epi == 2) c_elems += (double)k.M * k.N;
     if (k.xa == 1) c_elems += (k.xa_save ? 1.0 : 0.0) * (double)k.M * k.N + 2.0 * (k.M / k.xa_Nq) * (double)k.xa_Nk * k.N;
     if (k.xa == 2) c_elems += 2.0 * (double)k.M * k.N + 2.0 * (k.M / k.xa_Nq) * (double)k.xa_Nk * k.N;
-    g_prof.bytes += esz * (a_elems + (double)k.N * k.K + c_elems);
+    g_prof.bytes += esz * (a_elems + (double)k.N * k.K * (sub ? 4.0 : 1.0) + c_elems);
     g_prof.e0 = e0; g_prof.e1 = e1;
   }
 #ifdef DH_TUNING
@@ -1508,21 +1708,24 @@
   else
 #endif
   if (use_pp) { pp.splits = splits; g_last_tile.bm = pp.bm; g_last_tile.bn = pp.bn; launch_gemm_pp(dtype, k, pp, st, g_prof.e0, g_prof.e1); }
-  else if (t160) launch_tile<T, 128, 160, 4, 1, 1, 1>(gm, false, grid, st, k);
-  else if (mw2) launch_tile<T, 256, 128, 3, 1, 1, 2>(gm, lnf, grid, st, k, glu);
-  else if (BM == 128 && BN == 128 && (glu || (kMw128 && tiles_per_split >= kMw128))) launch_tile<T, 128, 128, 4, 1, 1, 2>(gm, lnf, grid, st, k, glu);
-  else if (kTwoPerCu && BM == 128 && BN == 64 && tiles * splits > 256 && tiles * splits <= 512)
-    launch_tile<T, 128, 64, 3, 1, 1, 1>(gm, lnf, grid, st, k, epi);
-  else if (BM == 128 && BN == 64 && tiles_per_split >= kKg2MinKt) launch_tile<T, 128, 64, 3, 1, 2, 1>(gm, lnf, grid, st, k, epi);
-  else if (BN == 320) launch_tile<T, 128, 320, 2, 1, 1, 2>(gm, false, grid, st, k);
-  else if (BM == 64) launch_tile<T, 64, 64, 4, 1, 1, 1>(gm, lnf, grid, st, k, epi);
-  else if (BN == 128 && kManyBlocks > 0 && tiles * splits >= kManyBlocks) launch_tile<T, 128, 128, 2, 1, 1, 1>(gm, lnf, grid, st, k);
-  else if (BN == 128) launch_tile<T, 128, 128, 4, 1, 1, 1>(gm, lnf, grid, st, k);
-  else launch_tile<T, 128, 64, 5, 1, 1, 1>(gm, lnf, grid, st, k, epi);
+  else switch (pick) {
+    case P_128x160_S4_K1_W1: launch_tile<T, 128, 160, 4, 1, 1, 1>(gm, false, grid, st, k); break;
+    case P_256x128_S3_K1_W2: launch_tile<T, 256, 128, 3, 1, 1, 2>(gm, lnf, grid, st, k, glu); break;
+    case P_128x128_S4_K1_W2: launch_tile<T, 128, 128, 4, 1, 1, 2>(gm, lnf, grid, st, k, glu); break;
+    case P_128x64_S3_K1_W1: launch_tile<T, 128, 64, 3, 1, 1, 1>(gm, lnf, grid, st, k, epi); break;
+    case P_128x64_S3_K2_W1: launch_tile<T, 128, 64, 3, 1, 2, 1>(gm, lnf, grid, st, k, epi); break;
+    case P_128x320_S2_K1_W2: launch_tile<T, 128, 320, 2, 1, 1, 2>(gm, false, grid, st, k); break;
+    case P_64x64_S4_K1_W1: launch_tile<T, 64, 64, 4, 1, 1, 1>(gm, lnf, grid, st, k, epi); break;
+    case P_128x128_S2_K1_W1: launch_tile<T, 128, 128, 2, 1, 1, 1>(gm, lnf, grid, st, k); break;
+    case P_128x128_S4_K1_W1: launch_tile<T, 128, 128, 4, 1, 1, 1>(gm, lnf, grid, st, k); break;
+    case P_128x64_S5_K1_W1: launch_tile<T, 128, 64, 5, 1, 1, 1>(gm, lnf, grid, st, k, epi); break;
+  }
   g_prof.e0 = g_prof.e1 = nullptr;
   g_last_xattn = k.xa;
   if (k.xa) { ++g_xattn_total; *xa_done = 1; }
-  g_last_tile.splits = splits; g_last_tile.pp = use_pp ? 1 : 0; g_last_tile.gn_epi = k.gn_epi;
+  g_last_tile.splits = splits; g_last_tile.pp = use_pp ? 1 : 0; g_last_tile.gn_epi = k.gn_epi; g_last_tile.sub = sub ? 1 : 0;
+  if (sub) ++g_sub_total[sub_t2 ? 2 : 0];
+  if (upb) ++g_sub_total[1];
   if (k.gn_epi) *gn_done = k.gn_S;
   if (splits > 1) {
     if (k.gn_part && k.gn_G > 0 && k.gn_HW > 0 && k.N % k.gn_G == 0 && (GN_GB * (k.N / k.gn_G)) % 8 == 0 &&
@@ -1540,6 +1743,7 @@
       hipLaunchKernelGGL((k_splitk_reduce<T>), dim3((unsigned)((groups + 255) / 256)), dim3(256), 0, st, k);
     }
   }
+  return k.K;
 }
 #undef DH_KNOB
 
@@ -1572,12 +1776,15 @@
   k.xa = 0; k.xa_k = a.xa_k; k.xa_v = a.xa_v; k.xa_ldk = a.xa_ldk; k.xa_o = a.xa_o; k.xa_ldo = a.xa_ldo; k.xa_lse = a.xa_lse;
   k.xa_H = a.xa_H; k.xa_Nq = a.xa_Nq; k.xa_Nk = a.xa_Nk; k.xa_save = a.xa_save;
   k.xa_q = a.xa_q; k.xa_ldq = a.xa_ldq; k.xa_dq = a.xa_dq; k.xa_lddq = a.xa_lddq;
+  k.sub = 0; k.sub_mlow = 1;
   if (a.gn_done) *a.gn_done = 0;
   if (a.lnb_done) *a.lnb_done = 0;
   if (a.xa_done) *a.xa_done = 0;
-  if (dtype == DH_DTYPE_F16) gemm_dispatch<f16>(k, a.partial_elems, st, a.gn_done, a.lnb_done, a.xa_done, dtype);
-  else gemm_dispatch<bf16>(k, a.partial_elems, st, a.gn_done, a.lnb_done, a.xa_done, dtype);
-  return 2.0 * (double)a.M * (double)a.N * (double)a.K;
+  int kk;
+  if (dtype == DH_DTYPE_F16) kk = gemm_dispatch<f16>(k, a.partial_elems, st, a.gn_done, a.lnb_done, a.xa_done, dtype, a.W_sub);
+  else kk = gemm_dispatch<bf16>(k, a.partial_elems, st, a.gn_done, a.lnb_done, a.xa_done, dtype, a.W_sub);
+  if (kk < 0) return -1.0;
+  return 2.0 * (double)a.M * (double)a.N * (double)kk;
 }
 
 }
@@ -1602,6 +1809,30 @@
   const dh::GemmTileReport& r = dh::g_last_tile;
   const int v[9] = {r.bm, r.bn, r.kg, r.stages, r.mw, r.splits, r.pp, r.gn_epi, r.reduce_gn};
   for (int i = 0; i < 9; ++i) out[i] = v[i];
+  return DH_OK;
+}
+
+extern "C" int dh_dbg_gemm_subpixel_carried(int* last) {
+  DH_REQUIRE(last != nullptr, "null pointer");
+  *last = dh::g_last_tile.sub;
+  return DH_OK;
+}
+
+extern "C" int dh_dbg_gemm_subpixel_counts(long long* out) {
+  DH_REQUIRE(out != nullptr, "null pointer");
+  for (int i = 0; i < 3; ++i) out[i] = dh::g_sub_total[i];
+  return DH_OK;
+}
+
+extern "C" int dh_dbg_gemm_subpixel(int force) {
+  DH_REQUIRE(force == 0 || force == 2, "subpixel: 0 policy, 2 whenever the kernel can carry the launch");
+  dh::g_sub_force = force;
+  return DH_OK;
+}
+
+extern "C" int dh_dbg_gemm_force_splits(int splits) {
+  DH_REQUIRE(splits >= 0 && splits <= 32, "0..32 splits");
+  dh::g_force_splits = splits;
   return DH_OK;
 }
 
diff --git a/diffusionhandles_amd/csrc/gemm_k.h b/diffusionhandles_amd/csrc/gemm_k.h
--- a/diffusionhandles_amd/csrc/gemm_k.h
+++ b/diffusionhandles_amd/csrc/gemm_k.h
@@ -50,7 +50,13 @@
   int xa, xa_Nq, xa_Nk, xa_H, xa_save;
   const void *xa_k, *xa_v; long xa_ldk; void* xa_o; long xa_ldo; float* xa_lse;
   const void* xa_q; long xa_ldq; void* xa_dq; long xa_lddq;
+  int sub, sub_mlow;
 };
+__device__ __forceinline__ int sub_out_row(const GemmK& p, int m) {
+  const int ph = m / p.sub_mlow, ml = m - ph * p.sub_mlow;
+  const int hw = p.Hout * p.Wout, b = ml / hw, r = ml - b * hw, i = r / p.Wout, j = r - i * p.Wout;
+  return (b * 2 * p.Hout + 2 * i + (ph >> 1)) * 2 * p.Wout + 2 * j + (ph & 1);
+}
 
 
 __host__ __device__ constexpr bool glub_tile_is_glu(int n0, int glub_f) { return n0 < glub_f; }
diff --git a/diffusionhandles_amd/csrc/unet_engine.cpp b/diffusionhandles_amd/csrc/unet_engine.cpp
--- a/diffusionhandles_amd/csrc/unet_engine.cpp
+++ b/diffusionhandles_amd/csrc/unet_engine.cpp
@@ -27,6 +27,8 @@
   int N = 0, K = 0, taps = 1;
   bool has_bwd = true, f32 = false;
   int glu_F = 0;
+  bool has_sub = false; size_t sub_off = 0, upb_off = 0;
+  bool has_t2 = false; size_t t2_off = 0;
 };
 
 struct ParamInfo {
@@ -205,6 +207,15 @@
     o.type = OP_GEMM; o.mode = A_CONV3; o.in0 = x; o.res = res;
     o.Hin = Hs; o.Win = Hs; o.Cin = Cin; o.Hout = Ho; o.Wout = Ho; o.stride = stride; o.up = up;
     o.wt = weight(Cout, 9 * Cin, 9);
+    if (up && stride == 1 && Cin % 64 == 0 && Cout % 64 == 0) {
+      Wt& w = u.wts[o.wt];
+      w.has_sub = true; w.sub_off = u.w16_elems; u.w16_elems += align_up((size_t)16 * Cout * Cin, 128);
+      w.upb_off = u.w16_elems; u.w16_elems += align_up((size_t)16 * Cout * Cin, 128);
+    }
+    if (stride == 2 && !up && Cin % 64 == 0 && Cout % 64 == 0) {
+      Wt& w = u.wts[o.wt];
+      w.has_t2 = true; w.t2_off = u.w16_elems; u.w16_elems += align_up((size_t)16 * Cout * Cin, 128);
+    }
     bind_mat(pre + ".weight", o.wt, Cout, 0, Cin, 9);
     o.bias_off = param_f32(pre + ".bias", Cout);
     if (temb_off >= 0) { o.rowvec_off = u.temb_f32_off + temb_off; o.rowvec_ld = u.temb_total; }
@@ -680,6 +691,13 @@
   }
   if (u->dtype == DH_DTYPE_F16) fold_ff_t<f16>(u, st);
   else fold_ff_t<bf16>(u, st);
+  for (const Wt& w : u->wts)
+    if (w.has_sub) {
+      launch_subpixel_weights(u->dtype, u->w16 + w.fwd_off, w.N, w.K / 9, u->w16 + w.sub_off, st);
+      launch_upb_weights(u->dtype, u->w16 + w.fwd_off, w.N, w.K / 9, u->w16 + w.upb_off, st);
+    }
+  for (const Wt& w : u->wts)
+    if (w.has_t2 && w.has_bwd) launch_t2_weights(u->w16 + w.bwd_off, w.K / 9, w.N, u->w16 + w.t2_off, st);
   u->fold_dirty = false;
 }
 
@@ -854,6 +872,7 @@
   g.M = B * to.rows; g.N = w.N; g.K = w.K;
   g.mode = o.mode; g.Hin = o.Hin; g.Win = o.Win; g.Cin = o.Cin; g.Hout = o.Hout; g.Wout = o.Wout;
   g.stride = o.stride; g.up = o.up;
+  if (o.up && w.has_sub) g.W_sub = u->w16 + w.sub_off;
   g.bias = o.bias_off >= 0 ? u->pf + o.bias_off : nullptr;
   if (o.rowvec_off >= 0) { g.rowvec = u->f32a + o.rowvec_off; g.rowvec_ld = o.rowvec_ld; g.rows_per_batch = to.rows; }
   if (o.res >= 0) { g.R = u->aptr(o.res); g.ldr = u->tens[o.res].ld; }
@@ -1185,6 +1204,16 @@
           u->flops_bwd += launch_gemm(dt, g, st);
           u->gready[o.in0] = 1;
         } else if (o.up) {
+          if (w.has_sub) {
+            GemmArgs h;
+            h.A = g.A; h.lda = g.lda; h.W = u->w16 + w.upb_off; h.partial = g.partial; h.partial_elems = g.partial_elems;
+            h.mode = A_UPT4; h.Hin = o.Hout; h.Win = o.Wout; h.Cin = w.N; h.Hout = o.Hin; h.Wout = o.Win;
+            h.M = B * o.Hin * o.Win; h.N = o.Cin; h.K = 16 * w.N;
+            h.C = u->gptr(o.in0); h.ldc = ti.C;
+            if (u->gready[o.in0]) { h.R = h.C; h.ldr = ti.C; }
+            const double fl = launch_gemm(dt, h, st);
+            if (fl >= 0) { u->flops_bwd += fl; u->gready[o.in0] = 1; break; }
+          }
           g.mode = A_CONV3; g.stride = 1; g.up = 0;
           g.Hin = o.Hout; g.Win = o.Wout; g.Cin = w.N; g.Hout = o.Hout; g.Wout = o.Wout;
           g.M = B * o.Hout * o.Wout; g.N = o.Cin; g.K = 9 * w.N;
@@ -1194,6 +1223,7 @@
           u->gready[o.in0] = 1;
         } else {
           g.mode = o.stride == 2 ? A_CONVT2 : A_CONV3;
+          if (o.stride == 2 && w.has_t2) g.W_sub = u->w16 + w.t2_off;
           g.stride = 1; g.up = 0;
           g.Hin = o.Hout; g.Win = o.Wout; g.Cin = w.N;
           g.Hout = o.Hin; g.Wout = o.Win;
@@ -1431,3 +1461,22 @@
   DH_LAUNCH_CHECK();
   return DH_OK;
 }
+
+extern "C" int dh_dbg_unet_subpixel_weights(dh_unet* u, int i, int* n_convs, int* N, int* Cin, void* w, void* w9, void* stream) {
+  DH_REQUIRE(u && n_convs && N && Cin, "null pointer");
+  hipStream_t st = (hipStream_t)stream;
+  std::vector<const Wt*> subs;
+  for (const Wt& wt : u->wts) if (wt.has_sub) subs.push_back(&wt);
+  *n_convs = (int)subs.size();
+  *N = 0; *Cin = 0;
+  if (i < 0 || i >= (int)subs.size()) return DH_OK;
+  if (u->fold_dirty) fold_layernorms(u, st);
+  const Wt& wt = *subs[i];
+  *N = wt.N; *Cin = wt.K / 9;
+  if (w) launch_untile_subpixel(u->w16 + wt.sub_off, wt.N, wt.K / 9, w, st);
+  if (w9)
+    hipLaunchKernelGGL((k_untile<unsigned short>), dim3(cdiv(wt.N * wt.K, 256)), dim3(256), 0, st,
+                       (const unsigned short*)(u->w16 + wt.fwd_off), wt.N, wt.K, (unsigned short*)w9);
+  DH_LAUNCH_CHECK();
+  return DH_OK;
+}
diff --git a/diffusionhandles_amd/csrc/unet_kernels.h b/diffusionhandles_amd/csrc/unet_kernels.h
--- a/diffusionhandles_amd/csrc/unet_kernels.h
+++ b/diffusionhandles_amd/csrc/unet_kernels.h
@@ -22,7 +22,7 @@
 __host__ __device__ inline int glu_col(int o, int gate) { return 32 * (o >> 4) + 16 * gate + (o & 15); }
 __host__ __device__ inline int glu_src_row(int n, int F) { return ((n >> 4) & 1) * F + 16 * (n >> 5) + (n & 15); }
 
-enum { A_DENSE = 0, A_CONV3 = 1, A_CONVT2 = 2 };
+enum { A_DENSE = 0, A_CONV3 = 1, A_CONVT2 = 2, A_UPT4 = 3 };
 
 struct GemmArgs {
   const void* A = nullptr; long lda = 0;
@@ -50,6 +50,7 @@
   const void *xa_k = nullptr, *xa_v = nullptr; long xa_ldk = 0; void* xa_o = nullptr; long xa_ldo = 0; float* xa_lse = nullptr;
   int xa_H = 0, xa_Nq = 0, xa_Nk = 0, xa_save = 1; int* xa_done = nullptr;
   const void* xa_q = nullptr; long xa_ldq = 0; void* xa_dq = nullptr; long xa_lddq = 0;
+  const void* W_sub = nullptr;
 };
 void launch_splitk_reduce_ln_bwd(int dtype, const float* partial, int splits, const void* x, const float* gamma,
                                  const float* stats, const void* add, void* dx, int rows, int C, hipStream_t st, long ldx = 0);
@@ -62,6 +63,16 @@
 }
 
 __host__ __device__ inline int conv_k_index(int tap, int c) { return (c >> 6) * 576 + tap * 64 + (c & 63); }
+
+__host__ __device__ inline int sub_k_index(int tap, int c) { return (c >> 6) * 256 + tap * 64 + (c & 63); }
+__host__ __device__ inline int sub_tap_lo(int a, int t) { return a == 0 ? (t == 0 ? 0 : 1) : (t == 0 ? 0 : 2); }
+__host__ __device__ inline int sub_tap_hi(int a, int t) { return a == 0 ? (t == 0 ? 1 : 3) : (t == 0 ? 2 : 3); }
+void launch_subpixel_weights(int dtype, const void* w9, int N, int Cin, void* out, hipStream_t st);
+__host__ __device__ inline int upb_k_index(int tap, int c) { return (c >> 6) * 1024 + tap * 64 + (c & 63); }
+void launch_upb_weights(int dtype, const void* w9, int N, int Cin, void* out, hipStream_t st);
+void launch_t2_weights(const void* wb, int N, int C, void* out, hipStream_t st);
+void launch_untile_upb(const void* tiled, int N, int Cin, void* plain, hipStream_t st);
+void launch_untile_subpixel(const void* tiled, int N, int Cin, void* plain, hipStream_t st);
 
 void launch_load_weight(int dtype, const float* src, int N, int C, int taps, void* fwd, long fwd_K, long row_off, void* bwd,
                         long bwd_K, long col_off, int Nb, float scale, hipStream_t st);
diff --git a/diffusionhandles_amd/csrc/vae_engine.cpp b/diffusionhandles_amd/csrc/vae_engine.cpp
--- a/diffusionhandles_amd/csrc/vae_engine.cpp
+++ b/diffusionhandles_amd/csrc/vae_engine.cpp
@@ -50,7 +50,7 @@
 enum VOp { V_CONV_IN, V_CONV_OUT, V_CONV, V_LINEAR, V_GN, V_ATTN };
 
 struct VTen { size_t off; int H, C; };
-struct VWt { size_t off; int N, K, taps; bool f32; };
+struct VWt { size_t off; int N, K, taps; bool f32; bool has_sub = false; size_t sub_off = 0; };
 struct VParam { std::string name; int ndim; int64_t shape[4]; int wt; int row_off; long f32_off; float scale; };
 struct VOpRec {
   int type = 0, in0 = -1, out = -1, res = -1, wt = -1;
@@ -76,6 +76,7 @@
   size_t partial_elems = 0;
   int t_out = -1;
   bool encoder = false;
+  bool sub_dirty = true;
 };
 
 namespace {
@@ -127,6 +128,10 @@
     o.type = V_CONV; o.in0 = x; o.res = res; o.Hin = t.H; o.Cin = t.C; o.up = up; o.stride = stride; o.pad = pad;
     o.Hout = stride == 2 ? t.H / 2 : t.H << up;
     o.wt = weight(Cout, 9 * t.C, 9, false);
+    if (up && stride == 1 && pad == 1 && t.C % 64 == 0 && Cout % 64 == 0) {
+      VWt& w = v.wts[o.wt];
+      w.has_sub = true; w.sub_off = v.w16_elems; v.w16_elems += align_up((size_t)16 * Cout * t.C, 128);
+    }
     bind(pre + ".weight", o.wt, Cout, 0, t.C, 9);
     o.bias = pf32(pre + ".bias", Cout);
     o.out = tensor(o.Hout, Cout);
@@ -375,6 +380,7 @@
     return DH_OK;
   }
   const VWt& w = v->wts[p.wt];
+  if (w.has_sub) v->sub_dirty = true;
   void* dst = w.f32 ? (void*)(v->pf + w.off) : (void*)(v->w16 + w.off);
   launch_load_weight(w.f32 ? DH_DTYPE_F32 : v->dtype, src, (int)p.shape[0], (int)p.shape[1], w.taps, dst, w.K, p.row_off, nullptr, 0, 0, w.N,
                      p.scale, st);
@@ -394,6 +400,11 @@
   const size_t in_elems = v->encoder ? (size_t)R * R * c.out_channels : (size_t)S * S * c.latent_channels;
   const size_t out_elems = v->encoder ? (size_t)S * S * 2 * c.latent_channels : (size_t)R * R * c.out_channels;
   auto aptr = [&](int t) { return v->act + v->tens[t].off; };
+  if (v->sub_dirty) {
+    for (const VWt& w : v->wts)
+      if (w.has_sub) launch_subpixel_weights(dt, v->w16 + w.off, w.N, w.K / 9, v->w16 + w.sub_off, st);
+    v->sub_dirty = false;
+  }
   for (int b = 0; b < batch; ++b) {
     const float* zb = z + (size_t)b * in_elems;
     float* ib = image + (size_t)b * out_elems;
@@ -418,6 +429,7 @@
           if (o.type == V_CONV) {
             g.mode = A_CONV3; g.Hin = o.Hin; g.Win = o.Hin; g.Cin = o.Cin; g.Hout = o.Hout; g.Wout = o.Hout; g.stride = o.stride; g.up = o.up;
             g.pad = o.pad;
+            if (o.up && w.has_sub) g.W_sub = v->w16 + w.sub_off;
           }
           g.bias = v->pf + o.bias;
           if (o.res >= 0) { g.R = aptr(o.res); g.ldr = v->tens[o.res].C; }
```
